# aynik/carta1

Measured on AMD Instinct MI355X. Metric: atrac1_stereo_frames_per_s_encode, higher is better.
Workload: dtype f32+f64

## Files before the change

carta1_amd/csrc/c1_api.hip:

```cpp
#include <algorithm>
#include <cmath>
#include <cstdarg>
#include <cstdio>
#include <cstdlib>
#include <cstring>
#include <limits>
#include <map>
#include <memory>
#include <atomic>
#include <mutex>
#include <string>
#include <thread>
#include <vector>

#include "c1_internal.h"
#include "c1_detect_bound.h"

#pragma clang fp contract(off)

namespace {

#include "c1_default_tables.inc"

thread_local std::string g_error;
// ... 66 lines not shown
  }
  for (int i = 0; i < 16; i++) { d->pre32_64[i][0] = (float)t.mdct_fwd64[2 * i]; d->pre32_64[i][1] = (float)t.mdct_fwd64[2 * i + 1]; }
  for (int i = 0; i < 64; i++) { d->pre32_256[i][0] = (float)t.mdct_fwd256[2 * i]; d->pre32_256[i][1] = (float)t.mdct_fwd256[2 * i + 1]; }
  for (int i = 0; i < 128; i++) { d->pre32_512[i][0] = (float)t.mdct_fwd512[2 * i]; d->pre32_512[i][1] = (float)t.mdct_fwd512[2 * i + 1]; }
  auto sigma2 = [&](const double *tab, int pairs, double want) {
    double mx = 0;
    for (int i = 0; i < pairs; i++) {
      const double m = tab[2 * i] * tab[2 * i] + tab[2 * i + 1] * tab[2 * i + 1];
      if (!(std::fabs(m - want) <= 1e-9 * want)) ok = false;
      mx = std::max(mx, m);
    }
    return mx;
  };
  const double s64 = sigma2(t.mdct_fwd64, 16, 0.5 / 64), s256 = sigma2(t.mdct_fwd256, 64, 0.5 / 256), s512 = sigma2(t.mdct_fwd512, 128, 1.0 / 512);
  const double (*tw)[2] = d->fft_tw;
  for (int h = 1; h <= 128; h <<= 1)
    for (int k = 0; k < h; k++) {
      const double ang = -M_PI * (double)k / (double)h;
      if (std::fabs(tw[h - 1 + k][0] - std::cos(ang)) > 1e-12 || std::fabs(tw[h - 1 + k][1] - std::sin(ang)) > 1e-12) ok = false;
    }
  for (int r = 0; r < 2; r++) {
    const int h = r == 0 ? 4 : 16;
    for (int k = 0; k < h; k++) {
      const double *a = tw[h - 1 + k], *b = tw[2 * h - 1 + k];
      float (*dst)[2] = r == 0 ? d->r4b[k] : d->r4c[k];
      dst[0][0] = (float)a[0]; dst[0][1] = (float)a[1];
      dst[1][0] = (float)b[0]; dst[1][1] = (float)b[1];
      dst[2][0] = (float)(a[0] * b[0] - a[1] * b[1]);
      dst[2][1] = (float)(a[0] * b[1] + a[1] * b[0]);
    }
  }
  for (int k = 0; k < 64; k++) { d->r2d[k][0] = (float)tw[63 + k][0]; d->r2d[k][1] = (float)tw[63 + k][1]; }
  for (int i = 0; i < 64 * 16; i++) d->norm32[i] = (float)d->norm[i];
  for (int i = 0; i < 16; i++) { d->inv32_64[i][0] = (float)t.mdct_inv64[2 * i]; d->inv32_64[i][1] = (float)t.mdct_inv64[2 * i + 1]; }
  for (int i = 0; i < 64; i++) { d->inv32_256[i][0] = (float)t.mdct_inv256[2 * i]; d->inv32_256[i][1] = (float)t.mdct_inv256[2 * i + 1]; }
  for (int i = 0; i < 128; i++) { d->inv32_512[i][0] = (float)t.mdct_inv512[2 * i]; d->inv32_512[i][1] = (float)t.mdct_inv512[2 * i + 1]; }
  for (int i = 0; i < 256; i++) { d->tw32[i][0] = (float)tw[i][0]; d->tw32[i][1] = (float)tw[i][1]; }
  const double u = std::ldexp(1.0, -24) * kSpecTheta;
  const double ka64 = kSpecKAPost + kSpecKARoundA + 2 * kSpecKARound4 + kSpecKAPre;
  const double ka128 = ka64 + kSpecKARound2;
  const double ka16 = kSpecKAPost + kSpecKARoundA + kSpecKARound4 + kSpecKAPre;
  for (int b = 0; b < 3; b++) {
    const double n = b == 2 ? 128 : 64, sg2 = b == 2 ? s512 : s256;
    d->spec_cz[b] = round_up_f32(u * (b == 2 ? ka128 : ka64) * std::sqrt(sg2 * n));
    const double gb = u * sg2 * std::sqrt(2 * n);
    if (b == 2) { d->spec_cw[b] = round_up_f32(gb * (5 * kSpecGH + kSpecGQ)); d->spec_cl[b] = 0.0f; }
    else { d->spec_cw[b] = round_up_f32(gb * kSpecGH * kSpecGQ); d->spec_cl[b] = round_up_f32(gb * (7 * kSpecGH + kSpecGQ)); }
    d->spec_cz_short[b] = round_up_f32(u * ka16 * std::sqrt(s64 * 16));
    const double gs = u * s64 * std::sqrt(2.0 * 16);
    if (b == 2) { d->spec_cw_short[b] = round_up_f32(gs * (5 * kSpecGH + kSpecGQ)); d->spec_cl_short[b] = 0.0f; }
    else { d->spec_cw_short[b] = round_up_f32(gs * kSpecGH * kSpecGQ); d->spec_cl_short[b] = round_up_f32(gs * (7 * kSpecGH + kSpecGQ)); }
  }
  d->spec_cz[3] = d->spec_cw[3] = d->spec_cl[3] = d->spec_cz_short[3] = d->spec_cw_short[3] = d->spec_cl_short[3] = 0.0f;
  d->spec_eabs = (float)std::ldexp(1.0, -70);
  for (int b = 0; b < 3; b++)
    d->det_ck[b] = round_up_f32(std::ldexp(1.0, -24) * C1_DET_THETA * (b == 2 ? C1_DET_K256 * 16.0 : C1_DET_K128 * std::sqrt(128.0)));
  d->det_ck[3] = 0.0f;
  d->det_eabs = round_up_f32(C1_DET_EABS);
  d->spec_ok = ok ? 1 : 0;
}

void build_device_tables(const c1_tables &t, C1DevTables *d) {
  memset(d, 0, sizeof *d);
  qmf_even_taps(d->tap_e);
  for (int j = 0; j < 24; j++) d->tap_o[j] = d->tap_e[23 - j];
  memcpy(d->window, t.window_short, sizeof d->window);
  memcpy(d->mdct_fwd64, t.mdct_fwd64, sizeof d->mdct_fwd64);
  memcpy(d->mdct_fwd256, t.mdct_fwd256, sizeof d->mdct_fwd256);
  memcpy(d->mdct_fwd512, t.mdct_fwd512, sizeof d->mdct_fwd512);
  memcpy(d->mdct_inv64, t.mdct_inv64, sizeof d->mdct_inv64);
  memcpy(d->mdct_inv256, t.mdct_inv256, sizeof d->mdct_inv256);
  memcpy(d->mdct_inv512, t.mdct_inv512, sizeof d->mdct_inv512);
  int stage = 0;
  for (int h = 1; h <= 128; h <<= 1, stage++) {
    const double wr = t.fft_w[stage][0], wi = t.fft_w[stage][1];
    double tr = 1.0, ti = 0.0;
    for (int k = 0; k < h; k++) {
      d->fft_tw[h - 1 + k][0] = tr;
      d->fft_tw[h - 1 + k][1] = ti;
      const double nr = tr * wr - ti * wi;
      ti = tr * wi + ti * wr;
      tr = nr;
    }
  }
  memcpy(d->scale_factors, t.scale_factors, sizeof d->scale_factors);
  for (int s = 0; s < 64; s++)
    for (int wl = 0; wl < 16; wl++) {
      const int bits = wl == 0 ? 0 : wl + 1;
      const int range = bits ? (1 << (bits - 1)) - 1 : 0;
      d->norm[s * 16 + wl] = (double)range / t.scale_factors[s];
    }
  d->log1p10 = t.log1p_10;
  auto floor_f32_bits = [](double x) -> uint32_t {
    float f = (float)x;
    if ((double)f > x) f = std::nextafterf(f, 0.0f);
    uint32_t u;
    memcpy(&u, &f, 4);
    return u;
  };
  d->sf_m1 = floor_f32_bits(C1D_SCALE_FACTORS[1]) & 0x7fffffu;
  d->sf_m2 = floor_f32_bits(C1D_SCALE_FACTORS[2]) & 0x7fffffu;
  d->sf_fast = 1;
  const uint32_t tm1 = floor_f32_bits(t.scale_factors[1]) & 0x7fffffu, tm2 = floor_f32_bits(t.scale_factors[2]) & 0x7fffffu;
  for (int i = 0; i < 64; i++) {
    const uint32_t u = floor_f32_bits(t.scale_factors[i]);
    const int e = (int)(u >> 23) - 127, want_e = i / 3 - 21;
    const uint32_t frac = u & 0x7fffffu, want = i % 3 == 0 ? 0u : (i % 3 == 1 ? tm1 : tm2);
    const bool exact_pow2 = i % 3 != 0 || (double)std::ldexp(1.0f, want_e) == t.scale_factors[i];
    if (e != want_e || frac != want || !exact_pow2) d->sf_fast = 0;
  }
  d->dq_fast = 1;
  d->dq_step = 1;
  for (int wl = 1; wl < 16 && d->dq_fast; wl++) {
    const int bits = wl + 1;
    const double range = (double)((1 << (bits - 1)) - 1), y = 1.0 / range;
    d->inv_range[wl] = y;
    for (int s = 1; s < 64 && d->dq_fast; s++) {
      const double sf = t.scale_factors[s];
      for (int q = -(1 << (bits - 1)); q < (1 << (bits - 1)); q++) {
        const double a = (double)q * sf;
        const double q0 = a * y, r = std::fma(-q0, range, a), fast = std::fma(r, y, q0), exact = a / range;
        if (!(fast == exact) || std::signbit(fast) != std::signbit(exact)) { d->dq_fast = 0; break; }
        const float f_exact = (float)exact, f_step = (float)((double)q * (sf * y));
        if (!(f_step == f_exact) || std::signbit(f_step) != std::signbit(f_exact)) d->dq_step = 0;
      }
    }
  }
  if (!d->dq_fast || getenv("C1_NO_DQ_STEP")) d->dq_step = 0;
  build_spec_tables(t, d);
}

int fill_call_fields(const c1_encode_options &o, C1DevEncOpts *d) {
  if (std::isnan(o.transient_threshold)) return fail(C1_ERR_ARG, "transient_threshold is NaN");
  d->threshold = o.transient_threshold;
  const bool detect = o.fixed_block_modes[0] < 0;
  for (int b = 0; b < 3; b++) {
    const int m = o.fixed_block_modes[b];
    if (detect) { d->modes[b] = -1; continue; }
    if (m < 0 || m > (b == 2 ? 3 : 2))
      return fail(C1_ERR_ARG, "fixed_block_modes[%d] = %d is outside 0..%d", b, m, b == 2 ? 3 : 2);
    d->modes[b] = m;
  }
  static const int no_tonal = getenv("C1_ALLOC_NO_TONAL") ? atoi(getenv("C1_ALLOC_NO_TONAL")) : 0;
  d->alloc_no_tonal = no_tonal;
  return C1_OK;
}

int build_table_fields(const c1_encode_options &o, C1DevEncOpts *d);

int build_encode_opts(const c1_encode_options &o, C1DevEncOpts *d) {
  struct Entry { double biased[64]; C1DevEncOpts table_part; };
  static std::mutex mu;
  static std::vector<Entry> cache;
  bool hit = false;
  {
    std::lock_guard<std::mutex> lock(mu);
    for (const Entry &e : cache)
      if (memcmp(e.biased, o.biased_scale_factors, sizeof e.biased) == 0) { *d = e.table_part; hit = true; break; }
  }
  if (!hit) {
    const int rc = build_table_fields(o, d);
    if (rc) return rc;
    std::lock_guard<std::mutex> lock(mu);
    if (cache.size() >= 8) cache.erase(cache.begin());
    Entry e;
    memcpy(e.biased, o.biased_scale_factors, sizeof e.biased);
    e.table_part = *d;
    cache.push_back(e);
  }
  return fill_call_fields(o, d);
}

int build_table_fields(const c1_encode_options &o, C1DevEncOpts *d) {
  memset(d, 0, sizeof *d);
  for (int i = 0; i < 64; i++) {
    if (!std::isfinite(o.biased_scale_factors[i]) || o.biased_scale_factors[i] < 0)
      return fail(C1_ERR_ARG, "biased_scale_factors[%d] is not a finite non-negative number", i);
    d->biased[i] = o.biased_scale_factors[i];
  }
  {
    const double l1 = std::log2(d->biased[1]), l63 = std::log2(d->biased[63]);
    const double slope = (l63 - l1) / 62.0;
    d->la_slope = (std::isfinite(slope) && std::isfinite(l1)) ? (float)slope : 0.0f;
    d->la_off = (std::isfinite(slope) && std::isfinite(l1)) ? (float)(l1 - slope) : 0.0f;
  }
  float pri[64 * 15];
  std::vector<float> uniq;
  for (int s = 1; s < 64; s++)
    for (int wl = 0; wl < 15; wl++) {
      const int b0 = wl == 0 ? 0 : wl + 1, b1 = wl + 2;
      const double ddf = wl == 0 ? 2.0 - std::ldexp(1.0, -b1) : std::ldexp(1.0, -b0) - std::ldexp(1.0, -b1);
      const double dbits = (double)(b1 - b0);
      pri[s * 15 + wl] = (float)(d->biased[s] * ddf / dbits);
      uniq.push_back(pri[s * 15 + wl]);
    }
  std::sort(uniq.begin(), uniq.end());
  uniq.erase(std::unique(uniq.begin(), uniq.end()), uniq.end());
  for (int s = 1; s < 64; s++)
    for (int wl = 0; wl < 15; wl++) {
      const auto it = std::lower_bound(uniq.begin(), uniq.end(), pri[s * 15 + wl]);
      d->rank[s * 16 + wl] = (uint16_t)(1 + (it - uniq.begin()));
    }
  d->rank_affine = 0;
  {
    std::vector<int> order;
    for (int s = 1; s < 64; s++)
      for (int wl = 0; wl < 15; wl++) order.push_back(s * 16 + wl);
    std::sort(order.begin(), order.end(), [&](int x, int y) { return d->rank[x] < d->rank[y]; });
    for (int A = 1; A <= 12 && !d->rank_affine; A++)
      for (int B = 1; B <= 36 && !d->rank_affine; B++)
        for (int C = -2 * B; C <= 2 * B && !d->rank_affine; C++) {
          auto key = [&](int idx) { const int s = idx >> 4, wl = idx & 15; return wl == 0 ? A * s + C : A * s - B * wl - B; };
          bool ok = true;
          int lo = key(order[0]), hi = lo;
          for (size_t i = 1; i < order.size() && ok; i++) {
            const int k0 = key(order[i - 1]), k1 = key(order[i]);
            const bool req = d->rank[order[i]] == d->rank[order[i - 1]];
            if (req ? (k1 != k0) : !(k1 > k0)) ok = false;
            lo = std::min(lo, k1); hi = std::max(hi, k1);
          }
          if (ok && hi - lo + 1 < 1023) {
            d->rank_affine = 1; d->rank_a = A; d->rank_b = B; d->rank_c = C; d->rank_off = 1 - lo;
          }
        }
  }
  if (d->rank_affine) {
    const int A = d->rank_a, B = d->rank_b, C = d->rank_c, off = d->rank_off;
    auto rk = [&](int s, int wl) { return wl == 0 ? A * s + C + off : A * s + off - B * (wl + 1); };
    auto entry = [&](int s, int wl) { return ((uint32_t)rk(s, wl) << 21) | ((uint32_t)s << 10) | ((uint32_t)wl << 6); };
    d->rank_step0 = (1u << 6) + ((uint32_t)(-2 * B - C) << 21);
    d->rank_step = (1u << 6) - ((uint32_t)B << 21);
    bool ok = true;
    for (int s = 1; s < 64 && ok; s++)
      for (int wl = 0; wl < 15 && ok; wl++) {
        if (rk(s, wl) < 1 || rk(s, wl) > 1022) ok = false;
        if (wl < 14 && entry(s, wl) + (wl == 0 ? d->rank_step0 : d->rank_step) != entry(s, wl + 1)) ok = false;
      }
    if (!ok) { d->rank_affine = 0; d->rank_step0 = d->rank_step = 0; }
  }
  {
    bool ok = true;
    for (int c = 0; c < 8; c++) {
      const double size = (double)kDistSizes[c];
      for (int s = 0; s < 64; s++) {
        const double bs = d->biased[s];
        const double zb = s != 0 ? (double)(float)(bs * 2.0 * size) : 0.0;
        const double cs = bs * size;
        d->dist[c][s][0] = zb;
        d->dist[c][s][1] = cs;
        if (s == 0) continue;
        if (!(zb >= (double)std::numeric_limits<float>::min())) ok = false;
        uint64_t u;
        memcpy(&u, &cs, sizeof u);
        for (int wl = 1; wl <= 15; wl++) {
          const int bits = wl + 1;
          const double want = bs * std::ldexp(1.0, -bits) * size;
          if ((int)((u >> 52) & 0x7ff) <= bits || (int)((u >> 52) & 0x7ff) == 0x7ff) { ok = false; continue; }
          const uint64_t v = u - ((uint64_t)bits << 52);
          if (memcmp(&v, &want, sizeof v) != 0) ok = false;
        }
      }
    }
    d->dist_tables = (ok && !getenv("C1_NO_DIST_TABLES")) ? 1 : 0;
  }
  return C1_OK;
}

constexpr int kTotals = 8;
constexpr int64_t kSpecMinUnits = 64;
constexpr int kListHead = 8;
constexpr int64_t kMaxModesBatchFrames = (int64_t)1 << 22;
constexpr int64_t kMaxChunkFrames = (int64_t)1 << 27;
constexpr bool kSignalStartsFused = false;

struct Timing {
  hipEvent_t start, stop;
  int kind;
};
enum { K_ANALYSIS = 0, K_ALLOCATE, K_PACK, K_DECODE, K_REDO, K_PACK_UNITS, K_DECODE_FIELDS, K_FROM_STATE, K_SIGNAL_STARTS, K_CHOOSE, K_MEASURE, K_METER, K_METER_PCM, K_KINDS };
const char *const kKindNames[K_KINDS] = {"analysis", "allocate", "pack", "decode", "redo", "pack_units", "decode_fields", "from_state", "signal_starts", "choose", "measure", "meter", "meter_pcm"};

}

struct c1_ctx {
  std::recursive_mutex mu;
  int device = 0;
  hipStream_t stream = nullptr;
  bool own_stream = false;
  C1DevTables *d_tables = nullptr;
  C1DevEncOpts *d_opts = nullptr;
  c1_encode_options last_opts;
  bool have_opts = false;
  int64_t ws_units = 0;
  float *d_coefs[2] = {nullptr, nullptr};
  uint8_t *d_side[2] = {nullptr, nullptr};
  uint8_t *d_alloc[2] = {nullptr, nullptr};
  uint8_t *d_cand[2] = {nullptr, nullptr};
  uint32_t *d_work[2] = {nullptr, nullptr};
  float *d_eps[2] = {nullptr, nullptr};
  uint32_t *d_redo[2] = {nullptr, nullptr};
  unsigned long long *d_spec_totals = nullptr;
  int spec_mode = 1;
  float spec_defer = 1.0f;
  bool decode_binary32 = false;
  int decode_model = C1_DECODE_EXACT;
  bool spec_tables_ok = false;
  int64_t det_units = 0;
  float *d_bands[2] = {nullptr, nullptr};
  double *d_feat[2] = {nullptr, nullptr};
  uint8_t *d_modes[2] = {nullptr, nullptr};
  uint32_t *d_lists[2] = {nullptr, nullptr};
  C1DevEncOpts *d_palette = nullptr;
  double *d_mask = nullptr, *h_mask = nullptr;
  hipEvent_t ev_mask = nullptr;
  double pal_tables[C1_MAX_BIAS_PALETTE][64];
  int pal_n = 0;
  uint32_t *d_pal_lists = nullptr;
  int64_t pal_entries = 0;
  uint8_t *d_trial = nullptr;
  int64_t trial_units = 0, trial_n = 0;
  float *d_bm_coefs = nullptr;
  uint8_t *d_bm_side = nullptr, *d_bm_cand_side = nullptr;
  int64_t bm_units = 0;
  bool overlap = false;
  hipStream_t s_tail = nullptr;
  hipEvent_t ev_main[2] = {nullptr, nullptr}, ev_tail[2] = {nullptr, nullptr};
  bool tail_used[2] = {false, false};
  bool tail_pending = false;
  int ws_next = 0;
  int64_t chunk_frames = 0;
  bool pipeline = true;
  int measured_wide = -1;
  bool signal_starts_fused = false;
  hipStream_t s_ana = nullptr, s_rest = nullptr;
  hipEvent_t ev_in = nullptr, ev_ana[2] = {nullptr, nullptr}, ev_free[2] = {nullptr, nullptr}, ev_end[2] = {nullptr, nullptr};
  int timing_depth = 0;
  bool profiling = false;
  std::vector<Timing> timings;
  std::vector<hipEvent_t> event_pool;
  double ms[K_KINDS] = {};
  int launches[K_KINDS] = {};
  void *d_io = nullptr;
  size_t d_io_bytes = 0;
  void *d_sig = nullptr;
  size_t d_sig_bytes = 0;
  uint32_t *h_rows = nullptr;
  size_t h_rows_bytes = 0;
  hipEvent_t ev_rows = nullptr;
  bool rows_pending = false;
  hipStream_t s_up = nullptr, s_down = nullptr;
  void *d_ring = nullptr;
  size_t d_ring_bytes = 0;
  hipEvent_t ev_up[2] = {nullptr, nullptr}, ev_run[2] = {nullptr, nullptr}, ev_down[2] = {nullptr, nullptr};
};

namespace {

#define CTX_GUARD(c)                                   \
  std::unique_lock<std::recursive_mutex> ctx_guard_;   \
  if (c) ctx_guard_ = std::unique_lock<std::recursive_mutex>((c)->mu)

int join_tail(c1_ctx *ctx) {
  if (!ctx->tail_pending) return C1_OK;
  for (int p = 0; p < 2; p++)
    if (ctx->tail_used[p]) HIP_TRY(hipStreamWaitEvent(ctx->stream, ctx->ev_tail[p], 0));
  ctx->tail_pending = false;
  return C1_OK;
}

int ctx_bind(c1_ctx *ctx, bool join = true) {
  if (!ctx) return fail(C1_ERR_ARG, "context is NULL");
  HIP_TRY(hipSetDevice(ctx->device));
  if (join) return join_tail(ctx);
  return C1_OK;
}

void free_workspace(c1_ctx *ctx) {
  for (int p = 0; p < 2; p++) {
    if (ctx->d_coefs[p]) (void)hipFree(ctx->d_coefs[p]);
    if (ctx->d_side[p]) (void)hipFree(ctx->d_side[p]);
    if (ctx->d_alloc[p]) (void)hipFree(ctx->d_alloc[p]);
    if (ctx->d_cand[p]) (void)hipFree(ctx->d_cand[p]);
    if (ctx->d_work[p]) (void)hipFree(ctx->d_work[p]);
    if (ctx->d_eps[p]) (void)hipFree(ctx->d_eps[p]);
    if (ctx->d_redo[p]) (void)hipFree(ctx->d_redo[p]);
    ctx->d_coefs[p] = nullptr; ctx->d_side[p] = nullptr; ctx->d_alloc[p] = nullptr; ctx->d_cand[p] = nullptr; ctx->d_work[p] = nullptr;
    ctx->d_eps[p] = nullptr; ctx->d_redo[p] = nullptr;
  }
  ctx->ws_units = 0;
  for (int p = 0; p < 2; p++) {
    if (ctx->d_bands[p]) (void)hipFree(ctx->d_bands[p]);
    if (ctx->d_feat[p]) (void)hipFree(ctx->d_feat[p]);
    if (ctx->d_modes[p]) (void)hipFree(ctx->d_modes[p]);
    if (ctx->d_lists[p]) (void)hipFree(ctx->d_lists[p]);
    ctx->d_bands[p] = nullptr; ctx->d_feat[p] = nullptr; ctx->d_modes[p] = nullptr; ctx->d_lists[p] = nullptr;
  }
  ctx->det_units = 0;
  if (ctx->d_pal_lists) (void)hipFree(ctx->d_pal_lists);
  ctx->d_pal_lists = nullptr;
  ctx->pal_entries = 0;
  if (ctx->d_trial) (void)hipFree(ctx->d_trial);
  ctx->d_trial = nullptr;
  ctx->trial_units = ctx->trial_n = 0;
  if (ctx->d_bm_coefs) (void)hipFree(ctx->d_bm_coefs);
  if (ctx->d_bm_side) (void)hipFree(ctx->d_bm_side);
  if (ctx->d_bm_cand_side) (void)hipFree(ctx->d_bm_cand_side);
  ctx->d_bm_coefs = nullptr; ctx->d_bm_side = nullptr; ctx->d_bm_cand_side = nullptr;
  ctx->bm_units = 0;
}

int ensure_detect_workspace(c1_ctx *ctx, int64_t units) {
  if (units <= ctx->det_units) return C1_OK;
  HIP_TRY(hipDeviceSynchronize());
  for (int p = 0; p < (ctx->pipeline ? 2 : 1); p++) {
    if (ctx->d_bands[p]) (void)hipFree(ctx->d_bands[p]);
    if (ctx->d_feat[p]) (void)hipFree(ctx->d_feat[p]);
    if (ctx->d_modes[p]) (void)hipFree(ctx->d_modes[p]);
    if (ctx->d_lists[p]) (void)hipFree(ctx->d_lists[p]);
    ctx->d_bands[p] = nullptr; ctx->d_feat[p] = nullptr; ctx->d_modes[p] = nullptr; ctx->d_lists[p] = nullptr;
    HIP_TRY(hipMalloc(&ctx->d_bands[p], (size_t)(units + C1_MAX_CHANNELS) * 512 * sizeof(float)));
    HIP_TRY(hipMalloc(&ctx->d_feat[p], (size_t)(units + C1_MAX_CHANNELS) * kFeatureWsDoubles * sizeof(double)));
    HIP_TRY(hipMalloc(&ctx->d_modes[p], (size_t)units));
    HIP_TRY(hipMalloc(&ctx->d_lists[p], ((size_t)units * 3 + 4) * sizeof(uint32_t)));
  }
  ctx->det_units = units;
  return C1_OK;
}

int ensure_workspace(c1_ctx *ctx, int64_t units) {
  if (units <= ctx->ws_units) return C1_OK;
  HIP_TRY(hipDeviceSynchronize());
  free_workspace(ctx);
  ctx->tail_used[0] = ctx->tail_used[1] = false;
  ctx->tail_pending = false;
  for (int p = 0; p < ((ctx->pipeline || ctx->overlap) ? 2 : 1); p++) {
    HIP_TRY(hipMalloc(&ctx->d_coefs[p], (size_t)units * 512 * sizeof(float)));
    HIP_TRY(hipMalloc(&ctx->d_side[p], (size_t)units * kSideBytes));
    HIP_TRY(hipMalloc(&ctx->d_alloc[p], (size_t)units * kAllocBytes));
    HIP_TRY(hipMalloc(&ctx->d_cand[p], (size_t)units * kCandidateBytes));
    HIP_TRY(hipMalloc(&ctx->d_work[p], ((size_t)units * 8 + 4) * sizeof(uint32_t)));
    HIP_TRY(hipMalloc(&ctx->d_eps[p], (size_t)units * kEpsFloats * sizeof(float)));
    HIP_TRY(hipMalloc(&ctx->d_redo[p], ((size_t)units * 4 + kListHead + 64) * sizeof(uint32_t)));
  }
  ctx->ws_units = units;
  return C1_OK;
}

constexpr size_t kWsBytesPerUnit = 512 * sizeof(float) + kSideBytes + kAllocBytes + kCandidateBytes + 8 * sizeof(uint32_t) + kEpsFloats * sizeof(float) + 4 * sizeof(uint32_t);
constexpr size_t kDetectWsBytesPerUnit = 512 * sizeof(float) + kFeatureWsDoubles * sizeof(double) + 1 + 3 * sizeof(uint32_t);
constexpr size_t kBestModesWsBytesPerUnit = 512 * sizeof(float) + 2 * kSideBytes;
int64_t chunk_for_call(c1_ctx *ctx, int64_t frames, int channels, bool detect, int trial_n = 0, bool best_modes = false) {
  const int64_t want = std::min(frames, ctx->chunk_frames);
  const bool trial_fits = trial_n == 0 || (want * channels <= ctx->trial_units && trial_n <= ctx->trial_n);
  if (want * channels <= ctx->ws_units && (!detect || want * channels <= ctx->det_units) && trial_fits &&
      (!best_modes || want * channels <= ctx->bm_units)) return want;
  size_t free_b = 0, total_b = 0;
  if (hipMemGetInfo(&free_b, &total_b) != hipSuccess) { (void)hipGetLastError(); return std::min<int64_t>(want, 1048576); }
  const size_t sets = (ctx->pipeline || ctx->overlap) ? 2 : 1, det_sets = ctx->pipeline ? 2 : 1;
  size_t avail = free_b + (size_t)ctx->ws_units * kWsBytesPerUnit * sets;
  size_t per_unit = kWsBytesPerUnit * sets;
  if (detect) { avail += (size_t)ctx->det_units * kDetectWsBytesPerUnit * det_sets; per_unit += kDetectWsBytesPerUnit * det_sets; }
  if (trial_n > 0) { avail += (size_t)ctx->trial_units * ctx->trial_n * kAllocBytes; per_unit += (size_t)trial_n * kAllocBytes; }
  if (best_modes) { avail += (size_t)ctx->bm_units * kBestModesWsBytesPerUnit; per_unit += kBestModesWsBytesPerUnit; }
  const int64_t fit = (int64_t)((double)avail * 0.9 / (double)per_unit) / channels;
  return std::max<int64_t>(16, std::min(want, fit));
}

void bind_lists(c1_ctx *ctx, int p, C1EncodeLaunch *L) {
  uint32_t *base = ctx->d_redo[p];
  const size_t u = (size_t)ctx->ws_units;
  L->redo_count = base;
  L->realloc_count = base + 1;
  L->reana_count = base + 2;
  L->redo_list = base + kListHead;
  L->realloc_list = base + kListHead + u;
  L->reana_list = base + kListHead + 2 * u;
}
void bind_defer(c1_ctx *ctx, int p, C1EncodeLaunch *L) {
  L->defer_list = ctx->d_redo[p] + kListHead + 3 * (size_t)ctx->ws_units;
}

int ensure_io(c1_ctx *ctx, size_t bytes) {
  if (bytes <= ctx->d_io_bytes) return C1_OK;
  if (ctx->d_io) hipFree(ctx->d_io);
  ctx->d_io = nullptr; ctx->d_io_bytes = 0;
  HIP_TRY(hipMalloc(&ctx->d_io, bytes));
  ctx->d_io_bytes = bytes;
  return C1_OK;
}

int upload_opts(c1_ctx *ctx, const c1_encode_options *opts) {
  if (!opts) return fail(C1_ERR_ARG, "options are NULL");
  if (ctx->have_opts && memcmp(&ctx->last_opts, opts, sizeof *opts) == 0) return C1_OK;
  C1DevEncOpts h;
  const int rc = build_encode_opts(*opts, &h);
  if (rc) return rc;
  int jr = join_tail(ctx);
  if (jr) return jr;
  HIP_TRY(hipStreamSynchronize(ctx->stream));
  HIP_TRY(hipMemcpy(ctx->d_opts, &h, sizeof h, hipMemcpyHostToDevice));
  ctx->last_opts = *opts;
  ctx->have_opts = true;
  return C1_OK;
}

struct PaletteCall {
  int n;
  const uint8_t *index;
};

int check_palette(const char *what, const c1_encode_options *palette, int n, bool call_fields) {
  if (n < 1 || n > C1_MAX_BIAS_PALETTE) return fail(C1_ERR_ARG, "%s: n_palette = %d is outside 1..%d", what, n, C1_MAX_BIAS_PALETTE);
  if (!palette) return fail(C1_ERR_ARG, "%s: palette is NULL", what);
  std::unique_ptr<C1DevEncOpts> d(new C1DevEncOpts);
  for (int k = 0; k < n; k++) {
    c1_encode_options o = palette[k];
    if (!call_fields) {
      o.transient_threshold = 1.0;
      o.fixed_block_modes[0] = o.fixed_block_modes[1] = o.fixed_block_modes[2] = -1;
    }
    const int rc = build_encode_opts(o, d.get());
    if (rc) { const std::string inner = g_error; return fail(rc, "%s: palette entry %d: %s", what, k, inner.c_str()); }
    if (call_fields && k > 0) {
      if (memcmp(&palette[k].transient_threshold, &palette[0].transient_threshold, sizeof(double)) != 0)
        return fail(C1_ERR_ARG, "%s: palette entry %d: transient_threshold differs from entry 0's, and no modes are given", what, k);
      if (memcmp(palette[k].fixed_block_modes, palette[0].fixed_block_modes, sizeof palette[0].fixed_block_modes) != 0)
        return fail(C1_ERR_ARG, "%s: palette entry %d: fixed_block_modes differ from entry 0's, and no modes are given", what, k);
    }
  }
  return C1_OK;
}

int check_measured_opts(const char *what, const c1_encode_options *opts, bool call_fields) {
  if (!opts) return fail(C1_ERR_ARG, "%s: options are NULL", what);
  std::unique_ptr<C1DevEncOpts> d(new C1DevEncOpts);
  c1_encode_options o = *opts;
  if (!call_fields) {
    o.transient_threshold = 1.0;
    o.fixed_block_modes[0] = o.fixed_block_modes[1] = o.fixed_block_modes[2] = -1;
  }
  const int rc = build_encode_opts(o, d.get());
  if (rc) { const std::string inner = g_error; return fail(rc, "%s: %s", what, inner.c_str()); }
  return C1_OK;
}

int upload_palette(c1_ctx *ctx, const char *what, const c1_encode_options *palette, int n) {
  bool same = ctx->d_palette && ctx->pal_n >= n;
  for (int k = 0; k < n && same; k++) same = memcmp(ctx->pal_tables[k], palette[k].biased_scale_factors, sizeof ctx->pal_tables[k]) == 0;
  if (same) return C1_OK;
  std::unique_ptr<C1DevEncOpts[]> h(new C1DevEncOpts[C1_MAX_BIAS_PALETTE]);
  for (int k = 0; k < n; k++) {
    c1_encode_options o = palette[k];
    o.transient_threshold = 1.0;
    o.fixed_block_modes[0] = o.fixed_block_modes[1] = o.fixed_block_modes[2] = -1;
    const int rc = build_encode_opts(o, &h[k]);
    if (rc) { const std::string inner = g_error; return fail(rc, "%s: palette entry %d: %s", what, k, inner.c_str()); }
  }
  int jr = join_tail(ctx);
  if (jr) return jr;
  HIP_TRY(hipStreamSynchronize(ctx->stream));
  if (!ctx->d_palette) HIP_TRY(hipMalloc(&ctx->d_palette, C1_MAX_BIAS_PALETTE * sizeof(C1DevEncOpts)));
  ctx->pal_n = 0;
  HIP_TRY(hipMemcpy(ctx->d_palette, h.get(), (size_t)n * sizeof(C1DevEncOpts), hipMemcpyHostToDevice));
  for (int k = 0; k < n; k++) memcpy(ctx->pal_tables[k], palette[k].biased_scale_factors, sizeof ctx->pal_tables[k]);
  ctx->pal_n = n;
  return C1_OK;
}

int ensure_palette_lists(c1_ctx *ctx, int64_t units, int n) {
  const int64_t entries = units * n;
  if (entries <= ctx->pal_entries) return C1_OK;
  HIP_TRY(hipDeviceSynchronize());
  if (ctx->d_pal_lists) (void)hipFree(ctx->d_pal_lists);
  ctx->d_pal_lists = nullptr; ctx->pal_entries = 0;
  HIP_TRY(hipMalloc(&ctx->d_pal_lists, ((size_t)entries + 8) * sizeof(uint32_t)));
  ctx->pal_entries = entries;
  return C1_OK;
}

int ensure_trial_allocs(c1_ctx *ctx, int64_t units, int n) {
  if (units <= ctx->trial_units && n <= ctx->trial_n) return C1_OK;
  HIP_TRY(hipDeviceSynchronize());
  if (ctx->d_trial) (void)hipFree(ctx->d_trial);
  ctx->d_trial = nullptr; ctx->trial_units = ctx->trial_n = 0;
  const int64_t u = std::max(units, ctx->trial_units), planes = std::max<int64_t>(n, ctx->trial_n);
  HIP_TRY(hipMalloc(&ctx->d_trial, (size_t)u * planes * kAllocBytes));
  ctx->trial_units = u; ctx->trial_n = planes;
  return C1_OK;
}

int ensure_best_modes_planes(c1_ctx *ctx, int64_t units) {
  if (units <= ctx->bm_units) return C1_OK;
  HIP_TRY(hipDeviceSynchronize());
  if (ctx->d_bm_coefs) (void)hipFree(ctx->d_bm_coefs);
  if (ctx->d_bm_side) (void)hipFree(ctx->d_bm_side);
  if (ctx->d_bm_cand_side) (void)hipFree(ctx->d_bm_cand_side);
  ctx->d_bm_coefs = nullptr; ctx->d_bm_side = nullptr; ctx->d_bm_cand_side = nullptr; ctx->bm_units = 0;
  HIP_TRY(hipMalloc(&ctx->d_bm_coefs, (size_t)units * 512 * sizeof(float)));
  HIP_TRY(hipMalloc(&ctx->d_bm_side, (size_t)units * kSideBytes));
  HIP_TRY(hipMalloc(&ctx->d_bm_cand_side, (size_t)units * kSideBytes));
  ctx->bm_units = units;
  return C1_OK;
}

struct BestModesCall {
  int n;
  const uint8_t *cand;
  uint8_t *choice, *modes_out;
  double *distortion, *energy;
  const int8_t *sf_offsets = nullptr;
  int n_offsets = 0;
  uint8_t *taken = nullptr;
  int8_t *shifts = nullptr;
};

struct BestBiasCall {
  int n;
  uint8_t *choice;
  double *distortion, *energy;
};

struct MeasuredCall {
  uint8_t *taken;
  double *distortion, *energy;
  const int8_t *sf_offsets = nullptr;
  int n_offsets = 0;
  int8_t *shifts = nullptr;
  const double *mask = nullptr;
  bool has_spread = false;
  double *weights = nullptr;
};

int check_index_bytes(const char *what, const uint8_t *index, int64_t frames, int channels, int n) {
  for (int64_t i = 0; i < frames * channels; i++) {
    if (index[i] < n) continue;
    if (channels == 2) return fail(C1_ERR_ARG, "%s: frame %lld, channel %d: bias index %d is not below n_palette = %d", what, (long long)(i / 2), (int)(i & 1), (int)index[i], n);
    return fail(C1_ERR_ARG, "%s: frame %lld: bias index %d is not below n_palette = %d", what, (long long)i, (int)index[i], n);
  }
  return C1_OK;
}

hipEvent_t take_event(c1_ctx *ctx) {
  if (!ctx->event_pool.empty()) {
    hipEvent_t e = ctx->event_pool.back();
    ctx->event_pool.pop_back();
    return e;
  }
  hipEvent_t e;
  hipEventCreateWithFlags(&e, hipEventDisableSystemFence);
  return e;
}
struct ScopedTiming {
  c1_ctx *ctx;
  Timing t;
  bool on;
  hipStream_t stream;
  ScopedTiming(c1_ctx *c, int kind, hipStream_t s = nullptr) : ctx(c), on(c->profiling), stream(s ? s : c->stream) {
    if (!on) return;
    t.kind = kind;
    t.start = take_event(ctx);
    t.stop = take_event(ctx);
    (void)hipEventRecord(t.start, stream);
  }
  ~ScopedTiming() {
    if (!on) return;
    (void)hipEventRecord(t.stop, stream);
    ctx->timings.push_back(t);
  }
};
void reset_timings(c1_ctx *ctx) {
  for (auto &t : ctx->timings) { ctx->event_pool.push_back(t.start); ctx->event_pool.push_back(t.stop); }
  ctx->timings.clear();
  for (int k = 0; k < K_KINDS; k++) { ctx->ms[k] = 0; ctx->launches[k] = 0; }
}
int collect_timings(c1_ctx *ctx) {
  if (ctx->timings.empty()) return C1_OK;
  int jr = join_tail(ctx);
  if (jr) return jr;
  HIP_TRY(hipStreamSynchronize(ctx->stream));
  for (auto &t : ctx->timings) {
    float ms = 0;
    HIP_TRY(hipEventElapsedTime(&ms, t.start, t.stop));
    ctx->ms[t.kind] += ms;
    ctx->launches[t.kind]++;
    ctx->event_pool.push_back(t.start);
    ctx->event_pool.push_back(t.stop);
  }
  ctx->timings.clear();
  return C1_OK;
}

void launch_measured(c1_ctx *ctx, const C1EncodeLaunch &L, bool all_long, const MeasuredCall *mc, int64_t at, hipStream_t stream) {
  ScopedTiming t(ctx, K_MEASURE, stream);
  uint8_t *taken = mc->taken ? mc->taken + at : nullptr;
  int8_t *shifts = mc->shifts ? mc->shifts + at * 52 : nullptr;
  double *distortion = mc->distortion ? mc->distortion + at * 2 : nullptr, *energy = mc->energy ? mc->energy + at : nullptr;
  double *weights = mc->weights ? mc->weights + at * 52 : nullptr;
  const bool finalize = L.units != nullptr;
  const int64_t units = L.frames * L.channels;
  const bool wide = ctx->measured_wide < 0 ? units <= kMeasuredWideUnits : ctx->measured_wide != 0;
  if (wide) {
    static const int8_t kNoOffset[1] = {0};
    c1k_launch_measured_wide(L, all_long, finalize, mc->sf_offsets ? mc->sf_offsets : kNoOffset, mc->sf_offsets ? mc->n_offsets : 1, mc->mask,
                             mc->has_spread, taken, mc->sf_offsets ? shifts : nullptr, distortion, energy, weights, stream);
  } else if (mc->mask) {
    c1k_launch_measured_masked(L, all_long, finalize, mc->sf_offsets, mc->n_offsets, mc->mask, mc->has_spread, taken, shifts, distortion,
                               energy, weights, stream);
  } else if (mc->sf_offsets) {
    c1k_launch_measured_sf(L, all_long, finalize, mc->sf_offsets, mc->n_offsets, taken, shifts, distortion, energy, stream);
  } else {
    c1k_launch_measured_alloc(L, all_long, finalize, taken, distortion, energy, stream);
  }
}

void launch_measured_modes(c1_ctx *ctx, const C1EncodeLaunch &L, const uint8_t *trial, int64_t trial_stride, const BestModesCall *bm,
                           int64_t at, hipStream_t stream) {
  ScopedTiming t(ctx, K_MEASURE, stream);
  const int64_t units = L.frames * L.channels;
  const bool wide = ctx->measured_wide < 0 ? units <= kMeasuredModesWideUnits : ctx->measured_wide != 0;
  (wide ? c1k_launch_measured_modes_wide : c1k_launch_measured_modes)(
      L, ctx->d_bm_coefs, ctx->d_bm_side, trial, trial_stride, bm->cand, bm->n, bm->sf_offsets, bm->n_offsets, L.units != nullptr,
      bm->choice ? bm->choice + at : nullptr, bm->modes_out ? bm->modes_out + at : nullptr, bm->taken ? bm->taken + at : nullptr,
      bm->shifts ? bm->shifts + at * 52 : nullptr, bm->distortion ? bm->distortion + at * bm->n * 2 : nullptr,
      bm->energy ? bm->energy + at * bm->n : nullptr, stream);
}

int check_channels(int channels) {
  if (channels != 1 && channels != 2) return fail(C1_ERR_ARG, "channels must be 1 or 2, got %d", channels);
  return C1_OK;
}

int check_mode_bytes(const char *what, const uint8_t *modes, int64_t frames, int channels) {
  static const char *const kField[3] = {"low", "mid", "high"};
  for (int64_t i = 0; i < frames * channels; i++) {
    const int b = modes[i];
    if ((b & ~0x3a) == 0 && ((b & 0x30) == 0 || (b & 0x30) == 0x30)) continue;
    char where[64];
    if (channels == 2) snprintf(where, sizeof where, "frame %lld, channel %d", (long long)(i / 2), (int)(i & 1));
    else snprintf(where, sizeof where, "frame %lld", (long long)i);
    for (int k = 0; k < 3; k++) {
      const int m = (b >> (2 * k)) & 3, other = k == 2 ? 3 : 2;
      if (m != 0 && m != other)
        return fail(C1_ERR_ARG, "%s: %s: %s field of mode byte 0x%02x is %d, not 0 or %d", what, where, kField[k], b, m, other);
    }
    return fail(C1_ERR_ARG, "%s: %s: bits 6-7 of mode byte 0x%02x are set", what, where, b);
  }
  return C1_OK;
}

int encode_device_impl(c1_ctx *ctx, const float *const *pcm, int channels, int64_t frames, int halo_frames,
                       const c1_encode_options *opts, uint8_t *units, float *bands, float *coefs_tap,
                       uint8_t *side_tap, uint8_t *alloc_tap, bool lazy = false, const uint8_t *given_modes = nullptr,
                       const PaletteCall *pal = nullptr, const BestBiasCall *best = nullptr, const BestModesCall *bm = nullptr,
                       const MeasuredCall *mc = nullptr) {
  CTX_GUARD(ctx);
  int rc = ctx_bind(ctx, false);
  if (rc) return rc;
  if ((rc = check_channels(channels))) return rc;
  if (frames < 0) return fail(C1_ERR_ARG, "frames must be >= 0");
  if (halo_frames < 0 || halo_frames > 2) return fail(C1_ERR_ARG, "halo_frames must be 0, 1 or 2");
  if (!pcm) return fail(C1_ERR_ARG, "pcm is NULL");
  for (int c = 0; c < channels; c++) {
    if (!pcm[c] && frames > 0) return fail(C1_ERR_ARG, "pcm[%d] is NULL", c);
    if ((uintptr_t)pcm[c] & 15) return fail(C1_ERR_ARG, "pcm[%d] must be 16-byte aligned on the device", c);
  }
  if ((rc = upload_opts(ctx, opts))) return rc;
  if (ctx->profiling && ctx->timing_depth == 0) reset_timings(ctx);
  if (frames == 0) return C1_OK;
  const bool detect = given_modes || bm || opts->fixed_block_modes[0] < 0;
  const bool taps = coefs_tap || side_tap || alloc_tap;
  const int64_t chunk = taps ? ctx->chunk_frames : chunk_for_call(ctx, frames, channels, detect, best ? best->n : (bm ? bm->n : 0), bm != nullptr);
  if ((rc = ensure_workspace(ctx, (taps ? frames : std::min(frames, chunk)) * channels))) return rc;
  if (detect && (rc = ensure_detect_workspace(ctx, (taps ? frames : std::min(frames, chunk)) * channels))) return rc;
  if (pal && (rc = ensure_palette_lists(ctx, std::min(frames, chunk) * channels, pal->n))) return rc;
  if (best && (rc = ensure_trial_allocs(ctx, std::min(frames, chunk) * channels, best->n))) return rc;
  if (bm && (rc = ensure_trial_allocs(ctx, std::min(frames, chunk) * channels, bm->n))) return rc;
  if (bm && (rc = ensure_best_modes_planes(ctx, std::min(frames, chunk) * channels))) return rc;
  bool bm_long = false, bm_short = false;
  for (int k = 0; bm && k < bm->n; k++) {
    if ((bm->cand[k] & 0x3f) != 0x3a) bm_long = true;
    if ((bm->cand[k] & 0x3f) != 0) bm_short = true;
  }
  if (taps && (!coefs_tap || !side_tap || !alloc_tap)) return fail(C1_ERR_ARG, "coefs, side and alloc taps must be given together");
  if (taps && frames > kMaxChunkFrames) return fail(C1_ERR_ARG, "stage taps are not chunked: at most %lld frames per call", (long long)kMaxChunkFrames);
  const bool all_long_modes = !detect && opts->fixed_block_modes[0] == 0 && opts->fixed_block_modes[1] == 0 &&
                              opts->fixed_block_modes[2] == 0 && !getenv("C1_NO_FAST_LONG");
  const bool all_short_modes = !detect && opts->fixed_block_modes[0] != 0 && opts->fixed_block_modes[1] != 0 &&
                               opts->fixed_block_modes[2] != 0;
  bool speculate = (all_long_modes || all_short_modes) && !taps && !pal && !best && !bm && !mc && units && ctx->spec_tables_ok && ctx->spec_mode != 0;
  bool quantize32 = !taps && units && ctx->spec_tables_ok && ctx->spec_mode != 0;
  static const bool det_spec_env_off = getenv("C1_DETECT_SPEC") && atoi(getenv("C1_DETECT_SPEC")) == 0;
  bool detect_spec = detect && !given_modes && !bm && !taps && ctx->spec_tables_ok && ctx->spec_mode != 0 && !det_spec_env_off;
  if (ctx->spec_mode == 1 && frames * channels < kSpecMinUnits) speculate = quantize32 = detect_spec = false;
  const bool overlap = speculate && ctx->overlap && ctx->s_tail != nullptr;
  if (!overlap && (rc = join_tail(ctx))) return rc;
  const bool piped = ctx->pipeline && !taps && frames > chunk && !speculate && !bm;
  hipStream_t sA = piped ? ctx->s_ana : ctx->stream, sB = piped ? ctx->s_rest : ctx->stream;
  if (piped) {
    HIP_TRY(hipEventRecord(ctx->ev_in, ctx->stream));
    HIP_TRY(hipStreamWaitEvent(sA, ctx->ev_in, 0));
    HIP_TRY(hipStreamWaitEvent(sB, ctx->ev_in, 0));
  }
  int64_t index = 0;
  for (int64_t f0 = 0, n = 0; f0 < frames; f0 += n, ++index) {
    n = taps ? frames : std::min(chunk, frames - f0);
    int p = piped ? (int)(index & 1) : 0;
    if (overlap) { p = ctx->ws_next; ctx->ws_next ^= 1; }
    C1EncodeLaunch L;
    memset(&L, 0, sizeof L);
    for (int c = 0; c < channels; c++) L.pcm[c] = pcm[c] + f0 * 512;
    L.channels = channels;
    L.frames = n;
    L.halo_frames = (int)std::min<int64_t>(2, f0 + halo_frames);
    L.tables = ctx->d_tables;
    L.opts = ctx->d_opts;
    L.coefs = taps ? coefs_tap : ctx->d_coefs[p];
    L.side = taps ? side_tap : ctx->d_side[p];
    L.alloc = taps ? alloc_tap : ctx->d_alloc[p];
    L.cand = ctx->d_cand[p];
    L.work_count = ctx->d_work[p];
    L.work_list = ctx->d_work[p] + 4;
    L.sel_list = ctx->d_work[p] + 4 + (size_t)ctx->ws_units * 7;
    L.bands = bands ? bands + f0 * channels * 512 : nullptr;
    L.units = units ? units + f0 * channels * C1_UNIT_BYTES : nullptr;
    const bool all_long = all_long_modes;
    if (piped && index >= 2) HIP_TRY(hipStreamWaitEvent(sA, ctx->ev_free[p], 0));
    if (speculate) {
      L.eps = ctx->d_eps[p];
      bind_lists(ctx, p, &L);
      if (ctx->spec_mode == 1) { bind_defer(ctx, p, &L); L.spec_defer = ctx->spec_defer; }
      if (c1k_pick_run(n, channels, 0) <= 64 && !getenv("C1_NO_SF_PREPASS"))
        L.open_masks = reinterpret_cast<unsigned long long *>((reinterpret_cast<uintptr_t>(ctx->d_redo[p] + kListHead + 3 * (size_t)ctx->ws_units + (size_t)ctx->ws_units / 4 + 4) + 7) & ~(uintptr_t)7);
      if (overlap && ctx->tail_used[p]) HIP_TRY(hipStreamWaitEvent(sA, ctx->ev_tail[p], 0));
      HIP_TRY(hipMemsetAsync(ctx->d_redo[p], 0, kListHead * sizeof(uint32_t), sA));
      {
        ScopedTiming t(ctx, K_ANALYSIS, sA);
        c1k_launch_analysis_spec(L, all_short_modes, sA);
        if (L.defer_list) {
          C1EncodeLaunch D = L;
          uint32_t *dense = ctx->d_redo[p] + kListHead + 2 * (size_t)ctx->ws_units;
          c1k_launch_defer_compact(L, dense, ctx->d_redo[p] + 3, sA);
          D.unit_list = dense;
          D.unit_count = ctx->d_redo[p] + 3;
          D.list_runs = 1;
          D.defer_list = nullptr;
          if (all_long_modes) c1k_launch_analysis_long(D, sA); else c1k_launch_analysis(D, false, sA);
        }
      }
      if (L.open_masks) {
        ScopedTiming t(ctx, K_REDO, sA);
        {
          C1EncodeLaunch X = L;
          uint32_t *open_list = ctx->d_redo[p] + kListHead + 2 * (size_t)ctx->ws_units;
          c1k_launch_open_compact(L, open_list, ctx->d_redo[p] + 5, sA);
          X.unit_list = open_list;
          X.unit_count = ctx->d_redo[p] + 5;
          X.list_runs = 0;
          X.list_zero_eps = 1;
          X.defer_list = nullptr;
          X.open_masks = nullptr;
          if (all_long_modes) c1k_launch_analysis_long(X, sA); else c1k_launch_analysis(X, false, sA);
        }
      }
      { ScopedTiming t(ctx, K_ALLOCATE, sA); c1k_launch_allocate(L, sA); }
      if (overlap && ctx->tail_used[p ^ 1]) HIP_TRY(hipStreamWaitEvent(sA, ctx->ev_tail[p ^ 1], 0));
      { ScopedTiming t(ctx, K_PACK, sA); c1k_launch_pack_spec(L, all_long_modes, sA); }
      hipStream_t sT = sA;
      if (overlap) {
        sT = ctx->s_tail;
        HIP_TRY(hipEventRecord(ctx->ev_main[p], sA));
        HIP_TRY(hipStreamWaitEvent(sT, ctx->ev_main[p], 0));
      }
      {
        ScopedTiming t(ctx, K_REDO, sT);
        hipStream_t sA = sT;
        C1EncodeLaunch R = L;
        R.defer_list = nullptr;
        R.unit_list = L.reana_list;
        R.unit_count = L.reana_count;
        if (all_long_modes) c1k_launch_analysis_long(R, sA); else c1k_launch_analysis(R, false, sA);
        if (!L.open_masks) {
          C1EncodeLaunch A = R;
          A.unit_list = L.realloc_list;
          A.unit_count = L.realloc_count;
          c1k_launch_allocate(A, sA);
        }
        R.unit_list = L.redo_list;
        R.unit_count = L.redo_count;
        c1k_launch_pack(R, all_long_modes, sA);
        c1k_launch_spec_totals(ctx->d_spec_totals, (uint64_t)(n * channels), ctx->d_redo[p], 0, sA);
      }
      if (overlap) {
        HIP_TRY(hipEventRecord(ctx->ev_tail[p], sT));
        ctx->tail_used[p] = true;
        ctx->tail_pending = true;
      }
      continue;
    }
    {
      ScopedTiming t(ctx, K_ANALYSIS, sA);
      if (all_long) c1k_launch_analysis_long(L, sA);
      else if (bm) {
        C1EncodeLaunch S2 = L;
        S2.coefs = ctx->d_bm_coefs;
        S2.side = ctx->d_bm_side;
        HIP_TRY(hipMemsetAsync(ctx->d_bm_cand_side, bm_long ? 0 : 0x3a, (size_t)n * channels, sA));
        c1k_launch_modes_front(L, ctx->d_bm_cand_side, ctx->d_bands[p], ctx->d_modes[p], ctx->d_lists[p], sA);
        c1k_launch_mdct_bands(bm_long ? L : S2, ctx->d_bands[p], ctx->d_modes[p], ctx->d_lists[p], sA);
        if (bm_long && bm_short) {
          c1k_launch_const_mode_lists(0x3a, n * channels, ctx->d_modes[p], ctx->d_lists[p], sA);
          c1k_launch_mdct_bands(S2, ctx->d_bands[p], ctx->d_modes[p], ctx->d_lists[p], sA);
        }
      } else if (given_modes) {
        c1k_launch_modes_front(L, given_modes + f0 * channels, ctx->d_bands[p], ctx->d_modes[p], ctx->d_lists[p], sA);
        c1k_launch_mdct_bands(L, ctx->d_bands[p], ctx->d_modes[p], ctx->d_lists[p], sA);
      } else if (detect) {
        c1k_launch_detect(L, ctx->d_bands[p], ctx->d_feat[p], ctx->d_modes[p], ctx->d_lists[p], detect_spec, nullptr, sA);
        if (detect_spec) c1k_launch_spec_totals(ctx->d_spec_totals, (uint64_t)(n * channels), ctx->d_lists[p] + 2, 2, sA);
        if (L.bands) HIP_TRY(hipMemcpyAsync(L.bands, ctx->d_bands[p] + (size_t)channels * 512, (size_t)n * channels * 512 * sizeof(float),
                                            hipMemcpyDeviceToDevice, sA));
      } else c1k_launch_analysis(L, false, sA);
    }
    if (piped) {
      HIP_TRY(hipEventRecord(ctx->ev_ana[p], sA));
      HIP_TRY(hipStreamWaitEvent(sB, ctx->ev_ana[p], 0));
    }
    if (bm) {
      const int64_t trial_stride = ctx->trial_units * kAllocBytes;
      for (int k = 0; k < bm->n; k++) {
        { ScopedTiming t(ctx, K_ANALYSIS, sB); c1k_launch_compose_side(L.side, ctx->d_bm_side, n * channels, bm->cand[k], ctx->d_bm_cand_side, sB); }
        ScopedTiming t(ctx, K_ALLOCATE, sB);
        C1EncodeLaunch A = L;
        A.side = ctx->d_bm_cand_side;
        A.alloc = ctx->d_trial + (size_t)k * trial_stride;
        c1k_launch_allocate(A, sB);
      }
      if (bm->sf_offsets) {
        launch_measured_modes(ctx, L, ctx->d_trial, trial_stride, bm, f0 * channels, sB);
      } else {
        ScopedTiming t(ctx, K_CHOOSE, sB);
        c1k_launch_choose_modes(L, ctx->d_bm_coefs, ctx->d_bm_side, ctx->d_trial, trial_stride, bm->cand, bm->n, L.units != nullptr,
                                bm->choice ? bm->choice + f0 * channels : nullptr, bm->modes_out ? bm->modes_out + f0 * channels : nullptr,
                                bm->distortion ? bm->distortion + f0 * channels * bm->n : nullptr,
                                bm->energy ? bm->energy + f0 * channels * bm->n : nullptr, sB);
      }
    } else if (best) {
      const int64_t trial_stride = ctx->trial_units * kAllocBytes;
      {
        ScopedTiming t(ctx, K_ALLOCATE, sB);
        for (int k = 0; k < best->n; k++) {
          C1EncodeLaunch A = L;
          A.opts = ctx->d_palette + k;
          A.alloc = ctx->d_trial + (size_t)k * trial_stride;
          c1k_launch_allocate(A, sB);
        }
      }
      ScopedTiming t(ctx, K_CHOOSE, sB);
      c1k_launch_choose_bias(L, ctx->d_trial, trial_stride, best->n, all_long, best->choice ? best->choice + f0 * channels : nullptr,
                             best->distortion ? best->distortion + f0 * channels * best->n : nullptr,
                             best->energy ? best->energy + f0 * channels : nullptr, sB);
    } else if (pal) {
      ScopedTiming t(ctx, K_ALLOCATE, sB);
      c1k_launch_allocate_palette(L, ctx->d_palette, pal->n, pal->index + f0 * channels, ctx->d_pal_lists, ctx->d_pal_lists + 8, n * channels, sB);
    } else { ScopedTiming t(ctx, K_ALLOCATE, sB); c1k_launch_allocate(L, sB); }
    if (mc) launch_measured(ctx, L, all_long, mc, f0 * channels, sB);
    if (L.units && quantize32) {
      ScopedTiming t(ctx, K_PACK, sB);
      L.eps = ctx->d_eps[p];
      bind_lists(ctx, p, &L);
      HIP_TRY(hipMemsetAsync(L.eps, 0, (size_t)n * channels * kEpsFloats * sizeof(float), sB));
      HIP_TRY(hipMemsetAsync(ctx->d_redo[p], 0, kListHead * sizeof(uint32_t), sB));
      c1k_launch_pack_spec(L, all_long, sB);
      C1EncodeLaunch R = L;
      R.unit_list = L.redo_list;
      R.unit_count = L.redo_count;
      c1k_launch_pack(R, all_long, sB);
      c1k_launch_spec_totals(ctx->d_spec_totals, (uint64_t)(n * channels), L.redo_count, 1, sB);
    } else if (L.units) { ScopedTiming t(ctx, K_PACK, sB); c1k_launch_pack(L, all_long, sB); }
    if (piped) HIP_TRY(hipEventRecord(ctx->ev_free[p], sB));
  }
  if (piped) {
    HIP_TRY(hipEventRecord(ctx->ev_end[0], sA));
    HIP_TRY(hipEventRecord(ctx->ev_end[1], sB));
    HIP_TRY(hipStreamWaitEvent(ctx->stream, ctx->ev_end[0], 0));
    HIP_TRY(hipStreamWaitEvent(ctx->stream, ctx->ev_end[1], 0));
  }
  if (overlap && !lazy && (rc = join_tail(ctx))) return rc;
  HIP_TRY(hipGetLastError());
  return C1_OK;
}

struct XsMatrix {
  uint32_t col[32];
  uint32_t apply(uint32_t s) const {
    uint32_t r = 0;
    for (int b = 0; b < 32; b++) if ((s >> b) & 1u) r ^= col[b];
    return r;
  }
};
uint32_t xs_step(uint32_t s) { s ^= s << 13; s ^= s >> 17; s ^= s << 5; return s; }
XsMatrix xs_power(uint64_t n) {
  XsMatrix result, base;
  for (int b = 0; b < 32; b++) { result.col[b] = 1u << b; base.col[b] = xs_step(1u << b); }
  while (n) {
    if (n & 1) { XsMatrix r; for (int b = 0; b < 32; b++) r.col[b] = base.apply(result.col[b]); result = r; }
    XsMatrix sq;
    for (int b = 0; b < 32; b++) sq.col[b] = base.apply(base.col[b]);
    base = sq;
    n >>= 1;
  }
  return result;
}

}

namespace {
struct DeviceScratch {
  std::vector<void *> ptrs;
  ~DeviceScratch() { for (void *p : ptrs) (void)hipFree(p); }
  template <class T> int alloc(T **out, size_t count) {
    void *p = nullptr;
    if (hipMalloc(&p, std::max<size_t>(count, 1) * sizeof(T)) != hipSuccess) return fail(C1_ERR_HIP, "device allocation of %zu bytes failed", count * sizeof(T));
    ptrs.push_back(p);
    *out = static_cast<T *>(p);
    return C1_OK;
  }
};
}

extern "C" {

int c1_abi_version(void) { return C1_ABI_VERSION; }
const char *c1_last_error(void) { return g_error.c_str(); }

int c1_device_count(int *count) {
  if (!count) return fail(C1_ERR_ARG, "count is NULL");
  int n = 0;
  const hipError_t e = hipGetDeviceCount(&n);
  if (e != hipSuccess) {
    *count = 0;
    return fail(C1_ERR_NO_DEVICE, "hipGetDeviceCount: %s", hipGetErrorString(e));
  }
  *count = n;
  return C1_OK;
}

int c1_get_default_tables(c1_tables *out) {
  if (!out) return fail(C1_ERR_ARG, "out is NULL");
  default_tables(out);
  return C1_OK;
}

int c1_set_tables(const c1_tables *tables) {
  std::lock_guard<std::mutex> lock(g_tables_mutex);
  if (!tables) { g_tables_custom = false; g_tables_gen++; return C1_OK; }
  const double *p = reinterpret_cast<const double *>(tables);
  for (size_t i = 0; i < sizeof(c1_tables) / sizeof(double); i++)
    if (!std::isfinite(p[i])) return fail(C1_ERR_ARG, "table entry %zu is not finite", i);
  g_tables = *tables;
  g_tables_custom = true;
  g_tables_gen++;
  return C1_OK;
}

int c1_table_fast_paths(int *scale_factor_bits, int *dequant_reciprocal) {
  c1_tables t;
  {
    std::lock_guard<std::mutex> lock(g_tables_mutex);
    if (g_tables_custom) t = g_tables; else default_tables(&t);
  }
  std::unique_ptr<C1DevTables> d(new C1DevTables);
  build_device_tables(t, d.get());
  if (scale_factor_bits) *scale_factor_bits = d->sf_fast;
  if (dequant_reciprocal) *dequant_reciprocal = d->dq_fast + d->dq_step;
  return C1_OK;
}

int c1_alloc_rank_form(const c1_encode_options *opts, int *affine, int *coef) {
  if (!opts) return fail(C1_ERR_ARG, "opts is NULL");
  std::unique_ptr<C1DevEncOpts> d(new C1DevEncOpts);
  const int rc = build_table_fields(*opts, d.get());
  if (rc) return rc;
  if (affine) *affine = d->rank_affine;
  if (coef) { coef[0] = d->rank_a; coef[1] = d->rank_b; coef[2] = d->rank_c; coef[3] = d->rank_off; }
  return C1_OK;
}

int c1_alloc_tables(const c1_encode_options *opts, int *affine, uint32_t *steps, uint16_t *rank, int *dist_ok, double *dist) {
  if (!opts) return fail(C1_ERR_ARG, "opts is NULL");
  std::unique_ptr<C1DevEncOpts> d(new C1DevEncOpts);
  const int rc = build_table_fields(*opts, d.get());
  if (rc) return rc;
  if (affine) *affine = d->rank_affine;
  if (steps) { steps[0] = d->rank_step0; steps[1] = d->rank_step; }
  if (rank) {
    for (int s = 0; s < 64; s++)
      for (int wl = 0; wl < 16; wl++)
        rank[s * 16 + wl] = !d->rank_affine ? d->rank[s * 16 + wl]
                            : (uint16_t)(wl == 0 ? d->rank_a * s + d->rank_c + d->rank_off : d->rank_a * s + d->rank_off - d->rank_b * (wl + 1));
  }
  if (dist_ok) *dist_ok = d->dist_tables;
  if (dist) memcpy(dist, d->dist, sizeof d->dist);
  return C1_OK;
}

int c1_default_encode_options(c1_encode_options *out) {
  if (!out) return fail(C1_ERR_ARG, "out is NULL");
  memset(out, 0, sizeof *out);
  c1_tables t;
  {
    std::lock_guard<std::mutex> lock(g_tables_mutex);
    if (g_tables_custom) t = g_tables; else default_tables(&t);
  }
  memcpy(out->biased_scale_factors, t.scale_factors, sizeof out->biased_scale_factors);
  out->transient_threshold = 1.0;
  out->fixed_block_modes[0] = out->fixed_block_modes[1] = out->fixed_block_modes[2] = -1;
  return C1_OK;
}

int c1_ctx_create(int device, void *hip_stream, c1_ctx **out) {
  if (!out) return fail(C1_ERR_ARG, "out is NULL");
  *out = nullptr;
  int n = 0;
  const hipError_t e = hipGetDeviceCount(&n);
  if (e != hipSuccess || n == 0)
    return fail(C1_ERR_NO_DEVICE, "no HIP device available (%s); this library has no CPU path",
                e != hipSuccess ? hipGetErrorString(e) : "device count is 0");
  if (device < 0 || device >= n) return fail(C1_ERR_ARG, "device %d out of range (0..%d)", device, n - 1);
  HIP_TRY(hipSetDevice(device));
  c1_ctx *ctx = new c1_ctx();
  ctx->device = device;
  if (hip_stream) ctx->stream = (hipStream_t)hip_stream;
  else {
    const hipError_t se = hipStreamCreateWithFlags(&ctx->stream, hipStreamNonBlocking);
    if (se != hipSuccess) { delete ctx; return fail(C1_ERR_HIP, "hipStreamCreate: %s", hipGetErrorString(se)); }
    ctx->own_stream = true;
  }
  c1_tables t;
  {
    std::lock_guard<std::mutex> lock(g_tables_mutex);
    if (g_tables_custom) t = g_tables; else default_tables(&t);
  }
  C1DevTables *h = new C1DevTables();
  build_device_tables(t, h);
  hipError_t me = hipMalloc(&ctx->d_tables, sizeof(C1DevTables));
  if (me == hipSuccess) me = hipMalloc(&ctx->d_opts, sizeof(C1DevEncOpts));
  if (me == hipSuccess) me = hipMemcpy(ctx->d_tables, h, sizeof *h, hipMemcpyHostToDevice);
  if (me == hipSuccess) me = hipMalloc(&ctx->d_spec_totals, kTotals * sizeof(unsigned long long));
  if (me == hipSuccess) me = hipMemset(ctx->d_spec_totals, 0, kTotals * sizeof(unsigned long long));
  ctx->spec_tables_ok = h->spec_ok != 0;
  {
    const char *sp = getenv("C1_SPEC");
    ctx->spec_mode = sp ? atoi(sp) : 1;
    if (ctx->spec_mode < 0 || ctx->spec_mode > 2) ctx->spec_mode = 1;
    const char *sd = getenv("C1_SPEC_DEFER");
    if (sd && atof(sd) > 0) ctx->spec_defer = (float)atof(sd);
  }
  delete h;
  if (me != hipSuccess) { c1_ctx_destroy(ctx); return fail(C1_ERR_HIP, "table upload: %s", hipGetErrorString(me)); }
  {
    hipError_t pe = hipStreamCreateWithFlags(&ctx->s_ana, hipStreamNonBlocking);
    if (pe == hipSuccess) pe = hipStreamCreateWithFlags(&ctx->s_rest, hipStreamNonBlocking);
    if (pe == hipSuccess) pe = hipEventCreateWithFlags(&ctx->ev_in, hipEventDisableTiming);
    for (int p = 0; p < 2 && pe == hipSuccess; p++) {
      pe = hipEventCreateWithFlags(&ctx->ev_ana[p], hipEventDisableTiming);
      if (pe == hipSuccess) pe = hipEventCreateWithFlags(&ctx->ev_free[p], hipEventDisableTiming);
      if (pe == hipSuccess) pe = hipEventCreateWithFlags(&ctx->ev_end[p], hipEventDisableTiming);
    }
    if (pe != hipSuccess) { c1_ctx_destroy(ctx); return fail(C1_ERR_HIP, "pipeline streams: %s", hipGetErrorString(pe)); }
    if (pe == hipSuccess) pe = hipStreamCreateWithFlags(&ctx->s_tail, hipStreamNonBlocking);
    for (int p = 0; p < 2 && pe == hipSuccess; p++) {
      pe = hipEventCreateWithFlags(&ctx->ev_main[p], hipEventDisableTiming);
      if (pe == hipSuccess) pe = hipEventCreateWithFlags(&ctx->ev_tail[p], hipEventDisableTiming);
    }
    if (pe != hipSuccess) { c1_ctx_destroy(ctx); return fail(C1_ERR_HIP, "tail stream: %s", hipGetErrorString(pe)); }
    const char *ov = getenv("C1_OVERLAP");
    ctx->overlap = ov ? atoi(ov) != 0 : false;
    const char *pl = getenv("C1_PIPELINE");
    ctx->pipeline = pl ? atoi(pl) != 0 : false;
  }
  const char *mw = getenv("C1_MEASURED_WIDE");
  ctx->measured_wide = mw ? (atoi(mw) != 0 ? 1 : 0) : -1;
  const char *ss = getenv("C1_SIGNAL_STARTS");
  ctx->signal_starts_fused = ss ? atoi(ss) != 0 : kSignalStartsFused;
  const char *env = getenv("C1_CHUNK_FRAMES");
  ctx->chunk_frames = env ? atoll(env) : (int64_t)1 << 24;
  if (ctx->chunk_frames < 16) ctx->chunk_frames = 16;
  if (ctx->chunk_frames > kMaxChunkFrames) ctx->chunk_frames = kMaxChunkFrames;
  *out = ctx;
  return C1_OK;
}

int c1_ctx_destroy(c1_ctx *ctx) {
  if (!ctx) return C1_OK;
  hipSetDevice(ctx->device);
  if (ctx->s_tail) hipStreamSynchronize(ctx->s_tail);
  if (ctx->stream) hipStreamSynchronize(ctx->stream);
  for (auto &t : ctx->timings) { hipEventDestroy(t.start); hipEventDestroy(t.stop); }
  for (auto e : ctx->event_pool) hipEventDestroy(e);
  if (ctx->d_tables) hipFree(ctx->d_tables);
  if (ctx->d_opts) hipFree(ctx->d_opts);
  if (ctx->d_palette) hipFree(ctx->d_palette);
  if (ctx->d_mask) hipFree(ctx->d_mask);
  if (ctx->h_mask) hipHostFree(ctx->h_mask);
  if (ctx->ev_mask) hipEventDestroy(ctx->ev_mask);
  if (ctx->d_spec_totals) hipFree(ctx->d_spec_totals);
  (void)hipDeviceSynchronize();
  free_workspace(ctx);
  if (ctx->s_tail) (void)hipStreamDestroy(ctx->s_tail);
  for (int p = 0; p < 2; p++) {
    if (ctx->ev_main[p]) (void)hipEventDestroy(ctx->ev_main[p]);
    if (ctx->ev_tail[p]) (void)hipEventDestroy(ctx->ev_tail[p]);
  }
  if (ctx->s_ana) (void)hipStreamDestroy(ctx->s_ana);
  if (ctx->s_rest) (void)hipStreamDestroy(ctx->s_rest);
  if (ctx->ev_in) (void)hipEventDestroy(ctx->ev_in);
  for (int p = 0; p < 2; p++) {
    if (ctx->ev_ana[p]) (void)hipEventDestroy(ctx->ev_ana[p]);
    if (ctx->ev_free[p]) (void)hipEventDestroy(ctx->ev_free[p]);
    if (ctx->ev_end[p]) (void)hipEventDestroy(ctx->ev_end[p]);
  }
  if (ctx->d_io) hipFree(ctx->d_io);
  if (ctx->d_sig) (void)hipFree(ctx->d_sig);
  if (ctx->h_rows) (void)hipHostFree(ctx->h_rows);
  if (ctx->ev_rows) (void)hipEventDestroy(ctx->ev_rows);
  if (ctx->d_ring) (void)hipFree(ctx->d_ring);
  if (ctx->s_up) (void)hipStreamDestroy(ctx->s_up);
  if (ctx->s_down) (void)hipStreamDestroy(ctx->s_down);
  for (int p = 0; p < 2; p++) {
    if (ctx->ev_up[p]) (void)hipEventDestroy(ctx->ev_up[p]);
    if (ctx->ev_run[p]) (void)hipEventDestroy(ctx->ev_run[p]);
    if (ctx->ev_down[p]) (void)hipEventDestroy(ctx->ev_down[p]);
  }
  if (ctx->own_stream && ctx->stream) hipStreamDestroy(ctx->stream);
  delete ctx;
  return C1_OK;
}

int c1_ctx_synchronize(c1_ctx *ctx) {
  CTX_GUARD(ctx);
  int rc = ctx_bind(ctx);
  if (rc) return rc;
  HIP_TRY(hipStreamSynchronize(ctx->stream));
  return C1_OK;
}

int c1_ctx_set_profiling(c1_ctx *ctx, int enabled) {
  if (!ctx) return fail(C1_ERR_ARG, "context is NULL");
  CTX_GUARD(ctx);
  ctx->profiling = enabled != 0;
  return C1_OK;
}

int c1_ctx_set_speculation(c1_ctx *ctx, int mode) {
  if (!ctx) return fail(C1_ERR_ARG, "context is NULL");
  if (mode < 0 || mode > 2) return fail(C1_ERR_ARG, "speculation mode must be 0, 1 or 2, got %d", mode);
  CTX_GUARD(ctx);
  ctx->spec_mode = mode;
  return C1_OK;
}

int c1_ctx_set_decode_model(c1_ctx *ctx, int model) {
  if (!ctx) return fail(C1_ERR_ARG, "context is NULL");
  if (model != C1_DECODE_EXACT && model != C1_DECODE_BINARY32_BULK && model != C1_DECODE_BINARY32)
    return fail(C1_ERR_ARG, "decode model must be 0, 1 or 2, got %d", model);
  CTX_GUARD(ctx);
  ctx->decode_model = model;
  ctx->decode_binary32 = model != C1_DECODE_EXACT;
  return C1_OK;
}

int c1_ctx_get_decode_model(c1_ctx *ctx, int *model) {
  if (!ctx) return fail(C1_ERR_ARG, "context is NULL");
  if (!model) return fail(C1_ERR_ARG, "model is NULL");
  CTX_GUARD(ctx);
  *model = ctx->decode_model;
  return C1_OK;
}

int c1_ctx_set_decode_precision(c1_ctx *ctx, int binary32) {
  return c1_ctx_set_decode_model(ctx, binary32 ? C1_DECODE_BINARY32_BULK : C1_DECODE_EXACT);
}

int c1_ctx_speculation_stats(c1_ctx *ctx, uint64_t *units, uint64_t *redone, int reset) {
  CTX_GUARD(ctx);
  int rc = ctx_bind(ctx);
  if (rc) return rc;
  unsigned long long tot[2] = {0, 0};
  HIP_TRY(hipMemcpyAsync(tot, ctx->d_spec_totals, sizeof tot, hipMemcpyDeviceToHost, ctx->stream));
  HIP_TRY(hipStreamSynchronize(ctx->stream));
  if (units) *units = tot[0];
  if (redone) *redone = tot[1];
  if (reset) {
    HIP_TRY(hipMemsetAsync(ctx->d_spec_totals, 0, kTotals * sizeof(unsigned long long), ctx->stream));
    HIP_TRY(hipStreamSynchronize(ctx->stream));
  }
  return C1_OK;
}

int c1_ctx_speculation_deferred(c1_ctx *ctx, uint64_t *units) {
  CTX_GUARD(ctx);
  int rc = ctx_bind(ctx);
  if (rc) return rc;
  unsigned long long tot[kTotals];
  HIP_TRY(hipMemcpyAsync(tot, ctx->d_spec_totals, sizeof tot, hipMemcpyDeviceToHost, ctx->stream));
  HIP_TRY(hipStreamSynchronize(ctx->stream));
  if (units) *units = tot[6];
  return C1_OK;
}

int c1_ctx_quantization_stats(c1_ctx *ctx, uint64_t *units, uint64_t *repacked) {
  CTX_GUARD(ctx);
  int rc = ctx_bind(ctx);
  if (rc) return rc;
  unsigned long long tot[4] = {0, 0, 0, 0};
  HIP_TRY(hipMemcpyAsync(tot, ctx->d_spec_totals, sizeof tot, hipMemcpyDeviceToHost, ctx->stream));
  HIP_TRY(hipStreamSynchronize(ctx->stream));
  if (units) *units = tot[2];
  if (repacked) *repacked = tot[3];
  return C1_OK;
}

int c1_ctx_detection_stats(c1_ctx *ctx, uint64_t *units, uint64_t *rechecked) {
  CTX_GUARD(ctx);
  int rc = ctx_bind(ctx);
  if (rc) return rc;
  unsigned long long tot[6] = {0, 0, 0, 0, 0, 0};
  HIP_TRY(hipMemcpyAsync(tot, ctx->d_spec_totals, sizeof tot, hipMemcpyDeviceToHost, ctx->stream));
  HIP_TRY(hipStreamSynchronize(ctx->stream));
  if (units) *units = tot[4];
  if (rechecked) *rechecked = tot[5];
  return C1_OK;
}

int c1_ctx_kernel_ms(c1_ctx *ctx, const char *name, double *ms, int *launches) {
  CTX_GUARD(ctx);
  int rc = ctx_bind(ctx);
  if (rc) return rc;
  if (!name || !ms) return fail(C1_ERR_ARG, "name or ms is NULL");
  if ((rc = collect_timings(ctx))) return rc;
  double total = 0;
  int count = 0;
  for (int k = 0; k < K_KINDS; k++) {
    if (!strcmp(name, kKindNames[k])) {
      *ms = ctx->ms[k];
      if (launches) *launches = ctx->launches[k];
      return C1_OK;
    }
    total += ctx->ms[k];
    count += ctx->launches[k];
  }
  if (!strcmp(name, "total")) {
    *ms = total;
    if (launches) *launches = count;
    return C1_OK;
  }
  return fail(C1_ERR_ARG, "unknown kernel name '%s'", name);
}

int c1_encode_device(c1_ctx *ctx, const float *const *pcm, int channels, int64_t frames, int halo_frames,
                     const c1_encode_options *opts, uint8_t *units) {
  if (!units && frames > 0) return fail(C1_ERR_ARG, "units is NULL");
  return encode_device_impl(ctx, pcm, channels, frames, halo_frames, opts, units, nullptr, nullptr, nullptr, nullptr, ctx && ctx->own_stream);
}
static int encode_device_joined(c1_ctx *ctx, const float *const *pcm, int channels, int64_t frames, int halo_frames,
                                const c1_encode_options *opts, uint8_t *units) {
  if (!units && frames > 0) return fail(C1_ERR_ARG, "units is NULL");
  return encode_device_impl(ctx, pcm, channels, frames, halo_frames, opts, units, nullptr, nullptr, nullptr, nullptr, false);
}

int c1_encode_modes_device(c1_ctx *ctx, const float *const *pcm, int channels, int64_t frames, int halo_frames,
                           const c1_encode_options *opts, const uint8_t *modes, uint8_t *units) {
  if (frames > 0 && (!modes || !units)) return fail(C1_ERR_ARG, "modes or units is NULL");
  if (frames > kMaxChunkFrames) return fail(C1_ERR_ARG, "at most %lld frames per call", (long long)kMaxChunkFrames);
  return encode_device_impl(ctx, pcm, channels, frames, halo_frames, opts, units, nullptr, nullptr, nullptr, nullptr, false, frames > 0 ? modes : nullptr);
}

int c1_encode_stages_device(c1_ctx *ctx, const float *const *pcm, int channels, int64_t frames, int halo_frames,
                            const c1_encode_options *opts, float *bands, float *coefs, uint8_t *side,
                            uint8_t *alloc) {
  return encode_device_impl(ctx, pcm, channels, frames, halo_frames, opts, nullptr, bands, coefs, side, alloc);
}

int c1_detect_stages_device(c1_ctx *ctx, const float *const *pcm, int channels, int64_t frames, int halo_frames,
                            const c1_encode_options *opts, float *mags, uint8_t *modes) {
  CTX_GUARD(ctx);
  int rc = ctx_bind(ctx);
  if (rc) return rc;
  if ((rc = check_channels(channels))) return rc;
  if (frames < 0 || halo_frames < 0 || halo_frames > 2) return fail(C1_ERR_ARG, "bad frames / halo_frames");
  if (!pcm || !opts) return fail(C1_ERR_ARG, "NULL argument");
  if (opts->fixed_block_modes[0] >= 0) return fail(C1_ERR_ARG, "the detector taps need transient detection (fixed_block_modes -1)");
  if (frames > kMaxChunkFrames) return fail(C1_ERR_ARG, "stage taps are not chunked: at most %lld frames per call", (long long)kMaxChunkFrames);
  for (int c = 0; c < channels; c++)
    if (!pcm[c] || ((uintptr_t)pcm[c] & 15)) return fail(C1_ERR_ARG, "pcm[%d] must be a 16-byte aligned device pointer", c);
  if ((rc = upload_opts(ctx, opts))) return rc;
  if (frames == 0) return C1_OK;
  const int64_t units = frames * channels;
  if ((rc = ensure_workspace(ctx, units))) return rc;
  if ((rc = ensure_detect_workspace(ctx, units))) return rc;
  C1EncodeLaunch L;
  memset(&L, 0, sizeof L);
  for (int c = 0; c < channels; c++) L.pcm[c] = pcm[c];
  L.channels = channels; L.frames = frames; L.halo_frames = halo_frames;
  L.tables = ctx->d_tables; L.opts = ctx->d_opts;
  L.coefs = ctx->d_coefs[0]; L.side = ctx->d_side[0]; L.alloc = ctx->d_alloc[0]; L.cand = ctx->d_cand[0];
  L.work_count = ctx->d_work[0]; L.work_list = ctx->d_work[0] + 4; L.sel_list = ctx->d_work[0] + 4 + (size_t)ctx->ws_units * 7;
  L.mags = mags;
  c1k_launch_detect(L, ctx->d_bands[0], ctx->d_feat[0], ctx->d_modes[0], ctx->d_lists[0], false, nullptr, ctx->stream);
  if (modes) HIP_TRY(hipMemcpyAsync(modes, ctx->d_modes[0], (size_t)units, hipMemcpyDeviceToDevice, ctx->stream));
  HIP_TRY(hipGetLastError());
  return C1_OK;
}

int c1_detect_scores_device(c1_ctx *ctx, const float *const *pcm, int channels, int64_t frames, int halo_frames,
                            const c1_encode_options *opts, int speculative, double *scores, uint8_t *modes, uint32_t *open_units) {
  CTX_GUARD(ctx);
  int rc = ctx_bind(ctx);
  if (rc) return rc;
  if ((rc = check_channels(channels))) return rc;
  if (frames < 0 || halo_frames < 0 || halo_frames > 2) return fail(C1_ERR_ARG, "bad frames / halo_frames");
  if (!pcm || !opts) return fail(C1_ERR_ARG, "NULL argument");
  if (opts->fixed_block_modes[0] >= 0) return fail(C1_ERR_ARG, "the detector taps need transient detection (fixed_block_modes -1)");
  if (frames > kMaxChunkFrames) return fail(C1_ERR_ARG, "stage taps are not chunked: at most %lld frames per call", (long long)kMaxChunkFrames);
  if (speculative && !ctx->spec_tables_ok) return fail(C1_ERR_ARG, "the installed tables do not admit the speculative paths");
  for (int c = 0; c < channels; c++)
    if (!pcm[c] || ((uintptr_t)pcm[c] & 15)) return fail(C1_ERR_ARG, "pcm[%d] must be a 16-byte aligned device pointer", c);
  if ((rc = upload_opts(ctx, opts))) return rc;
  if (frames == 0) return C1_OK;
  const int64_t units = frames * channels;
  if ((rc = ensure_detect_workspace(ctx, units))) return rc;
  C1EncodeLaunch L;
  memset(&L, 0, sizeof L);
  for (int c = 0; c < channels; c++) L.pcm[c] = pcm[c];
  L.channels = channels; L.frames = frames; L.halo_frames = halo_frames;
  L.tables = ctx->d_tables; L.opts = ctx->d_opts;
  c1k_launch_detect(L, ctx->d_bands[0], ctx->d_feat[0], ctx->d_modes[0], ctx->d_lists[0], speculative != 0, scores, ctx->stream);
  if (modes) HIP_TRY(hipMemcpyAsync(modes, ctx->d_modes[0], (size_t)units, hipMemcpyDeviceToDevice, ctx->stream));
  if (open_units) HIP_TRY(hipMemcpyAsync(open_units, ctx->d_lists[0] + 2, sizeof(uint32_t), hipMemcpyDeviceToDevice, ctx->stream));
  HIP_TRY(hipGetLastError());
  return C1_OK;
}

int c1_detect_spec_mags_device(c1_ctx *ctx, const float *const *pcm, int channels, int64_t frames, int halo_frames,
                               float *mags, float *bounds) {
  CTX_GUARD(ctx);
  int rc = ctx_bind(ctx);
  if (rc) return rc;
  if ((rc = check_channels(channels))) return rc;
  if (frames < 0 || halo_frames < 0 || halo_frames > 2) return fail(C1_ERR_ARG, "bad frames / halo_frames");
  if (!pcm || !mags || !bounds) return fail(C1_ERR_ARG, "NULL argument");
  if (frames > kMaxChunkFrames) return fail(C1_ERR_ARG, "stage taps are not chunked: at most %lld frames per call", (long long)kMaxChunkFrames);
  if (!ctx->spec_tables_ok) return fail(C1_ERR_ARG, "the installed tables do not admit the speculative paths");
  for (int c = 0; c < channels; c++)
    if (!pcm[c] || ((uintptr_t)pcm[c] & 15)) return fail(C1_ERR_ARG, "pcm[%d] must be a 16-byte aligned device pointer", c);
  if (frames == 0) return C1_OK;
  if ((rc = ensure_detect_workspace(ctx, frames * channels))) return rc;
  C1EncodeLaunch L;
  memset(&L, 0, sizeof L);
  for (int c = 0; c < channels; c++) L.pcm[c] = pcm[c];
  L.channels = channels; L.frames = frames; L.halo_frames = halo_frames;
  L.tables = ctx->d_tables; L.opts = ctx->d_opts;
  L.mags = mags; L.mag_bounds = bounds;
  c1k_launch_detect_spec_tap(L, ctx->d_bands[0], ctx->d_feat[0], ctx->stream);
  HIP_TRY(hipGetLastError());
  return C1_OK;
}

int c1_log2f_error_device(c1_ctx *ctx, uint32_t first_bits, uint64_t count, double *out_host) {
  CTX_GUARD(ctx);
  int rc = ctx_bind(ctx);
  if (rc) return rc;
  if (!out_host) return fail(C1_ERR_ARG, "out is NULL");
  if (first_bits < 0x00800000u || (uint64_t)first_bits + count > 0x7f800000ull) return fail(C1_ERR_ARG, "range must stay within the normal positive binary32 numbers");
  if ((rc = ensure_io(ctx, 16))) return rc;
  c1k_launch_log2f_error(first_bits, count, reinterpret_cast<unsigned long long *>(ctx->d_io), ctx->stream);
  HIP_TRY(hipGetLastError());
  HIP_TRY(hipMemcpyAsync(out_host, ctx->d_io, 16, hipMemcpyDeviceToHost, ctx->stream));
  HIP_TRY(hipStreamSynchronize(ctx->stream));
  return C1_OK;
}

int c1_alloc_bounds_device(c1_ctx *ctx, const uint8_t *side, int64_t units, const c1_encode_options *opts, double *out) {
  CTX_GUARD(ctx);
  int rc = ctx_bind(ctx);
  if (rc) return rc;
  if (units < 0 || units > ((int64_t)1 << 24) || (units > 0 && (!side || !out))) return fail(C1_ERR_ARG, "bad units / NULL argument");
  if ((rc = upload_opts(ctx, opts))) return rc;
  if (units == 0) return C1_OK;
  if ((rc = ensure_workspace(ctx, units * 2))) return rc;
  C1EncodeLaunch L;
  memset(&L, 0, sizeof L);
  L.channels = 1;
  L.frames = units;
  L.tables = ctx->d_tables;
  L.opts = ctx->d_opts;
  L.side = const_cast<uint8_t *>(side);
  L.alloc = ctx->d_alloc[0];
  L.cand = ctx->d_cand[0];
  L.work_count = ctx->d_work[0];
  L.work_list = ctx->d_work[0] + 4;
  L.sel_list = ctx->d_work[0] + 4 + (size_t)ctx->ws_units * 7;
  c1k_launch_alloc_tap(L, out, ctx->stream);
  HIP_TRY(hipGetLastError());
  return C1_OK;
}

int c1_libm_device(c1_ctx *ctx, int fn, const double *in, double *out, int64_t n) {
  CTX_GUARD(ctx);
  int rc = ctx_bind(ctx);
  if (rc) return rc;
  if (fn < 0 || fn > 4 || n < 0 || (n > 0 && (!in || !out))) return fail(C1_ERR_ARG, "bad fn / n / NULL argument");
  if (fn == 4) c1k_launch_js_log2(in, out, n, ctx->stream);
  else c1k_launch_libm(fn, in, out, n, ctx->stream);
  HIP_TRY(hipGetLastError());
  return C1_OK;
}

int c1_spec_stages_device(c1_ctx *ctx, const float *const *pcm, int channels, int64_t frames, int halo_frames,
                          const c1_encode_options *opts, float *coefs, float *eps, uint8_t *side) {
  CTX_GUARD(ctx);
  int rc = ctx_bind(ctx);
  if (rc) return rc;
  if ((rc = check_channels(channels))) return rc;
  if (frames < 0 || halo_frames < 0 || halo_frames > 2) return fail(C1_ERR_ARG, "bad frames / halo_frames");
  if (!pcm || !opts || !coefs || !eps || !side) return fail(C1_ERR_ARG, "NULL argument");
  const bool sp_long = opts->fixed_block_modes[0] == 0 && opts->fixed_block_modes[1] == 0 && opts->fixed_block_modes[2] == 0;
  const bool sp_short = opts->fixed_block_modes[0] > 0 && opts->fixed_block_modes[1] > 0 && opts->fixed_block_modes[2] > 0;
  if (!sp_long && !sp_short)
    return fail(C1_ERR_ARG, "the speculative analysis covers fixed block modes with all bands long or all bands short");
  if (!ctx->spec_tables_ok) return fail(C1_ERR_STATE, "the installed tables fail the checks the error bound relies on");
  for (int c = 0; c < channels; c++)
    if (!pcm[c] || ((uintptr_t)pcm[c] & 15)) return fail(C1_ERR_ARG, "pcm[%d] must be a 16-byte aligned device pointer", c);
  if ((rc = upload_opts(ctx, opts))) return rc;
  if (frames == 0) return C1_OK;
  C1EncodeLaunch L;
  memset(&L, 0, sizeof L);
  for (int c = 0; c < channels; c++) L.pcm[c] = pcm[c];
  L.channels = channels; L.frames = frames; L.halo_frames = halo_frames;
  L.tables = ctx->d_tables; L.opts = ctx->d_opts;
  L.coefs = coefs; L.eps = eps; L.side = side;
  c1k_launch_analysis_spec(L, sp_short, ctx->stream);
  HIP_TRY(hipGetLastError());
  return C1_OK;
}


int c1_quantize(c1_ctx *ctx, const float *coefficients, int n, int scale_factor_index, int bits_per_sample, int32_t *out) {
  CTX_GUARD(ctx);
  int rc = ctx_bind(ctx);
  if (rc) return rc;
  if (n < 0 || (n > 0 && (!coefficients || !out))) return fail(C1_ERR_ARG, "quantize: bad arguments");
  if (scale_factor_index < 0 || scale_factor_index > 63) return fail(C1_ERR_ARG, "quantize: scaleFactorIndex %d outside SCALE_FACTORS", scale_factor_index);
  if (n == 0) return C1_OK;
  DeviceScratch ds;
  float *dx; int32_t *dq;
  if ((rc = ds.alloc(&dx, (size_t)n)) || (rc = ds.alloc(&dq, (size_t)n))) return rc;
  HIP_TRY(hipMemcpyAsync(dx, coefficients, (size_t)n * sizeof(float), hipMemcpyHostToDevice, ctx->stream));
  c1k_launch_quantize_one(ctx->d_tables, dx, n, scale_factor_index, bits_per_sample, dq, ctx->stream);
  HIP_TRY(hipMemcpyAsync(out, dq, (size_t)n * sizeof(int32_t), hipMemcpyDeviceToHost, ctx->stream));
  HIP_TRY(hipStreamSynchronize(ctx->stream));
  return C1_OK;
}

int c1_dequantize(c1_ctx *ctx, const int32_t *quantized, int n, int scale_factor_index, int bits_per_sample, float *out) {
  CTX_GUARD(ctx);
  int rc = ctx_bind(ctx);
  if (rc) return rc;
  if (n < 0 || (n > 0 && (!quantized || !out))) return fail(C1_ERR_ARG, "dequantize: bad arguments");
  if (scale_factor_index < 0 || scale_factor_index > 63) return fail(C1_ERR_ARG, "dequantize: scaleFactorIndex %d outside SCALE_FACTORS", scale_factor_index);
  if (n == 0) return C1_OK;
  DeviceScratch ds;
  int32_t *dq; float *dx;
  if ((rc = ds.alloc(&dq, (size_t)n)) || (rc = ds.alloc(&dx, (size_t)n))) return rc;
  HIP_TRY(hipMemcpyAsync(dq, quantized, (size_t)n * sizeof(int32_t), hipMemcpyHostToDevice, ctx->stream));
  c1k_launch_dequantize_one(ctx->d_tables, dq, n, scale_factor_index, bits_per_sample, dx, ctx->stream);
  HIP_TRY(hipMemcpyAsync(out, dx, (size_t)n * sizeof(float), hipMemcpyDeviceToHost, ctx->stream));
  HIP_TRY(hipStreamSynchronize(ctx->stream));
  return C1_OK;
}

int c1_fft(c1_ctx *ctx, float *real, float *imag, int n, const double *w) {
  CTX_GUARD(ctx);
  int rc = ctx_bind(ctx);
  if (rc) return rc;
  if (n < 1 || (n & (n - 1)) || n > (1 << 22)) return fail(C1_ERR_ARG, "fft: size must be a power of two <= 2^22, got %d", n);
  if (!real || !imag || (n > 1 && !w)) return fail(C1_ERR_ARG, "fft: NULL argument");
  if (n == 1) return C1_OK;
  int stages = 0;
  while ((1 << stages) < n) stages++;
  DeviceScratch ds;
  float *dr, *di; double *dw, *dtw;
  if ((rc = ds.alloc(&dr, (size_t)n)) || (rc = ds.alloc(&di, (size_t)n)) || (rc = ds.alloc(&dw, (size_t)2 * stages)) || (rc = ds.alloc(&dtw, (size_t)n))) return rc;
  HIP_TRY(hipMemcpyAsync(dr, real, (size_t)n * sizeof(float), hipMemcpyHostToDevice, ctx->stream));
  HIP_TRY(hipMemcpyAsync(di, imag, (size_t)n * sizeof(float), hipMemcpyHostToDevice, ctx->stream));
  HIP_TRY(hipMemcpyAsync(dw, w, (size_t)2 * stages * sizeof(double), hipMemcpyHostToDevice, ctx->stream));
  c1k_launch_fft_reference(dr, di, n, dw, dtw, ctx->stream);
  HIP_TRY(hipMemcpyAsync(real, dr, (size_t)n * sizeof(float), hipMemcpyDeviceToHost, ctx->stream));
  HIP_TRY(hipMemcpyAsync(imag, di, (size_t)n * sizeof(float), hipMemcpyDeviceToHost, ctx->stream));
  HIP_TRY(hipStreamSynchronize(ctx->stream));
  return C1_OK;
}

int c1_qmf_analysis_batch(c1_ctx *ctx, const float *pcm, int64_t frames, int halo_frames, float *bands) {
  CTX_GUARD(ctx);
  int rc = ctx_bind(ctx);
  if (rc) return rc;
  if (frames < 0 || halo_frames < 0 || halo_frames > 2) return fail(C1_ERR_ARG, "qmf analysis: bad frames / halo_frames");
  if (frames == 0) return C1_OK;
  if (!pcm || !bands) return fail(C1_ERR_ARG, "qmf analysis: NULL argument");
  if (frames > (1 << 20)) return fail(C1_ERR_ARG, "qmf analysis: at most 2^20 frames per call");
  DeviceScratch ds;
  float *dp, *db, *dc; uint8_t *dside, *dalloc;
  const size_t total = (size_t)(frames + halo_frames) * 512;
  if ((rc = ds.alloc(&dp, total)) || (rc = ds.alloc(&db, (size_t)frames * 512)) || (rc = ds.alloc(&dc, (size_t)frames * 512)) ||
      (rc = ds.alloc(&dside, (size_t)frames * kSideBytes)) || (rc = ds.alloc(&dalloc, (size_t)frames * kAllocBytes))) return rc;
  HIP_TRY(hipMemcpyAsync(dp, pcm, total * sizeof(float), hipMemcpyHostToDevice, ctx->stream));
  c1_encode_options o;
  c1_default_encode_options(&o);
  o.fixed_block_modes[0] = o.fixed_block_modes[1] = o.fixed_block_modes[2] = 0;
  const float *chan[1] = {dp + (size_t)halo_frames * 512};
  if ((rc = encode_device_impl(ctx, chan, 1, frames, halo_frames, &o, nullptr, db, dc, dside, dalloc))) return rc;
  HIP_TRY(hipMemcpyAsync(bands, db, (size_t)frames * 512 * sizeof(float), hipMemcpyDeviceToHost, ctx->stream));
  HIP_TRY(hipStreamSynchronize(ctx->stream));
  return C1_OK;
}

int c1_mdct_batch(c1_ctx *ctx, const float *bands, int64_t frames, int halo_frames, const int32_t *block_modes, float *coefs,
                  float *bands_windowed) {
  CTX_GUARD(ctx);
  int rc = ctx_bind(ctx);
  if (rc) return rc;
  if (frames < 0 || halo_frames < 0 || halo_frames > 1) return fail(C1_ERR_ARG, "mdct: halo_frames must be 0 or 1");
  if (frames == 0) return C1_OK;
  if (!bands || !block_modes || !coefs) return fail(C1_ERR_ARG, "mdct: NULL argument");
  if (frames > (1 << 20)) return fail(C1_ERR_ARG, "mdct: at most 2^20 frames per call");
  std::vector<uint8_t> modes((size_t)frames);
  std::vector<uint32_t> lists(4 + 2 * (size_t)frames, 0u);
  for (int64_t f = 0; f < frames; f++) {
    const int m0 = block_modes[3 * f] ? 2 : 0, m1 = block_modes[3 * f + 1] ? 2 : 0, m2 = block_modes[3 * f + 2] ? 3 : 0;
    modes[(size_t)f] = (uint8_t)(m0 | (m1 << 2) | (m2 << 4));
    if (modes[(size_t)f] == 0) lists[4 + lists[0]++] = (uint32_t)f;
    else lists[4 + (size_t)frames + lists[1]++] = (uint32_t)f;
  }
  DeviceScratch ds;
  float *db, *dc, *dw = nullptr; uint8_t *dm, *dside; uint32_t *dl;
  if ((rc = ds.alloc(&db, (size_t)(frames + 1) * 512)) || (rc = ds.alloc(&dc, (size_t)frames * 512)) || (rc = ds.alloc(&dm, (size_t)frames)) ||
      (rc = ds.alloc(&dside, (size_t)frames * kSideBytes)) || (rc = ds.alloc(&dl, lists.size()))) return rc;
  if (bands_windowed && (rc = ds.alloc(&dw, (size_t)frames * 512))) return rc;
  if (!halo_frames) HIP_TRY(hipMemsetAsync(db, 0, 512 * sizeof(float), ctx->stream));
  HIP_TRY(hipMemcpyAsync(db + (halo_frames ? 0 : 512), bands, (size_t)(frames + halo_frames) * 512 * sizeof(float), hipMemcpyHostToDevice, ctx->stream));
  HIP_TRY(hipMemcpyAsync(dm, modes.data(), modes.size(), hipMemcpyHostToDevice, ctx->stream));
  HIP_TRY(hipMemcpyAsync(dl, lists.data(), lists.size() * sizeof(uint32_t), hipMemcpyHostToDevice, ctx->stream));
  C1EncodeLaunch L;
  memset(&L, 0, sizeof L);
  L.channels = 1; L.frames = frames; L.halo_frames = halo_frames;
  L.tables = ctx->d_tables; L.opts = ctx->d_opts;
  L.coefs = dc; L.side = dside;
  c1k_launch_mdct_bands(L, db, dm, dl, ctx->stream);
  if (dw) c1k_launch_window_bands(db + 512, dm, frames, ctx->d_tables, dw, ctx->stream);
  HIP_TRY(hipMemcpyAsync(coefs, dc, (size_t)frames * 512 * sizeof(float), hipMemcpyDeviceToHost, ctx->stream));
  if (dw) HIP_TRY(hipMemcpyAsync(bands_windowed, dw, (size_t)frames * 512 * sizeof(float), hipMemcpyDeviceToHost, ctx->stream));
  HIP_TRY(hipStreamSynchronize(ctx->stream));
  HIP_TRY(hipGetLastError());
  return C1_OK;
}


namespace {
constexpr int64_t kMaxStageFrames = (int64_t)1 << 20;

int check_field_domain(const char *what, int64_t units, int channels, int64_t first_frame, const int32_t *nbfu, const int32_t *sfi,
                       const int32_t *wl) {
  auto where = [&](int64_t u) {
    char at[64];
    if (channels == 1) snprintf(at, sizeof at, "frame %lld", (long long)(first_frame + u));
    else snprintf(at, sizeof at, "frame %lld channel %d", (long long)(first_frame + u / channels), (int)(u % channels));
    return std::string(at);
  };
  for (int64_t u = 0; u < units; u++) {
    const int32_t n = nbfu[u];
    if (n < 0 || n > 52) return fail(C1_ERR_ARG, "%s: %s: nBfu %d outside 0..52", what, where(u).c_str(), n);
    for (int b = 0; b < n; b++) {
      const int32_t w = wl[52 * u + b], s = sfi[52 * u + b];
      if (w < 0 || w > 15) return fail(C1_ERR_ARG, "%s: %s BFU %d: word length index %d outside 0..15", what, where(u).c_str(), b, w);
      if (s < 0 || s > 63) return fail(C1_ERR_ARG, "%s: %s BFU %d: scale factor index %d outside 0..63", what, where(u).c_str(), b, s);
    }
  }
  return C1_OK;
}

constexpr int64_t kFieldInts = 1 + 3 + 52 + 52 + 512;
C1FieldPtrs field_layout(const int32_t *base, int64_t units) {
  return C1FieldPtrs{base, base + units, base + 4 * units, base + 56 * units, base + 108 * units};
}
C1FieldPtrs field_unit(const C1FieldPtrs &p, int64_t u) {
  return C1FieldPtrs{p.nbfu + u, p.modes + 3 * u, p.sfi + 52 * u, p.wl + 52 * u, p.q + 512 * u};
}
}

int c1_unpack_units(c1_ctx *ctx, const uint8_t *units, int64_t frames, int32_t *nbfu, int32_t *block_modes, int32_t *sfi,
                    int32_t *wl, int32_t *quantized) {
  CTX_GUARD(ctx);
  int rc = ctx_bind(ctx);
  if (rc) return rc;
  if (frames < 0 || frames > kMaxStageFrames) return fail(C1_ERR_ARG, "unpack: frames must be 0 .. 2^20, got %lld", (long long)frames);
  if (frames == 0) return C1_OK;
  if (!units || !nbfu || !block_modes || !sfi || !wl || !quantized) return fail(C1_ERR_ARG, "unpack: NULL argument");
  DeviceScratch ds;
  uint8_t *du; int32_t *dn, *dm, *ds_, *dw, *dq;
  const size_t n = (size_t)frames;
  if ((rc = ds.alloc(&du, n * C1_UNIT_BYTES)) || (rc = ds.alloc(&dn, n)) || (rc = ds.alloc(&dm, 3 * n)) || (rc = ds.alloc(&ds_, 52 * n)) ||
      (rc = ds.alloc(&dw, 52 * n)) || (rc = ds.alloc(&dq, 512 * n))) return rc;
  HIP_TRY(hipMemcpyAsync(du, units, n * C1_UNIT_BYTES, hipMemcpyHostToDevice, ctx->stream));
  c1k_launch_unpack_units(du, frames, dn, dm, ds_, dw, dq, ctx->stream);
  HIP_TRY(hipGetLastError());
  HIP_TRY(hipMemcpyAsync(nbfu, dn, n * sizeof(int32_t), hipMemcpyDeviceToHost, ctx->stream));
  HIP_TRY(hipMemcpyAsync(block_modes, dm, 3 * n * sizeof(int32_t), hipMemcpyDeviceToHost, ctx->stream));
  HIP_TRY(hipMemcpyAsync(sfi, ds_, 52 * n * sizeof(int32_t), hipMemcpyDeviceToHost, ctx->stream));
  HIP_TRY(hipMemcpyAsync(wl, dw, 52 * n * sizeof(int32_t), hipMemcpyDeviceToHost, ctx->stream));
  HIP_TRY(hipMemcpyAsync(quantized, dq, 512 * n * sizeof(int32_t), hipMemcpyDeviceToHost, ctx->stream));
  HIP_TRY(hipStreamSynchronize(ctx->stream));
  return C1_OK;
}

int c1_dequantize_frames(c1_ctx *ctx, int64_t frames, const int32_t *nbfu, const int32_t *block_modes, const int32_t *sfi,
                         const int32_t *wl, const int32_t *quantized, float *coefs) {
  CTX_GUARD(ctx);
  int rc = ctx_bind(ctx);
  if (rc) return rc;
  if (frames < 0 || frames > kMaxStageFrames) return fail(C1_ERR_ARG, "dequantize frames: frames must be 0 .. 2^20, got %lld", (long long)frames);
  if (frames == 0) return C1_OK;
  if (!nbfu || !block_modes || !sfi || !wl || !quantized || !coefs) return fail(C1_ERR_ARG, "dequantize frames: NULL argument");
  if ((rc = check_field_domain("dequantize frames", frames, 1, 0, nbfu, sfi, wl))) return rc;
  DeviceScratch ds;
  int32_t *dn, *dm, *ds_, *dw, *dq; float *dc;
  const size_t n = (size_t)frames;
  if ((rc = ds.alloc(&dn, n)) || (rc = ds.alloc(&dm, 3 * n)) || (rc = ds.alloc(&ds_, 52 * n)) || (rc = ds.alloc(&dw, 52 * n)) ||
      (rc = ds.alloc(&dq, 512 * n)) || (rc = ds.alloc(&dc, 512 * n))) return rc;
  HIP_TRY(hipMemcpyAsync(dn, nbfu, n * sizeof(int32_t), hipMemcpyHostToDevice, ctx->stream));
  HIP_TRY(hipMemcpyAsync(dm, block_modes, 3 * n * sizeof(int32_t), hipMemcpyHostToDevice, ctx->stream));
  HIP_TRY(hipMemcpyAsync(ds_, sfi, 52 * n * sizeof(int32_t), hipMemcpyHostToDevice, ctx->stream));
  HIP_TRY(hipMemcpyAsync(dw, wl, 52 * n * sizeof(int32_t), hipMemcpyHostToDevice, ctx->stream));
  HIP_TRY(hipMemcpyAsync(dq, quantized, 512 * n * sizeof(int32_t), hipMemcpyHostToDevice, ctx->stream));
  c1k_launch_dequantize_frames(ctx->d_tables, dn, dm, ds_, dw, dq, frames, dc, ctx->stream);
  HIP_TRY(hipGetLastError());
  HIP_TRY(hipMemcpyAsync(coefs, dc, 512 * n * sizeof(float), hipMemcpyDeviceToHost, ctx->stream));
  HIP_TRY(hipStreamSynchronize(ctx->stream));
  return C1_OK;
}

int c1_imdct_batch(c1_ctx *ctx, const float *coefs, int64_t frames, int halo_frames, const int32_t *block_modes, float *bands) {
  CTX_GUARD(ctx);
  int rc = ctx_bind(ctx);
  if (rc) return rc;
  if (halo_frames < 0 || halo_frames > 1) return fail(C1_ERR_ARG, "imdct: halo_frames must be 0 or 1, got %d", halo_frames);
  if (frames < 0 || frames > kMaxStageFrames) return fail(C1_ERR_ARG, "imdct: frames must be 0 .. 2^20, got %lld", (long long)frames);
  if (frames == 0) return C1_OK;
  if (!coefs || !block_modes || !bands) return fail(C1_ERR_ARG, "imdct: NULL argument");
  DeviceScratch ds;
  float *dc, *db; int32_t *dm;
  const size_t n = (size_t)frames, all = (size_t)(frames + halo_frames);
  if ((rc = ds.alloc(&dc, 512 * all)) || (rc = ds.alloc(&dm, 3 * all)) || (rc = ds.alloc(&db, 512 * n))) return rc;
  HIP_TRY(hipMemcpyAsync(dc, coefs, 512 * all * sizeof(float), hipMemcpyHostToDevice, ctx->stream));
  HIP_TRY(hipMemcpyAsync(dm, block_modes, 3 * all * sizeof(int32_t), hipMemcpyHostToDevice, ctx->stream));
  c1k_launch_imdct_frames(ctx->d_tables, dc, dm, frames, halo_frames, db, ctx->stream);
  HIP_TRY(hipGetLastError());
  HIP_TRY(hipMemcpyAsync(bands, db, 512 * n * sizeof(float), hipMemcpyDeviceToHost, ctx->stream));
  HIP_TRY(hipStreamSynchronize(ctx->stream));
  return C1_OK;
}

int c1_qmf_synthesis_batch(c1_ctx *ctx, const float *bands, int64_t frames, int halo_frames, float *pcm) {
  CTX_GUARD(ctx);
  int rc = ctx_bind(ctx);
  if (rc) return rc;
  if (halo_frames < 0 || halo_frames > 1) return fail(C1_ERR_ARG, "qmf synthesis: halo_frames must be 0 or 1, got %d", halo_frames);
  if (frames < 0 || frames > kMaxStageFrames) return fail(C1_ERR_ARG, "qmf synthesis: frames must be 0 .. 2^20, got %lld", (long long)frames);
  if (frames == 0) return C1_OK;
  if (!bands || !pcm) return fail(C1_ERR_ARG, "qmf synthesis: NULL argument");
  DeviceScratch ds;
  float *db, *dp;
  const size_t n = (size_t)frames, all = (size_t)(frames + halo_frames);
  if ((rc = ds.alloc(&db, 512 * all)) || (rc = ds.alloc(&dp, 512 * n))) return rc;
  HIP_TRY(hipMemcpyAsync(db, bands, 512 * all * sizeof(float), hipMemcpyHostToDevice, ctx->stream));
  c1k_launch_qmf_synthesis_frames(ctx->d_tables, db, frames, halo_frames, dp, ctx->stream);
  HIP_TRY(hipGetLastError());
  HIP_TRY(hipMemcpyAsync(pcm, dp, 512 * n * sizeof(float), hipMemcpyDeviceToHost, ctx->stream));
  HIP_TRY(hipStreamSynchronize(ctx->stream));
  return C1_OK;
}


int c1_select_block_modes(c1_ctx *ctx, const float *bands, int64_t frames, int halo_frames, double threshold, int32_t *block_modes) {
  CTX_GUARD(ctx);
  int rc = ctx_bind(ctx);
  if (rc) return rc;
  if (halo_frames < 0 || halo_frames > 1) return fail(C1_ERR_ARG, "select block modes: halo_frames must be 0 or 1, got %d", halo_frames);
  if (frames < 0 || frames > kMaxStageFrames) return fail(C1_ERR_ARG, "select block modes: frames must be 0 .. 2^20, got %lld", (long long)frames);
  if (frames == 0) return C1_OK;
  if (!bands || !block_modes) return fail(C1_ERR_ARG, "select block modes: NULL argument");
  DeviceScratch ds;
  float *db, *dm; int32_t *dmodes;
  const size_t n = (size_t)frames, all = (size_t)(frames + halo_frames);
  if ((rc = ds.alloc(&db, 512 * all)) || (rc = ds.alloc(&dm, 256 * all)) || (rc = ds.alloc(&dmodes, 3 * n))) return rc;
  HIP_TRY(hipMemcpyAsync(db, bands, 512 * all * sizeof(float), hipMemcpyHostToDevice, ctx->stream));
  c1k_launch_block_modes_from_bands(ctx->d_tables, db, frames, halo_frames, threshold, dm, dmodes, ctx->stream);
  HIP_TRY(hipGetLastError());
  HIP_TRY(hipMemcpyAsync(block_modes, dmodes, 3 * n * sizeof(int32_t), hipMemcpyDeviceToHost, ctx->stream));
  HIP_TRY(hipStreamSynchronize(ctx->stream));
  return C1_OK;
}

int c1_quantize_frames(c1_ctx *ctx, const float *coefs, int64_t frames, const int32_t *block_modes, const c1_encode_options *opts,
                       int32_t *nbfu, int32_t *sfi, int32_t *wl, int32_t *quantized) {
  CTX_GUARD(ctx);
  int rc = ctx_bind(ctx);
  if (rc) return rc;
  if (!opts) return fail(C1_ERR_ARG, "quantize frames: options are NULL");
  if (frames < 0 || frames > kMaxStageFrames) return fail(C1_ERR_ARG, "quantize frames: frames must be 0 .. 2^20, got %lld", (long long)frames);
  if (frames == 0) return C1_OK;
  if (!coefs || !block_modes || !nbfu || !sfi || !wl || !quantized) return fail(C1_ERR_ARG, "quantize frames: NULL argument");
  c1_encode_options o = *opts;
  o.transient_threshold = 1.0;
  o.fixed_block_modes[0] = o.fixed_block_modes[1] = o.fixed_block_modes[2] = -1;
  if ((rc = upload_opts(ctx, &o))) return rc;
  DeviceScratch ds;
  float *dc; int32_t *dmodes, *dn, *ds_, *dw, *dq; uint8_t *dside, *dalloc, *dcand; uint32_t *dwork;
  const size_t n = (size_t)frames;
  if ((rc = ds.alloc(&dc, 512 * n)) || (rc = ds.alloc(&dmodes, 3 * n)) || (rc = ds.alloc(&dside, kSideBytes * n)) ||
      (rc = ds.alloc(&dalloc, kAllocBytes * n)) || (rc = ds.alloc(&dcand, (size_t)kCandidateBytes * n)) ||
      (rc = ds.alloc(&dwork, 4 + 8 * n)) || (rc = ds.alloc(&dn, n)) || (rc = ds.alloc(&ds_, 52 * n)) || (rc = ds.alloc(&dw, 52 * n)) ||
      (rc = ds.alloc(&dq, 512 * n))) return rc;
  HIP_TRY(hipMemcpyAsync(dc, coefs, 512 * n * sizeof(float), hipMemcpyHostToDevice, ctx->stream));
  HIP_TRY(hipMemcpyAsync(dmodes, block_modes, 3 * n * sizeof(int32_t), hipMemcpyHostToDevice, ctx->stream));
  c1k_launch_stage_scale_factors(ctx->d_tables, dc, dmodes, frames, dside, ctx->stream);
  C1EncodeLaunch L;
  memset(&L, 0, sizeof L);
  L.channels = 1;
  L.frames = frames;
  L.tables = ctx->d_tables;
  L.opts = ctx->d_opts;
  L.side = dside;
  L.alloc = dalloc;
  L.cand = dcand;
// ... 3456 lines not shown
```

carta1_amd/csrc/c1_internal.h:

```cpp
#pragma once

#include <hip/hip_runtime.h>
#include <stdint.h>
#include <stdlib.h>

#include "../../include/carta1_hip.h"

struct C1DevTables {
  double tap_e[24];
  double tap_o[24];
  double window[32];
  double mdct_fwd64[32];
  double mdct_fwd256[128];
  double mdct_fwd512[256];
  double mdct_inv64[32];
  double mdct_inv256[128];
  double mdct_inv512[256];
  double fft_tw[256][2];
  double scale_factors[64];
  double norm[64 * 16];
  double log1p10;
  uint32_t sf_m1, sf_m2;
  int32_t sf_fast;
  int32_t dq_fast;
  int32_t dq_step;
  double inv_range[16];
  float tap32[24];
  float tap_pair[26][2];
  float win32[32];
  float pre32_64[16][2];
  float pre32_256[64][2];
  float pre32_512[128][2];
  float r4b[4][3][2];
  float r4c[16][3][2];
  float r2d[64][2];
  float norm32[64 * 16];
  float inv32_64[16][2], inv32_256[64][2], inv32_512[128][2];
  float tw32[256][2];
  float spec_cz[4], spec_cw[4], spec_cl[4];
  float spec_cz_short[4], spec_cw_short[4], spec_cl_short[4];
  float spec_eabs;
  float det_ck[4];
  float det_eabs;
  int32_t spec_ok;
};

struct C1DevEncOpts {
  double biased[64];
  double threshold;
  int32_t modes[3];
  int32_t pad_;
  uint16_t rank[64 * 16];
  int32_t rank_affine, rank_a, rank_b, rank_c, rank_off;
  float la_slope, la_off;
  int32_t alloc_no_tonal;
  uint32_t rank_step0, rank_step;
  int32_t dist_tables;
  alignas(16) double dist[8][64][2];
};
constexpr int kDistSizes[8] = {4, 6, 7, 8, 9, 10, 12, 20};

constexpr int kRunFrames = 16;
constexpr int kRunFramesDecode = 64;
constexpr int kRunFramesLong = 64;
constexpr int kSideBytes = 64;
constexpr int kAllocBytes = 32;
constexpr int kCandidateBytes = 8 * 8 + 8 * 32 + 8 * 8;
constexpr int kCandLbOffset = 8 * 8 + 8 * 32;
constexpr int kEpsFloats = 4;
constexpr uint32_t kEpsFlagSfOpen = 1u;
constexpr uint32_t kEpsFlagExact = 2u;
constexpr int kSpecCheckFrames = 16;

struct C1EncodeLaunch {
  const float *pcm[C1_MAX_CHANNELS];
  int channels;
  int64_t frames;
  int halo_frames;
  const C1DevTables *tables;
  const C1DevEncOpts *opts;
  float *coefs;
  uint8_t *side;
  uint8_t *alloc;
  uint8_t *cand;
  uint32_t *work_list;
  uint32_t *work_count;
  uint32_t *sel_list;
  float *bands;
  float *mags;
  float *mag_bounds;
  uint8_t *units;
  float *eps;
  uint32_t *redo_list;
  uint32_t *redo_count;
  uint32_t *realloc_list;
  uint32_t *realloc_count;
  uint32_t *reana_list;
  uint32_t *reana_count;
  uint32_t *defer_list;
  unsigned long long *open_masks;
  int list_zero_eps;
  float spec_defer;
  const uint32_t *unit_list;
  const uint32_t *unit_count;
  int list_runs;
  int run_frames;
  int spread_bits;
};

struct C1DecodeLaunch {
  const uint8_t *units;
  int channels;
  int64_t frames;
  int halo_units;
  const C1DevTables *tables;
  float *pcm[C1_MAX_CHANNELS];
  int run_frames;
};

struct C1MeasurePcmLaunch {
  const uint8_t *units;
  int channels;
  int64_t frames;
  int halo_units;
  int halo_frames;
  const C1DevTables *tables;
  const float *pcm[C1_MAX_CHANNELS];
  double *noise, *signal, *totals;
  int run_frames;
};

struct C1FieldPtrs {
  const int32_t *nbfu, *modes, *sfi, *wl, *q;
};
struct C1DecodeFieldsLaunch {
  C1FieldPtrs cur;
  C1FieldPtrs prev;
  int channels;
  int64_t frames;
  int halo_frames;
  const C1DevTables *tables;
  float *pcm[C1_MAX_CHANNELS];
  int run_frames;
  int binary32;
};

struct C1EncStateLaunch {
  const float *pcm;
  int64_t pcm_stride;
  const float *in;
  float *out;
  int64_t n;
  const C1DevTables *tables;
  const C1DevEncOpts *opts;
  float *coefs;
  uint8_t *side;
  int detect;
  int state_only;
  const uint32_t *src_rows, *in_rows, *out_rows;
  int in_broadcast, keep_mags;
};
struct C1DecStateLaunch {
  C1FieldPtrs fields;
  const float *in;
  float *out;
  float *pcm;
  int64_t pcm_stride;
  int64_t n;
  const C1DevTables *tables;
  const uint32_t *dst_rows, *in_rows, *out_rows;
  int in_broadcast;
  int binary32;
};

struct C1SignalStartsLaunch {
  const float *pcm;
  const float *in;
  float *out;
  int64_t n;
  const C1DevTables *tables;
  const C1DevEncOpts *opts;
  float *coefs;
  uint8_t *side;
  int detect, state_only;
  const uint32_t *src_rows, *in_rows, *out_rows, *counts, *first_rows;
  int64_t row_base;
  int in_broadcast, keep_mags, count_all;
  const uint8_t *modes;
};
struct C1ScatterRowsLaunch {
  const uint32_t *dst_rows;
  int64_t n;
  const uint32_t *units_src; uint32_t *units_dst;
  const uint8_t *taken_src; uint8_t *taken_dst;
  const uint32_t *shifts_src; uint32_t *shifts_dst;
  const uint32_t *distortion_src; uint32_t *distortion_dst;
  const uint32_t *energy_src; uint32_t *energy_dst;
  const uint32_t *weights_src; uint32_t *weights_dst;
};

constexpr int kRunDefault = 64;
inline int c1k_pick_run(int64_t frames, int channels, int slots) {
  static const int forced = getenv("C1_RUN_FRAMES") ? atoi(getenv("C1_RUN_FRAMES")) : 0;
  (void)slots;
  if (forced > 0) return forced < 4 ? 4 : forced;
  const int64_t units = frames * channels;
  if (units >= (int64_t)kRunDefault * 2048) return kRunDefault;
  const int run = (int)((units + 2047) / 2048);
  return run < 4 ? 4 : run;
}
template <class Kernel>
inline int c1k_wave_slots(Kernel kernel) {
  int per_cu = 0, cus = 0, dev = 0;
  if (hipOccupancyMaxActiveBlocksPerMultiprocessor(&per_cu, kernel, 64, 0) != hipSuccess || per_cu <= 0) per_cu = 8;
  if (hipGetDevice(&dev) != hipSuccess || hipDeviceGetAttribute(&cus, hipDeviceAttributeMultiprocessorCount, dev) != hipSuccess || cus <= 0) cus = 256;
  return per_cu * cus;
}

void c1k_launch_analysis(const C1EncodeLaunch &L, bool detect, hipStream_t stream);
void c1k_launch_analysis_long(const C1EncodeLaunch &L, hipStream_t stream);
void c1k_launch_analysis_spec(const C1EncodeLaunch &L, bool all_short, hipStream_t stream);
constexpr int kFeatureWsDoubles = 20;
void c1k_launch_detect(const C1EncodeLaunch &L, float *bands_ws, double *feat_ws, uint8_t *modes_ws, uint32_t *lists_ws,
                       bool speculative, double *score_tap, hipStream_t stream);
void c1k_launch_modes_front(const C1EncodeLaunch &L, const uint8_t *given_modes, float *bands_ws, uint8_t *modes_ws, uint32_t *lists_ws,
                            hipStream_t stream);
void c1k_launch_mdct_bands(const C1EncodeLaunch &L, const float *bands_ws, const uint8_t *modes_ws, const uint32_t *lists_ws, hipStream_t stream);
void c1k_launch_unpack_units(const uint8_t *units, int64_t frames, int32_t *nbfu, int32_t *modes, int32_t *sfi, int32_t *wl,
                             int32_t *q, hipStream_t stream);
void c1k_launch_dequantize_frames(const C1DevTables *tables, const int32_t *nbfu, const int32_t *modes, const int32_t *sfi,
                                  const int32_t *wl, const int32_t *q, int64_t frames, float *coefs, hipStream_t stream);
void c1k_launch_imdct_frames(const C1DevTables *tables, const float *coefs, const int32_t *modes, int64_t frames, int halo,
                             float *bands, hipStream_t stream);
void c1k_launch_qmf_synthesis_frames(const C1DevTables *tables, const float *bands, int64_t frames, int halo, float *pcm,
                                     hipStream_t stream);
void c1k_launch_block_modes_from_bands(const C1DevTables *tables, const float *bands, int64_t frames, int halo, double threshold,
                                       float *mags, int32_t *modes, hipStream_t stream);
void c1k_launch_stage_mode_lists(const int32_t *modes, int64_t frames, uint8_t *mode_bytes, uint32_t *lists, hipStream_t stream);
void c1k_launch_stage_scale_factors(const C1DevTables *tables, const float *coefs, const int32_t *modes, int64_t frames, uint8_t *side,
                                    hipStream_t stream);
void c1k_launch_stage_fields(const C1DevTables *tables, const float *coefs, const int32_t *modes, const uint8_t *side,
                             const uint8_t *alloc, int64_t frames, int32_t *nbfu, int32_t *sfi, int32_t *wl, int32_t *q,
                             hipStream_t stream);
void c1k_launch_pack_units(const int32_t *nbfu, const int32_t *modes, const int32_t *sfi, const int32_t *wl, const int32_t *q,
                           int64_t frames, uint8_t *units, hipStream_t stream);
void c1k_launch_quantize_one(const C1DevTables *tables, const float *x, int n, int sfi, int bits, int32_t *out, hipStream_t stream);
void c1k_launch_dequantize_one(const C1DevTables *tables, const int32_t *q, int n, int sfi, int bits, float *out, hipStream_t stream);
void c1k_launch_fft_reference(float *real, float *imag, int n, const double *w, double *twiddle_scratch , hipStream_t stream);
void c1k_launch_window_bands(const float *bands, const uint8_t *modes, int64_t units, const C1DevTables *tables, float *out, hipStream_t stream);
void c1k_launch_js_log2(const double *in, double *out, int64_t n, hipStream_t stream);
void c1k_launch_find_scale_factors(const double *values, const int64_t *offsets, const int64_t *counts, int64_t problems, int32_t *out,
                                   hipStream_t stream);
void c1k_launch_perform_fft(const double *samples, const int64_t *offsets, int64_t problems, int n, const double *w, double *tw,
                            float *re, float *im, float *mag, hipStream_t stream);
void c1k_launch_detect_transients(const double *cur, const int64_t *cur_off, const double *prev, const int64_t *prev_off,
                                  const uint8_t *has_prev, const double *thresholds, int64_t problems, const C1DevTables *tables,
                                  uint8_t *transient, double *scores, hipStream_t stream);
void c1k_launch_allocate_bits(const double *data, const int64_t *bfu_off, const int32_t *bfu_len, const int32_t *bfu_sizes,
                              const int32_t *max_bfus, int64_t problems, const double *bsf, int32_t *count, int32_t *wl, int32_t *sfi,
                              uint8_t *fallback, hipStream_t stream);
void c1k_launch_detect_spec_tap(const C1EncodeLaunch &L, float *bands_ws, double *feat_ws, hipStream_t stream);
void c1k_launch_libm(int fn, const double *in, double *out, int64_t n, hipStream_t stream);
void c1k_launch_log2f_error(uint32_t first, uint64_t count, unsigned long long *out, hipStream_t stream);
void c1k_launch_allocate(const C1EncodeLaunch &L, hipStream_t stream);
void c1k_launch_alloc_tap(const C1EncodeLaunch &L, double *out, hipStream_t stream);
void c1k_launch_allocate_palette(const C1EncodeLaunch &L, const C1DevEncOpts *palette, int n, const uint8_t *index, uint32_t *counts,
                                 uint32_t *lists, int64_t stride, hipStream_t stream);
void c1k_launch_choose_bias(const C1EncodeLaunch &L, const uint8_t *trial, int64_t trial_stride, int n_palette, bool all_long,
                            uint8_t *choice, double *distortion, double *energy, hipStream_t stream);
void c1k_launch_const_mode_lists(int byte, int64_t units, uint8_t *modes_ws, uint32_t *lists_ws, hipStream_t stream);
void c1k_launch_compose_side(const uint8_t *side_long, const uint8_t *side_short, int64_t units, int byte, uint8_t *out, hipStream_t stream);
void c1k_launch_choose_modes(const C1EncodeLaunch &L, const float *coefs_short, const uint8_t *side_short, const uint8_t *trial,
                             int64_t trial_stride, const uint8_t *cand, int n_cand, bool finalize, uint8_t *choice, uint8_t *modes_out,
                             double *distortion, double *energy, hipStream_t stream);
void c1k_launch_measured_modes(const C1EncodeLaunch &L, const float *coefs_short, const uint8_t *side_short, const uint8_t *trial,
                               int64_t trial_stride, const uint8_t *cand, int n_cand, const int8_t *sf_offsets, int n_offsets, bool finalize,
                               uint8_t *choice, uint8_t *modes_out, uint8_t *taken, int8_t *shifts, double *distortion, double *energy,
                               hipStream_t stream);
void c1k_launch_measured_modes_wide(const C1EncodeLaunch &L, const float *coefs_short, const uint8_t *side_short, const uint8_t *trial,
                                    int64_t trial_stride, const uint8_t *cand, int n_cand, const int8_t *sf_offsets, int n_offsets,
                                    bool finalize, uint8_t *choice, uint8_t *modes_out, uint8_t *taken, int8_t *shifts, double *distortion,
                                    double *energy, hipStream_t stream);
constexpr int64_t kMeasuredModesWideUnits = 8192;
void c1k_launch_measured_alloc(const C1EncodeLaunch &L, bool all_long, bool finalize, uint8_t *taken, double *distortion, double *energy,
                               hipStream_t stream);
void c1k_launch_measured_sf(const C1EncodeLaunch &L, bool all_long, bool finalize, const int8_t *sf_offsets, int n_offsets, uint8_t *taken,
                            int8_t *shifts, double *distortion, double *energy, hipStream_t stream);
void c1k_launch_measured_masked(const C1EncodeLaunch &L, bool all_long, bool finalize, const int8_t *sf_offsets, int n_offsets,
                                const double *mask, bool has_spread, uint8_t *taken, int8_t *shifts, double *distortion, double *energy,
                                double *weights, hipStream_t stream);
void c1k_launch_measured_wide(const C1EncodeLaunch &L, bool all_long, bool finalize, const int8_t *sf_offsets, int n_offsets,
                              const double *mask, bool has_spread, uint8_t *taken, int8_t *shifts, double *distortion, double *energy,
                              double *weights, hipStream_t stream);
constexpr int64_t kMeasuredWideUnits = 8192;
void c1k_launch_unit_mode_bytes(const uint8_t *units, int64_t n, uint8_t *modes, hipStream_t stream);
void c1k_launch_measure_units(const C1DevTables *tables, const float *coefs, const uint8_t *units, int64_t n, const double *mask,
                              bool has_spread, double *noise, double *signal, double *totals, double *weights, hipStream_t stream);
void c1k_launch_measure_pcm(const C1MeasurePcmLaunch &L, hipStream_t stream);
void c1k_launch_pack(const C1EncodeLaunch &L, bool all_long, hipStream_t stream);
void c1k_launch_pack_spec(const C1EncodeLaunch &L, bool all_long, hipStream_t stream);
void c1k_launch_spec_totals(unsigned long long *totals, uint64_t units, const uint32_t *counts, int kind, hipStream_t stream);
void c1k_launch_defer_compact(const C1EncodeLaunch &L, uint32_t *list, uint32_t *counts, hipStream_t stream);
void c1k_launch_open_compact(const C1EncodeLaunch &L, uint32_t *list, uint32_t *count, hipStream_t stream);
void c1k_launch_decode(const C1DecodeLaunch &L, bool binary32, hipStream_t stream);
void c1k_launch_decode_fields(const C1DecodeFieldsLaunch &L, hipStream_t stream);
void c1k_launch_encode_from_states(const C1EncStateLaunch &L, hipStream_t stream);
void c1k_launch_decode_from_states(const C1DecStateLaunch &L, hipStream_t stream);
void c1k_launch_encode_rows(const C1EncStateLaunch &L, hipStream_t stream);
void c1k_launch_decode_rows(const C1DecStateLaunch &L, hipStream_t stream);
void c1k_launch_copy_rows(uint32_t *dst, const uint32_t *dst_rows, const uint32_t *src, const uint32_t *src_rows, int src_broadcast,
                          int64_t n, int dwords, hipStream_t stream);
void c1k_launch_signal_starts(const C1SignalStartsLaunch &L, hipStream_t stream);
void c1k_launch_scatter_signal_rows(const C1ScatterRowsLaunch &L, hipStream_t stream);
void c1k_launch_state_mags(const C1DevTables *tables, const float *bands, int64_t rows, float *states, hipStream_t stream);
void c1k_launch_generate_white(const uint32_t *frame_states, int64_t frames, float *pcm, int kind_mask, double amp, hipStream_t stream);
void c1k_launch_generate_pink(const uint32_t *segment_states, int64_t frames, float *pcm, int kind_mask, hipStream_t stream);
void c1k_launch_generate_sines(int64_t frames, float *pcm, int kind_mask, uint32_t seed, hipStream_t stream);
void c1k_launch_pcm_from_int(const void *src, int bits, int channels, int64_t n, float *const *pcm, hipStream_t stream);
void c1k_launch_pcm_to_int16(const float *const *pcm, int channels, int64_t n, int16_t *dst, hipStream_t stream);
```

carta1_amd/csrc/c1_k_spec.hip:

```cpp
#include "c1_device.h"

namespace {

constexpr int kR2 = 840;
constexpr int kW2 = kR2 + 320;
constexpr int kMemFloats = kW2 + 304;
constexpr int kW1Tail = 768;
constexpr int kIn2 = 1;
struct alignas(16) SpecLds {
  alignas(16) float mem[kMemFloats];
  alignas(16) float pre2[76];
  alignas(4) uint8_t sfi[64];
};
typedef uint4 SpecGeo;
static_assert(sizeof(SpecLds) % 16 == 0 && (kW2 + 48) % 4 == 0, "16-byte groups of every wave's buffers stay aligned");
__host__ __device__ constexpr int in01(int b, int i) { return kR2 + 64 * (i >> 5) + 32 * b + ((i & 31) ^ b); }

constexpr int kSpecWaves = 4;
constexpr int kSpecTabBase = (int)offsetof(C1DevTables, win32);
constexpr int kSpecTabFloats = ((int)offsetof(C1DevTables, r2d) + (int)sizeof(((C1DevTables *)nullptr)->r2d) - kSpecTabBase) / 4;
static_assert(offsetof(C1DevTables, pre32_64) > offsetof(C1DevTables, win32) && offsetof(C1DevTables, r2d) > offsetof(C1DevTables, r4c) &&
              offsetof(C1DevTables, norm32) == offsetof(C1DevTables, r2d) + sizeof(((C1DevTables *)nullptr)->r2d), "win32 .. r2d are one contiguous block");
constexpr int kSpecLdsBytes = kSpecWaves * (int)sizeof(SpecLds) + 64 * (int)sizeof(SpecGeo) + kSpecTabFloats * 4 + 28 * 16 + 64 * 8;
static_assert((kSpecLdsBytes + 1279) / 1280 <= 25, "speculative analysis: 5 workgroups of 4 waves per CU = at most 25 LDS blocks of 1 280 bytes each");
constexpr int kE2 = 0, kH2 = 288, kE0 = kR2, kH0 = kR2 + 160, kE1 = kR2 + 288, kH1 = kR2 + 448;

__device__ __forceinline__ int w1_phys(int v) { return __mul24(12, v >> 3) + (v & 7); }

template <int D, int NP, int OFF>
__device__ __forceinline__ void qmf_core_f32(const v2f (&Wr)[NP], TablesPtr T, float (&lo)[D], float (&hi)[D]) {
  static_assert(OFF + D - 1 + 23 < NP, "the window registers cover every tap");
  v2f tp[26];
#pragma unroll
  for (int j = 0; j < 26; j++) tp[j] = *reinterpret_cast<const __attribute__((address_space(4))) v2f *>(T->tap_pair[j]);
  const float e12 = T->tap32[12];
#pragma unroll
  for (int d = 0; d < D; d++) {
    v2f p1 = Wr[OFF + d + 23] * tp[0];
#pragma unroll
    for (int j = 1; j <= 10; j++) p1 = pk_fma(Wr[OFF + d + 23 - j], tp[j], p1);
    v2f p2 = Wr[OFF + d] * tp[23];
#pragma unroll
    for (int j = 22; j >= 13; j--) p2 = pk_fma(Wr[OFF + d + 23 - j], tp[j], p2);
    p1 = pk_fma(Wr[OFF + d + 12], tp[24], p1);
    p2 = pk_fma(Wr[OFF + d + 11], tp[25], p2);
    const v2f sum = p1 + p2;
    const float ev = __builtin_fmaf(e12, Wr[OFF + d + 11].y, sum.y);
    const float od = __builtin_fmaf(e12, Wr[OFF + d + 12].x, sum.x);
    lo[d] = ev + od;
    hi[d] = ev - od;
  }
}

struct SpecBase {
  int ia3, ic0;
  int q2;
  int ib, id;
  int pt0;
  int za, zb, zc, zd;
  int g;
  int e0, e1;
  int po0;
  int d1;
  bool band0, band2, use_lo, use_hi;
};
__device__ __forceinline__ SpecBase spec_base(int lane) {
  SpecBase B;
  const int band = lane < 16 ? 0 : (lane < 32 ? 1 : 2);
  const int g = lane - (band == 0 ? 0 : (band == 1 ? 16 : 32));
  const int n4 = band == 2 ? 128 : 64, q = n4 / 4;
  const int r = bitrev(g, band == 2 ? 5 : 4);
  auto in = [band](int i) { return band == 2 ? kIn2 + i : in01(band, i); };
  const int tab_base = band == 2 ? (int)offsetof(C1DevTables, pre32_512) : (int)offsetof(C1DevTables, pre32_256);
  B.ia3 = in(3 * n4 - 1 - 2 * r) - 192;
  B.ic0 = in(n4 + 2 * r);
  B.q2 = 2 * q;
  B.use_lo = r < 8;
  B.use_hi = r >= q - 8;
  B.ib = B.use_lo ? in(3 * n4 + 2 * r) : in(2 * r + 2 * q);
  B.id = B.use_lo ? in(n4 - 1 - 2 * r) : in(14 * q - 1 - 2 * r);
  B.pt0 = tab_base + 8 * r;
  const int pbase = band == 0 ? 0 : (band == 1 ? 64 : 128);
  B.za = zslot(pbase + 4 * g);
  B.zb = zslot(pbase + 16 * (g >> 2) + (g & 3));
  B.zc = zslot(pbase + 64 * (g >> 4) + (g & 15));
  B.zd = zslot(128 + (g & 31));
  B.g = g;
  const int cbase = band == 0 ? 0 : (band == 1 ? 128 : 256), n2 = 2 * n4;
  B.e0 = cbase + 2 * g;
  B.e1 = cbase + n2 - 1 - 2 * g;
  B.po0 = tab_base + 8 * g;
  B.d1 = band == 2 ? 64 : 16;
  B.band0 = band == 0;
  B.band2 = band == 2;
  return B;
}

__device__ __forceinline__ v2f pk_mul_yy_nyx(v2f x, v2f w) {
  v2f r;
  asm("v_pk_mul_f32 %0, %1, %2 op_sel:[1,1] op_sel_hi:[1,0] neg_lo:[0,1]" : "=v"(r) : "v"(x), "v"(w));
  return r;
}
__device__ __forceinline__ v2f pk_mul_yx_yny(v2f x, v2f t) {
  v2f r;
  asm("v_pk_mul_f32 %0, %1, %2 op_sel:[1,1] op_sel_hi:[0,1] neg_hi:[0,1]" : "=v"(r) : "v"(x), "v"(t));
  return r;
}
__device__ __forceinline__ v2f cmul32n(v2f x, v2f w) {
  const v2f t = pk_mul_yy_nyx(x, w);
  return pk_fma(x.xx, w, t);
}
__device__ __forceinline__ v2f lds_f2(const v2f *p) { return *(const volatile __attribute__((address_space(3))) v2f *)p; }
__device__ __forceinline__ void radix4_round(v2f (&x)[4], v2f wa, v2f wb, v2f wab) {
  const v2f y1 = cmul32n(x[1], wa), y2 = cmul32n(x[2], wb), y3 = cmul32n(x[3], wab);
  const v2f t0 = x[0] + y1, t1 = x[0] - y1, t2 = y2 + y3, t3 = y2 - y3;
  x[0] = t0 + t2;
  x[2] = t0 - t2;
  x[1] = pk_fma(t3.yx, PMN, t1);
  x[3] = pk_fma(t3.yx, PNM, t1);
}

__device__ __attribute__((noinline)) bool spec_should_defer(const uint8_t *sfi, int lane, float e0, float e1, float e2,
                                                  const C1DevEncOpts *O, float threshold) {
  const int s = lane < 52 ? (int)sfi[lane] : 0;
  const float size = (float)(lane < 4 ? 8 : lane < 8 ? 4 : lane < 12 ? 8 : lane < 24 ? 6 : lane < 28 ? 7 : lane < 32 ? 9 : lane < 36 ? 10 : lane < 44 ? 12 : 20);
  const bool act = s > 0;
  const float sf = (float)s;
  const float l = __builtin_fmaf(sf, 0.33333334f, -21.0f);
  const float lb = __builtin_fmaf(O->la_slope, sf, O->la_off);
  const float eb = lane >= 36 ? e2 : (lane >= 20 ? e1 : e0);
  const float sz = act ? size : 0.0f;
  constexpr float kBudget = 1136.0f;
  const float n_all = wave_sum(sz);
  if (!(n_all > 0.0f)) return false;
  float Lw = (wave_sum(sz * lb) - kBudget) * __builtin_amdgcn_rcpf(n_all);
  {
    const float d = lb - Lw;
    const float bits = fminf(fmaxf(d, 0.0f), 16.0f);
    const float spend = wave_sum(sz * bits);
    const float n = wave_sum((d > 0.0f && d < 16.0f) ? sz : 0.0f);
    if (n > 0.0f) Lw += (spend - kBudget) * __builtin_amdgcn_rcpf(n);
  }
  const float bits = fminf(fmaxf(lb - Lw, 0.0f), 16.0f);
  const float inv_sf = __builtin_amdgcn_exp2f(-l);
  const float pm = (act && bits >= 1.0f) ? size * eb * inv_sf * __builtin_amdgcn_exp2f(bits) : 0.0f;
  const float ps = act ? fminf(1.0f, 9.7f * eb * inv_sf) : 0.0f;
  const float P = wave_sum(pm + ps);
  return !(P <= threshold);
}

__device__ __forceinline__ uint32_t spread_block(uint32_t b, uint32_t n, int bits) {
  if (bits < 4) return b;
  const uint32_t mask = (1u << bits) - 1u;
  const int sh = (bits >> 1) + 1;
  uint32_t x = b;
  do {
    x = (x * 0x9E3779B1u) & mask;
    x ^= x >> sh;
    x = (x * 0x85EBCA6Bu) & mask;
    x ^= x >> sh;
  } while (x >= n);
  return x;
}

template <bool SHORT>
__global__ __launch_bounds__(C1_WAVE * kSpecWaves, 5) void k_analysis_spec(C1EncodeLaunch L) {
  __shared__ SpecLds Sw[kSpecWaves];
  __shared__ alignas(16) float tab[kSpecTabFloats];
  __shared__ alignas(16) float tail_w[28][4];
  __shared__ alignas(8) float out_w[64][2];
  __shared__ alignas(16) SpecGeo geo[64];
  const int wave = __builtin_amdgcn_readfirstlane((int)(threadIdx.x >> 6));
  SpecLds &S = Sw[wave];
  const int lane0 = threadIdx.x & 63;
  int lane = lane0;
  {
    const float *src = reinterpret_cast<const float *>(reinterpret_cast<const char *>(L.tables) + kSpecTabBase);
    for (int i = threadIdx.x; i < kSpecTabFloats; i += C1_WAVE * kSpecWaves) tab[i] = src[i];
    if (threadIdx.x < 28 * 4) {
      const int idx = threadIdx.x >> 2, j = threadIdx.x & 3;
      const bool input = idx < 10;
      const int k = 4 * (input ? idx - 1 : idx - 10) - 1 + j;
      tail_w[idx][j] = (k >= 0 && k < 32) ? src[input ? 31 - k : k] : 1.0f;
    }
    if (threadIdx.x >= 128 && threadIdx.x < 128 + 64) {
      const int l = threadIdx.x - 128, k = 2 * (l - 48);
      out_w[l][0] = l >= 48 ? src[31 - k] : 1.0f;
      out_w[l][1] = l >= 48 ? src[30 - k] : 1.0f;
    }
    if (!SHORT && threadIdx.x >= 192) {
      const int l = threadIdx.x - 192;
      const SpecBase G = spec_base(l);
      const SfLong F = sf_long_geometry(l);
      const int po = G.po0 - kSpecTabBase, u = G.band0 ? 8 * G.d1 : -8 * G.d1, t = G.band0 ? 256 : -256;
      geo[l] = make_uint4((uint32_t)(4 * (G.band0 ? G.e0 : G.e1)) | ((uint32_t)(4 * (G.band0 ? G.e1 : G.e0)) << 16),
                          (uint32_t)po | ((uint32_t)(po + 8 * G.d1) << 16), ((uint32_t)u & 0xffffu) | ((uint32_t)t << 16),
                          (uint32_t)(F.src & ~3) | ((uint32_t)F.b << 9) | (F.wide ? 1u << 15 : 0u) | (F.store ? 1u << 16 : 0u));
    }
  }
  __syncthreads();
  const float *win = tab;
  auto table_f2 = [&](int , int byte_offset) -> v2f {
    return lds_f2(reinterpret_cast<const v2f *>(reinterpret_cast<const char *>(tab) + (byte_offset - kSpecTabBase)));
  };
  const uint32_t n_slots = (uint32_t)((L.frames + L.run_frames - 1) / L.run_frames) * (uint32_t)L.channels;
  const uint32_t group = L.spread_bits > 0 ? spread_block(blockIdx.x, gridDim.x, L.spread_bits) : blockIdx.x;
  const uint32_t slot = group * kSpecWaves + (uint32_t)wave;
  if (slot >= n_slots) return;
  const int ch = (int)(slot % (uint32_t)L.channels);
  const int64_t f0 = (int64_t)(slot / (uint32_t)L.channels) * L.run_frames;
  const float *__restrict__ pcm = L.pcm[ch];
  float *mem = S.mem;

  for (int i = lane; i < 72; i += 64) mem[kW1Tail + i] = 0.0f;
  if (lane < 48) mem[kW2 + 256 + lane] = 0.0f;
  float ov0a = 0.0f, ov0b = 0.0f, ov1a = 0.0f, ov1b = 0.0f;
  for (int i = lane; i < 76; i += 64) S.pre2[i] = 0.0f;
  if (lane < 16) reinterpret_cast<uint32_t *>(S.sfi)[lane] = 0u;
  SpecBase B0 = spec_base(lane0);
  const SfLong SFL0 = SHORT ? sf_geometry(lane0, 2, 2, 3) : sf_long_geometry(lane0);
  if (SHORT && lane == 0) S.sfi[52] = (uint8_t)((L.opts->modes[0] & 3) | ((L.opts->modes[1] & 3) << 2) | ((L.opts->modes[2] & 3) << 4));
  const int s_band = lane0 < 16 ? 0 : (lane0 < 32 ? 1 : 2);
  const int s_g = lane0 - (s_band == 0 ? 0 : (s_band == 1 ? 16 : 32));
  const int s_blk = s_g >> 2, s_r2 = 2 * bitrev(s_g & 3, 2);
  const int s_eb0 = (s_band == 0 ? kE0 : (s_band == 1 ? kE1 : kE2)) + 32 * s_blk;
  const int s_hb0 = (s_band == 0 ? kH0 : (s_band == 1 ? kH1 : kH2)) + 32 * s_blk;
  const int s_c0 = (s_band == 0 ? 0 : (s_band == 1 ? 128 : 256)) + 32 * s_blk + 2 * (s_g & 3);
  constexpr int RT = 0;
  float p_prev = 0.0f, q_prev = 0.0f;
  wave_fence();

  const int64_t f_end = (f0 + L.run_frames < L.frames) ? f0 + L.run_frames : L.frames;
  int64_t f_first = f0 - 1;
  if (f_first < -(int64_t)L.halo_frames) f_first = -(int64_t)L.halo_frames;
  if (f_first > f0) f_first = f0;
  typedef float v4f __attribute__((ext_vector_type(4)));
  v4f pre_a, pre_b;
  {
    const v4f *p4 = reinterpret_cast<const v4f *>(pcm + f_first * 512);
    pre_a = p4[lane0]; pre_b = p4[64 + lane0];
    asm volatile("" : "+v"(pre_a), "+v"(pre_b));
  }
  uint32_t deferred_from = 0xffffffffu;
  unsigned long long open_bits = 0ull;
  for (int64_t f = f_first; f < f_end; ++f) {
    const bool emit = (f >= f0);
    TablesPtr T = tables_for_this_frame(L.tables);
    lane = lane_for_this_frame(lane0);
    if constexpr (!SHORT) {
      asm volatile("" : "+v"(B0.ia3), "+v"(B0.ic0), "+v"(B0.q2), "+v"(B0.ib), "+v"(B0.id), "+v"(B0.pt0));
      asm volatile("" : "+v"(B0.za), "+v"(B0.zb), "+v"(B0.zc), "+v"(B0.zd), "+v"(B0.g));
    }

    float P;
    {
      const v4f a = pre_a, b = pre_b;
      {
        const int p = w1_phys(lane);
        float dl = 0.0f;
        if (lane < 48) dl = mem[kW1Tail + p];
        const int s = __mul24(6, lane) - 2 * (lane & 1);
        *reinterpret_cast<v4f *>(&mem[72 + s]) = a;
        *reinterpret_cast<v4f *>(&mem[72 + 384 + s]) = b;
        if (lane < 48) mem[p] = dl;
      }
      v2f p2 = V2(a.x, a.y) * V2(a.x, a.y);
      p2 = pk_fma(V2(a.z, a.w), V2(a.z, a.w), p2);
      p2 = pk_fma(V2(b.x, b.y), V2(b.x, b.y), p2);
      p2 = pk_fma(V2(b.z, b.w), V2(b.z, b.w), p2);
      const float p = p2.x + p2.y;
      P = wave_sum(p);
    }
    wave_fence();
    float Q;
    {
      float lo[4], hi[4];
      if (own_block()) {
        v2f W[28];
        const float4 *src = reinterpret_cast<const float4 *>(mem + __mul24(12, lane));
#pragma unroll
        for (int k = 0; k < 14; k++) {
          v4f t = *reinterpret_cast<const v4f *>(&src[3 * (k >> 1) + (k & 1)]);
          if (k == 0) asm volatile("" : "+v"(t));
          W[2 * k] = V2(t.x, t.y); W[2 * k + 1] = V2(t.z, t.w);
        }
        qmf_core_f32<4, 28, 1>(W, T, lo, hi);
      } else { for (int d = 0; d < 4; d++) { lo[d] = mem[lane + d]; hi[d] = 1.0f; } }
      {
        const v4f *p4 = reinterpret_cast<const v4f *>(pcm + ((f + 1 < f_end) ? f + 1 : f) * 512);
        pre_a = p4[lane]; pre_b = p4[64 + lane];
      }
      if (lane < 48) mem[kW2 + lane] = mem[kW2 + 256 + lane];
      *reinterpret_cast<float4 *>(&mem[kW2 + 48 + 4 * lane]) = make_float4(lo[0], lo[1], lo[2], lo[3]);
      v2f q2 = V2(lo[0], lo[1]) * V2(lo[0], lo[1]);
      q2 = pk_fma(V2(lo[2], lo[3]), V2(lo[2], lo[3]), q2);
      const float q = q2.x + q2.y;
      Q = wave_sum(q);
      if constexpr (!SHORT) {
      if (emit && lane < 36) *reinterpret_cast<float2 *>(&mem[kIn2 + 111 + 2 * lane]) = *reinterpret_cast<const float2 *>(&S.pre2[2 * lane]);
      {
        const int wi = min(max(lane - 45, 0), 10);
        const float4 wh = *reinterpret_cast<const float4 *>(tail_w[wi]);
        const v2f h01 = V2(hi[0], hi[1]) * V2(wh.x, wh.y), h23 = V2(hi[2], hi[3]) * V2(wh.z, wh.w);
        if (emit && lane <= 54) *reinterpret_cast<float4 *>(&mem[kIn2 + 183 + 4 * lane]) = make_float4(h01.x, h01.y, h23.x, h23.y);
      }
      if (lane >= 46) {
        const float4 wl = *reinterpret_cast<const float4 *>(tail_w[10 + lane - 46]);
        const v2f l01 = V2(hi[0], hi[1]) * V2(wl.x, wl.y), l23 = V2(hi[2], hi[3]) * V2(wl.z, wl.w);
        *reinterpret_cast<float4 *>(&S.pre2[4 * (lane - 46)]) = make_float4(l01.x, l01.y, l23.x, l23.y);
      }
      } else {
        if (emit) {
          if (lane < 32) mem[kE2 + lane] = S.pre2[1 + lane];
          if (lane < 39) {
            const float x = S.pre2[33 + lane];
            mem[kE2 + 32 + lane] = win[lane & 31] * x;
            mem[kH2 + lane] = x * win[31 - (lane & 31)];
          }
        }
#pragma unroll
        for (int d = 0; d < 4; d++) {
          const int pos = 39 + 4 * lane + d;
          const float x = hi[d];
          if (pos < 256) {
            const float e = win[pos & 31] * x;
            if (emit) { mem[kE2 + 32 + pos] = e; mem[kH2 + pos] = x * win[31 - (pos & 31)]; }
            if (pos >= 224) S.pre2[1 + pos - 224] = e;
          } else S.pre2[33 + pos - 256] = x;
        }
      }
    }
    wave_fence();
    {
      float lo[2], hi[2];
      if (own_block()) {
        v2f W[26];
        const float4 *src = reinterpret_cast<const float4 *>(mem + kW2 + 4 * lane);
#pragma unroll
        for (int k = 0; k < 13; k++) {
          v4f t = *reinterpret_cast<const v4f *>(&src[k]);
          if (k == 0) asm volatile("" : "+v"(t));
          W[2 * k] = V2(t.x, t.y); W[2 * k + 1] = V2(t.z, t.w);
        }
        qmf_core_f32<2, 26, 1>(W, T, lo, hi);
      } else { for (int d = 0; d < 2; d++) { lo[d] = mem[lane + d]; hi[d] = 1.0f; } }
      if constexpr (!SHORT) {
      const int u = lane + 40, at = kR2 + 2 * (u + (u & ~15));
      {
        const v2f wh = *reinterpret_cast<const v2f *>(out_w[lane]);
        const v2f o0 = V2(lo[0], lo[1]) * wh, o1 = V2(hi[1], hi[0]) * wh.yx;
        if (emit) {
          *reinterpret_cast<v2f *>(&mem[at]) = o0;
          *reinterpret_cast<v2f *>(&mem[at + 32]) = o1;
        }
      }
      if (lane >= 48) {
        const int k = 2 * (lane - 48);
        const float wl0 = win[k], wl1 = win[k + 1];
        if (emit) {
          const int uo = lane - 24, ato = kR2 + 2 * (uo + (uo & ~15));
          *reinterpret_cast<float2 *>(&mem[ato]) = make_float2(ov0a, ov0b);
          *reinterpret_cast<float2 *>(&mem[ato + 32]) = make_float2(ov1b, ov1a);
        }
        ov0a = wl0 * lo[0]; ov0b = wl1 * lo[1];
        ov1a = wl0 * hi[0]; ov1b = wl1 * hi[1];
      }
      } else {
        const int k = (2 * lane) & 31;
        const float wl0 = win[k], wl1 = win[k + 1], wh0 = win[31 - k], wh1 = win[30 - k];
        const float e00 = wl0 * lo[0], e01 = wl1 * lo[1], e10 = wl0 * hi[0], e11 = wl1 * hi[1];
        if (emit) {
          if (lane >= 48) {
            *reinterpret_cast<float2 *>(&mem[kE0 + 2 * (lane - 48)]) = make_float2(ov0a, ov0b);
            *reinterpret_cast<float2 *>(&mem[kE1 + 2 * (lane - 48)]) = make_float2(ov1a, ov1b);
          }
          *reinterpret_cast<float2 *>(&mem[kE0 + 32 + 2 * lane]) = make_float2(e00, e01);
          *reinterpret_cast<float2 *>(&mem[kE1 + 32 + 2 * lane]) = make_float2(e10, e11);
          *reinterpret_cast<float2 *>(&mem[kH0 + 2 * lane]) = make_float2(lo[0] * wh0, lo[1] * wh1);
          *reinterpret_cast<float2 *>(&mem[kH1 + 2 * lane]) = make_float2(hi[0] * wh0, hi[1] * wh1);
        }
        if (lane >= 48) { ov0a = e00; ov0b = e01; ov1a = e10; ov1b = e11; }
      }
    }
    const float W = __builtin_amdgcn_sqrtf(P + p_prev), Lw = __builtin_amdgcn_sqrtf(Q + q_prev);
    p_prev = P; q_prev = Q;
    wave_fence();
    if (!emit) {
      asm volatile("" : "+v"(pre_a), "+v"(pre_b));
      continue;
    }

    v2f x[4];
    float zrow;
    uint32_t gw_sf = 0;
    if constexpr (!SHORT) {
    const SpecBase &B = B0;
    {
      const int qb = 4 * B.q2;
      const v2f t0 = table_f2(RT, B.pt0), t1 = table_f2(RT, B.pt0 + 2 * qb);
      const v2f t2 = table_f2(RT, B.pt0 + qb), t3 = table_f2(RT, B.pt0 + __mul24(3, qb));
      const float a0 = mem[B.ia3 + 192], c0 = mem[B.ic0];
      const float a1 = mem[B.ia3 + 64], c1 = mem[B.ic0 + 128];
      const float a2 = mem[B.ia3 + 128], c2 = mem[B.ic0 + 64];
      const float a3 = mem[B.ia3], c3 = mem[B.ic0 + 192];
      const float bb = mem[B.ib], dd = mem[B.id];
      const float b0 = B.use_lo ? bb : 0.0f, d0 = B.use_lo ? dd : 0.0f;
      const float b3 = B.use_hi ? bb : 0.0f, d3 = B.use_hi ? dd : 0.0f;
      const v2f rm0 = pk_fma(V2(b0, d0), PMN, V2(a0, c0)), rm3 = pk_fma(V2(b3, d3), PNM, V2(a3, c3));
      const v2f rm1 = V2(a1, c1), rm2 = V2(a2, c2);
      auto twiddle = [](v2f rm, v2f t) { const v2f u = pk_mul_yx_yny(rm, t); return pk_fma(rm, t.xx, u); };
      x[0] = twiddle(rm0, t0); x[1] = twiddle(rm1, t1); x[2] = twiddle(rm2, t2); x[3] = twiddle(rm3, t3);
      v2f en2 = x[0] * x[0];
#pragma unroll
      for (int j = 1; j < 4; j++) en2 = pk_fma(x[j], x[j], en2);
      zrow = row_allreduce(en2.x + en2.y);
      const v2f u0 = x[0] + x[1], u1 = x[0] - x[1], u2 = x[2] + x[3], u3 = x[2] - x[3];
      x[0] = u0 + u2;
      x[2] = u0 - u2;
      x[1] = pk_fma(u3.yx, PMN, u1);
      x[3] = pk_fma(u3.yx, PNM, u1);
    }
    v2f *z = reinterpret_cast<v2f *>(mem);
    {
      float4 *dst = reinterpret_cast<float4 *>(z + B.za);
      dst[0] = make_float4(x[0].x, x[0].y, x[1].x, x[1].y);
      dst[1] = make_float4(x[2].x, x[2].y, x[3].x, x[3].y);
    }
    const int twb = (int)offsetof(C1DevTables, r4b) + 24 * (B.g & 3);
    const v2f wBa = table_f2(RT, twb), wBb = table_f2(RT, twb + 8), wBc = table_f2(RT, twb + 16);
    wave_fence();
    {
      v2f *p = z + B.zb;
      x[0] = lds_f2(p); x[1] = lds_f2(p + 4); x[2] = lds_f2(p + 8); x[3] = lds_f2(p + 12);
      radix4_round(x, wBa, wBb, wBc);
      p[0] = x[0]; p[4] = x[1]; p[8] = x[2]; p[12] = x[3];
    }
    const int twc = (int)offsetof(C1DevTables, r4c) + 24 * (B.g & 15), twd = (int)offsetof(C1DevTables, r2d) + 8 * (B.g & 31);
    const v2f wCa = table_f2(RT, twc), wCb = table_f2(RT, twc + 8), wCc = table_f2(RT, twc + 16);
    const v2f wDa = table_f2(RT, twd), wDb = table_f2(RT, twd + 256);
    wave_fence();
    {
      v2f *p = z + B.zc;
      x[0] = lds_f2(p); x[1] = lds_f2(p + 20); x[2] = lds_f2(p + 40); x[3] = lds_f2(p + 60);
      radix4_round(x, wCa, wCb, wCc);
      if (B.band2) { p[0] = x[0]; p[20] = x[1]; p[40] = x[2]; p[60] = x[3]; }
    }
    const SpecGeo gw = geo[lane];
    const int po0 = kSpecTabBase + (int)(gw.y & 0xffffu), po1 = kSpecTabBase + (int)(gw.y >> 16);
    const v2f p0 = table_f2(RT, po0), p1 = table_f2(RT, po1);
    const v2f p2 = table_f2(RT, po0 + 256), p3 = table_f2(RT, po1 + 256);
    wave_fence();
    if (B.band2) {
      const v2f *p = z + B.zd;
      x[0] = lds_f2(p); x[1] = lds_f2(p + 80); x[2] = lds_f2(p + 40); x[3] = lds_f2(p + 120);
      const v2f y1 = cmul32n(x[1], wDa), y3 = cmul32n(x[3], wDb);
      const v2f e0 = x[0], e2 = x[2];
      x[0] = e0 + y1; x[1] = e0 - y1; x[2] = e2 + y3; x[3] = e2 - y3;
    }
    char *coefw = reinterpret_cast<char *>(mem + kR2);
    const int cf = (int)(gw.x & 0xffffu), cs = (int)(gw.x >> 16);
    const int su = (int)(gw.z << 16) >> 16, st = (int)gw.z >> 16, sut = su + st;
#pragma unroll
    for (int j = 0; j < 4; j++) {
      const v2f t = j == 0 ? p0 : (j == 1 ? p1 : (j == 2 ? p2 : p3));
      const int step = j == 0 ? 0 : (j == 1 ? su : (j == 2 ? st : sut));
      const v2f u = pk_mul_yx_yny(x[j], t);
      const v2f o = pk_fma(x[j], t.xx, u);
      *reinterpret_cast<float *>(coefw + (cf + step)) = -o.x;
      *reinterpret_cast<float *>(coefw + (cs - step)) = o.y;
    }
    gw_sf = gw.w;
    wave_fence();

    }
    float *coef = mem + kR2;
    if constexpr (SHORT) {
    int eb = s_eb0, hb = s_hb0, r2 = s_r2;
    asm volatile("" : "+v"(eb), "+v"(hb), "+v"(r2));
    {
      const int pt = (int)offsetof(C1DevTables, pre32_64) + 4 * r2;
      const v2f t0 = table_f2(RT, pt), t1 = table_f2(RT, pt + 64), t2 = table_f2(RT, pt + 32), t3 = table_f2(RT, pt + 96);
      const float a0 = mem[hb + 15 - r2], b0 = mem[hb + 16 + r2], c0 = mem[eb + 16 + r2], d0 = mem[eb + 15 - r2];
      const float a2 = mem[hb + 7 - r2], b2 = mem[hb + 24 + r2], c2 = mem[eb + 24 + r2], d2 = mem[eb + 7 - r2];
      const float a1 = mem[eb + 31 - r2], b1 = mem[eb + r2], c1 = mem[hb + r2], d1 = mem[hb + 31 - r2];
      const float a3 = mem[eb + 23 - r2], b3 = mem[eb + 8 + r2], c3 = mem[hb + 8 + r2], d3 = mem[hb + 23 - r2];
      const v2f rm0 = pk_fma(V2(b0, d0), PMN, V2(a0, c0)), rm2 = pk_fma(V2(b2, d2), PMN, V2(a2, c2));
      const v2f rm1 = pk_fma(V2(b1, d1), PNM, V2(a1, c1)), rm3 = pk_fma(V2(b3, d3), PNM, V2(a3, c3));
      auto twiddle = [](v2f rm, v2f t) { const v2f u = rm.yx * (t.yy * PMN); return pk_fma(rm, t.xx, u); };
      x[0] = twiddle(rm0, t0); x[1] = twiddle(rm1, t1); x[2] = twiddle(rm2, t2); x[3] = twiddle(rm3, t3);
      v2f en2 = x[0] * x[0];
#pragma unroll
      for (int j = 1; j < 4; j++) en2 = pk_fma(x[j], x[j], en2);
      float en = en2.x + en2.y;
      en += dpp_read<0xB1>(en);
      en += dpp_read<0x4E>(en);
      en = fmaxf(en, dpp_read<0x141>(en));
      zrow = fmaxf(en, dpp_read<0x140>(en));
      const v2f u0 = x[0] + x[1], u1 = x[0] - x[1], u2 = x[2] + x[3], u3 = x[2] - x[3];
      x[0] = u0 + u2;
      x[2] = u0 - u2;
      x[1] = pk_fma(u3.yx, PMN, u1);
      x[3] = pk_fma(u3.yx, PNM, u1);
    }
    {
      v2f *z = reinterpret_cast<v2f *>(mem);
      int za = B0.za, zb = B0.zb, g3 = s_g & 3;
      asm volatile("" : "+v"(za), "+v"(zb), "+v"(g3));
      const int twb = (int)offsetof(C1DevTables, r4b) + 24 * g3;
      const v2f wBa = table_f2(RT, twb), wBb = table_f2(RT, twb + 8), wBc = table_f2(RT, twb + 16);
      const int po = (int)offsetof(C1DevTables, pre32_64) + 8 * g3;
      const v2f p0 = table_f2(RT, po), p1 = table_f2(RT, po + 32), p2 = table_f2(RT, po + 64), p3 = table_f2(RT, po + 96);
      wave_fence();
      float4 *dst = reinterpret_cast<float4 *>(z + za);
      dst[0] = make_float4(x[0].x, x[0].y, x[1].x, x[1].y);
      dst[1] = make_float4(x[2].x, x[2].y, x[3].x, x[3].y);
      wave_fence();
      const v2f *p = z + zb;
      x[0] = p[0]; x[1] = p[4]; x[2] = p[8]; x[3] = p[12];
      radix4_round(x, wBa, wBb, wBc);
      wave_fence();
      float *coefw = mem + kR2;
      int c0i = s_c0;
      asm volatile("" : "+v"(c0i));
      const bool band0 = B0.band0;
#pragma unroll
      for (int j = 0; j < 4; j++) {
        const v2f t = j == 0 ? p0 : (j == 1 ? p1 : (j == 2 ? p2 : p3));
        const int e0 = c0i + 8 * j, e1 = (c0i | 31) - ((c0i & 31) + 8 * j);
        const v2f u = x[j].yx * (t.yy * PMN);
        const v2f o = pk_fma(x[j], t.xx, u);
        coefw[band0 ? e0 : e1] = -o.x;
        coefw[band0 ? e1 : e0] = o.y;
      }
    }
    wave_fence();

    }
    const int64_t unit = f * L.channels + ch;
    asm volatile("" : "+v"(pre_a), "+v"(pre_b));
    {
      v4f *dst = reinterpret_cast<v4f *>(L.coefs + (unit << 9));
      const v4f *src = reinterpret_cast<const v4f *>(coef);
      const int lq = lane_for_this_frame(lane0);
      __builtin_nontemporal_store(src[lq], &dst[lq]);
      __builtin_nontemporal_store(src[64 + lq], &dst[64 + lq]);
    }
    const float Z0 = __builtin_amdgcn_sqrtf(lane_value(zrow, 0)), Z1 = __builtin_amdgcn_sqrtf(lane_value(zrow, 16));
    const float Z2 = __builtin_amdgcn_sqrtf(SHORT ? fmaxf(lane_value(zrow, 32), lane_value(zrow, 48)) : lane_value(zrow, 32) + lane_value(zrow, 48));
    const float eabs = T->spec_eabs;
    const float cz0 = SHORT ? T->spec_cz_short[0] : T->spec_cz[0], cz1 = SHORT ? T->spec_cz_short[1] : T->spec_cz[1], cz2 = SHORT ? T->spec_cz_short[2] : T->spec_cz[2];
    const float cw0 = SHORT ? T->spec_cw_short[0] : T->spec_cw[0], cw1 = SHORT ? T->spec_cw_short[1] : T->spec_cw[1], cw2 = SHORT ? T->spec_cw_short[2] : T->spec_cw[2];
    const float cl0 = SHORT ? T->spec_cl_short[0] : T->spec_cl[0], cl1 = SHORT ? T->spec_cl_short[1] : T->spec_cl[1], cl2 = SHORT ? T->spec_cl_short[2] : T->spec_cl[2];
    const float e0 = __builtin_fmaf(cz0, Z0, __builtin_fmaf(cw0, W, __builtin_fmaf(cl0, Lw, eabs)));
    const float e1 = __builtin_fmaf(cz1, Z1, __builtin_fmaf(cw1, W, __builtin_fmaf(cl1, Lw, eabs)));
    const float e2 = __builtin_fmaf(cz2, Z2, __builtin_fmaf(cw2, W, __builtin_fmaf(cl2, Lw, eabs)));
    bool unstable;
    {
      SfLong SFL = SFL0;
      float mx = 0.0f;
      if constexpr (SHORT) {
        asm volatile("" : "+v"(SFL.src), "+v"(SFL.cnt));
        const float *src = coef + SFL.src;
#pragma unroll
        for (int j = 0; j < 12; j++) mx = fmaxf(mx, fabsf(src[j < SFL.cnt ? j : SFL.cnt - 1]));
      } else {
        const uint32_t sw = gw_sf;
        SFL.b = (int)((sw >> 9) & 63u);
        SFL.wide = ((sw >> 15) & 1u) != 0u;
        SFL.store = ((sw >> 16) & 1u) != 0u;
        const float4 *grp = reinterpret_cast<const float4 *>(coef + (sw & 0x1ffu));
        mx = sf_scan_long_groups(grp[0], grp[1], grp[2]);
      }
      const float other = __int_as_float(__builtin_amdgcn_update_dpp(0, __float_as_int(mx), 0xB1, 0xf, 0xf, false));
      mx = fmaxf(mx, SFL.wide ? other : 0.0f);
      const float e = SFL.b >= 36 ? e2 : (SFL.b >= 20 ? e1 : e0);
      const float lo = fmaxf((mx - e) * 0.99999976f, 0.0f), hi = (mx + e) * 1.00000024f;
      const int s_lo = scale_factor_index_fast(lo, T->sf_m1, T->sf_m2), s_hi = scale_factor_index_fast(hi, T->sf_m1, T->sf_m2);
      if (SFL.store) S.sfi[SFL.b] = (uint8_t)s_lo;
      unstable = lane < 60 && !(s_lo == s_hi && e < __builtin_huge_valf());
    }
    const bool any_unstable = __builtin_amdgcn_ballot_w64(unstable) != 0;
    wave_fence();
    if (L.defer_list != nullptr && (((int)(f - f0)) & (kSpecCheckFrames - 1)) == 0) {
      if (spec_should_defer(S.sfi, lane, e0, e1, e2, L.opts, L.spec_defer)) { deferred_from = (uint32_t)unit; break; }
    }
    if (any_unstable) open_bits |= 1ull << (int)((f - f0) & 63);
    if (lane < 16) reinterpret_cast<uint32_t *>(L.side + unit * kSideBytes)[lane] = reinterpret_cast<const uint32_t *>(S.sfi)[lane];
    if (lane == 0) *reinterpret_cast<float4 *>(L.eps + unit * kEpsFloats) = make_float4(e0, e1, e2, __int_as_float(any_unstable ? 1 : 0));
    wave_fence();
  }
  if (L.defer_list != nullptr && lane0 == 0) L.defer_list[slot] = deferred_from;
  if (L.open_masks != nullptr && lane0 == 0) L.open_masks[slot] = open_bits;
}

__global__ __launch_bounds__(256) void k_defer_compact(const uint32_t *__restrict__ slots, uint32_t n_slots, uint32_t *__restrict__ list, uint32_t *__restrict__ counts,
                                                        int channels, int run_frames, uint32_t frames) {
  const uint32_t i = blockIdx.x * 256u + threadIdx.x;
  const uint32_t u = i < n_slots ? slots[i] : 0xffffffffu;
  const bool on = u != 0xffffffffu;
  uint32_t covered = 0;
  if (on) {
    const uint32_t f = u / (uint32_t)channels;
    uint32_t end = (f / (uint32_t)run_frames + 1u) * (uint32_t)run_frames;
    if (end > frames) end = frames;
    covered = end - f;
  }
  const uint64_t mask = __builtin_amdgcn_ballot_w64(on);
  if (mask == 0) return;
  int cov = (int)covered;
  cov = wave_inclusive_scan(cov);
  const int lane = threadIdx.x & 63;
  uint32_t at = 0;
  if (lane == 63) {
    at = atomicAdd(counts, (uint32_t)__popcll(mask));
    atomicAdd(counts + 1, (uint32_t)cov);
  }
  at = (uint32_t)__builtin_amdgcn_readlane((int)at, 63);
  if (on) list[at + __popcll(mask & ((1ull << lane) - 1ull))] = u;
}

__global__ __launch_bounds__(256) void k_open_compact(const unsigned long long *__restrict__ masks, uint32_t n_slots, uint32_t *__restrict__ list,
                                                       uint32_t *__restrict__ count, int channels, int run_frames) {
  const uint32_t i = blockIdx.x * 256u + threadIdx.x;
  unsigned long long m = i < n_slots ? masks[i] : 0ull;
  const int mine = __popcll(m);
  if (__builtin_amdgcn_ballot_w64(mine != 0) == 0) return;
  const int scan = wave_inclusive_scan(mine);
  const int lane = threadIdx.x & 63;
  uint32_t at = 0;
  if (lane == 63) at = atomicAdd(count, (uint32_t)scan);
  at = (uint32_t)__builtin_amdgcn_readlane((int)at, 63) + (uint32_t)(scan - mine);
  const uint32_t run = i / (uint32_t)channels, ch = i % (uint32_t)channels;
  while (m != 0ull) {
    const int k = __ffsll((long long)m) - 1;
    m &= m - 1ull;
    list[at++] = (run * (uint32_t)run_frames + (uint32_t)k) * (uint32_t)channels + ch;
  }
}

__global__ void k_spec_totals(unsigned long long *totals, unsigned long long units, const uint32_t *counts, int kind) {
  if (kind == 0) {
    const unsigned long long deferred = counts[4];
    totals[0] += units - deferred;
    totals[1] += counts[2] + counts[5];
    totals[2] += deferred;
    totals[3] += counts[0] - counts[2];
    totals[6] += deferred;
  } else if (kind == 1) {
    totals[2] += units;
    totals[3] += counts[0];
  } else {
    totals[4] += units;
    totals[5] += counts[0];
  }
}

}

void c1k_launch_spec_totals(unsigned long long *totals, uint64_t units, const uint32_t *counts, int kind, hipStream_t stream) {
  hipLaunchKernelGGL(k_spec_totals, dim3(1), dim3(1), 0, stream, totals, (unsigned long long)units, counts, kind);
}
void c1k_launch_open_compact(const C1EncodeLaunch &L, uint32_t *list, uint32_t *count, hipStream_t stream) {
  const int run = c1k_pick_run(L.frames, L.channels, 0);
  const int64_t slots = (L.frames + run - 1) / run * L.channels;
  hipLaunchKernelGGL(k_open_compact, dim3((unsigned)((slots + 255) / 256)), dim3(256), 0, stream, (const unsigned long long *)L.open_masks, (uint32_t)slots, list, count,
                     L.channels, run);
}
void c1k_launch_defer_compact(const C1EncodeLaunch &L, uint32_t *list, uint32_t *counts, hipStream_t stream) {
  const int run = c1k_pick_run(L.frames, L.channels, 0);
  const int64_t slots = (L.frames + run - 1) / run * L.channels;
  hipLaunchKernelGGL(k_defer_compact, dim3((unsigned)((slots + 255) / 256)), dim3(256), 0, stream, (const uint32_t *)L.defer_list, (uint32_t)slots, list, counts,
                     L.channels, run, (uint32_t)L.frames);
}

void c1k_launch_analysis_spec(const C1EncodeLaunch &L0, bool all_short, hipStream_t stream) {
  static const int slots = c1k_wave_slots(k_analysis_spec<false>);
  C1EncodeLaunch L = L0;
  L.run_frames = c1k_pick_run(L.frames, L.channels, slots);
  const int64_t runs = (L.frames + L.run_frames - 1) / L.run_frames, n_slots = runs * L.channels;
  const dim3 grid((unsigned)((n_slots + kSpecWaves - 1) / kSpecWaves)), block(C1_WAVE * kSpecWaves);
  static const bool no_spread = getenv("C1_NO_SPREAD") != nullptr;
  L.spread_bits = 0;
  if (!no_spread) while ((1ll << L.spread_bits) < (int64_t)grid.x) L.spread_bits++;
  if (all_short) hipLaunchKernelGGL((k_analysis_spec<true>), grid, block, 0, stream, L);
  else hipLaunchKernelGGL((k_analysis_spec<false>), grid, block, 0, stream, L);
}
```

Baseline: 198.0 million.

## Interleave two analysis streams per wave in speculative long-block kernel

Restructures the speculative analysis kernel so each wavefront processes two independent slots (channel/run streams) interleaved frame by frame, halving threads per block while keeping the same number of slots per block. The goal is to expose instruction-level parallelism and hide the latency of wave reductions, LDS round trips and PCM loads by overlapping two independent dependency chains. Window weights are hoisted out of the per-stream loop. The cost is roughly doubled register and LDS pressure per wave (launch bounds drop to 3 waves per SIMD), plus extra bookkeeping for streams of different lengths. Short-block mode keeps a single stream, and an environment variable can select the old path.

```diff
diff --git a/carta1_amd/csrc/c1_api.hip b/carta1_amd/csrc/c1_api.hip
--- a/carta1_amd/csrc/c1_api.hip
+++ b/carta1_amd/csrc/c1_api.hip
@@ -392,6 +392,7 @@
   unsigned long long *d_spec_totals = nullptr;
   int spec_mode = 1;
   float spec_defer = 1.0f;
+  int spec_streams = kSpecStreams;
   bool decode_binary32 = false;
   int decode_model = C1_DECODE_EXACT;
   bool spec_tables_ok = false;
@@ -925,7 +926,7 @@
       HIP_TRY(hipMemsetAsync(ctx->d_redo[p], 0, kListHead * sizeof(uint32_t), sA));
       {
         ScopedTiming t(ctx, K_ANALYSIS, sA);
-        c1k_launch_analysis_spec(L, all_short_modes, sA);
+        c1k_launch_analysis_spec(L, all_short_modes, ctx->spec_streams, sA);
         if (L.defer_list) {
           C1EncodeLaunch D = L;
           uint32_t *dense = ctx->d_redo[p] + kListHead + 2 * (size_t)ctx->ws_units;
@@ -1245,6 +1246,8 @@
     if (ctx->spec_mode < 0 || ctx->spec_mode > 2) ctx->spec_mode = 1;
     const char *sd = getenv("C1_SPEC_DEFER");
     if (sd && atof(sd) > 0) ctx->spec_defer = (float)atof(sd);
+    const char *ss = getenv("C1_SPEC_STREAMS");
+    if (ss && (atoi(ss) == 1 || atoi(ss) == 2)) ctx->spec_streams = atoi(ss);
   }
   delete h;
   if (me != hipSuccess) { c1_ctx_destroy(ctx); return fail(C1_ERR_HIP, "table upload: %s", hipGetErrorString(me)); }
@@ -1630,7 +1633,7 @@
   L.channels = channels; L.frames = frames; L.halo_frames = halo_frames;
   L.tables = ctx->d_tables; L.opts = ctx->d_opts;
   L.coefs = coefs; L.eps = eps; L.side = side;
-  c1k_launch_analysis_spec(L, sp_short, ctx->stream);
+  c1k_launch_analysis_spec(L, sp_short, ctx->spec_streams, ctx->stream);
   HIP_TRY(hipGetLastError());
   return C1_OK;
 }
diff --git a/carta1_amd/csrc/c1_internal.h b/carta1_amd/csrc/c1_internal.h
--- a/carta1_amd/csrc/c1_internal.h
+++ b/carta1_amd/csrc/c1_internal.h
@@ -219,7 +219,8 @@
 
 void c1k_launch_analysis(const C1EncodeLaunch &L, bool detect, hipStream_t stream);
 void c1k_launch_analysis_long(const C1EncodeLaunch &L, hipStream_t stream);
-void c1k_launch_analysis_spec(const C1EncodeLaunch &L, bool all_short, hipStream_t stream);
+constexpr int kSpecStreams = 2;
+void c1k_launch_analysis_spec(const C1EncodeLaunch &L, bool all_short, int streams, hipStream_t stream);
 constexpr int kFeatureWsDoubles = 20;
 void c1k_launch_detect(const C1EncodeLaunch &L, float *bands_ws, double *feat_ws, uint8_t *modes_ws, uint32_t *lists_ws,
                        bool speculative, double *score_tap, hipStream_t stream);
diff --git a/carta1_amd/csrc/c1_k_spec.hip b/carta1_amd/csrc/c1_k_spec.hip
--- a/carta1_amd/csrc/c1_k_spec.hip
+++ b/carta1_amd/csrc/c1_k_spec.hip
@@ -163,39 +163,44 @@
   return x;
 }
 
-template <bool SHORT>
-__global__ __launch_bounds__(C1_WAVE * kSpecWaves, 5) void k_analysis_spec(C1EncodeLaunch L) {
+template <bool SHORT, int NS>
+__global__ __launch_bounds__(C1_WAVE * kSpecWaves / NS, NS == 1 ? 5 : 3) void k_analysis_spec(C1EncodeLaunch L) {
+  static_assert(NS == 1 || NS == 2, "one or two streams per wave");
+  static_assert(!SHORT || NS == 1, "short blocks: one stream per wave (two were not measured)");
+  constexpr int kThreads = C1_WAVE * kSpecWaves / NS;
   __shared__ SpecLds Sw[kSpecWaves];
   __shared__ alignas(16) float tab[kSpecTabFloats];
   __shared__ alignas(16) float tail_w[28][4];
   __shared__ alignas(8) float out_w[64][2];
   __shared__ alignas(16) SpecGeo geo[64];
   const int wave = __builtin_amdgcn_readfirstlane((int)(threadIdx.x >> 6));
-  SpecLds &S = Sw[wave];
+  SpecLds *const S = &Sw[wave * NS];
   const int lane0 = threadIdx.x & 63;
   int lane = lane0;
   {
     const float *src = reinterpret_cast<const float *>(reinterpret_cast<const char *>(L.tables) + kSpecTabBase);
-    for (int i = threadIdx.x; i < kSpecTabFloats; i += C1_WAVE * kSpecWaves) tab[i] = src[i];
-    if (threadIdx.x < 28 * 4) {
-      const int idx = threadIdx.x >> 2, j = threadIdx.x & 3;
+    for (int i = threadIdx.x; i < kSpecTabFloats; i += kThreads) tab[i] = src[i];
+    for (int v = threadIdx.x; v < C1_WAVE * kSpecWaves; v += kThreads) {
+    if (v < 28 * 4) {
+      const int idx = v >> 2, j = v & 3;
       const bool input = idx < 10;
       const int k = 4 * (input ? idx - 1 : idx - 10) - 1 + j;
       tail_w[idx][j] = (k >= 0 && k < 32) ? src[input ? 31 - k : k] : 1.0f;
     }
-    if (threadIdx.x >= 128 && threadIdx.x < 128 + 64) {
-      const int l = threadIdx.x - 128, k = 2 * (l - 48);
+    if (v >= 128 && v < 128 + 64) {
+      const int l = v - 128, k = 2 * (l - 48);
       out_w[l][0] = l >= 48 ? src[31 - k] : 1.0f;
       out_w[l][1] = l >= 48 ? src[30 - k] : 1.0f;
     }
-    if (!SHORT && threadIdx.x >= 192) {
-      const int l = threadIdx.x - 192;
+    if (!SHORT && v >= 192) {
+      const int l = v - 192;
       const SpecBase G = spec_base(l);
       const SfLong F = sf_long_geometry(l);
       const int po = G.po0 - kSpecTabBase, u = G.band0 ? 8 * G.d1 : -8 * G.d1, t = G.band0 ? 256 : -256;
       geo[l] = make_uint4((uint32_t)(4 * (G.band0 ? G.e0 : G.e1)) | ((uint32_t)(4 * (G.band0 ? G.e1 : G.e0)) << 16),
                           (uint32_t)po | ((uint32_t)(po + 8 * G.d1) << 16), ((uint32_t)u & 0xffffu) | ((uint32_t)t << 16),
                           (uint32_t)(F.src & ~3) | ((uint32_t)F.b << 9) | (F.wide ? 1u << 15 : 0u) | (F.store ? 1u << 16 : 0u));
+    }
     }
   }
   __syncthreads();
@@ -205,21 +210,46 @@
   };
   const uint32_t n_slots = (uint32_t)((L.frames + L.run_frames - 1) / L.run_frames) * (uint32_t)L.channels;
   const uint32_t group = L.spread_bits > 0 ? spread_block(blockIdx.x, gridDim.x, L.spread_bits) : blockIdx.x;
-  const uint32_t slot = group * kSpecWaves + (uint32_t)wave;
-  if (slot >= n_slots) return;
-  const int ch = (int)(slot % (uint32_t)L.channels);
-  const int64_t f0 = (int64_t)(slot / (uint32_t)L.channels) * L.run_frames;
-  const float *__restrict__ pcm = L.pcm[ch];
-  float *mem = S.mem;
-
-  for (int i = lane; i < 72; i += 64) mem[kW1Tail + i] = 0.0f;
-  if (lane < 48) mem[kW2 + 256 + lane] = 0.0f;
-  float ov0a = 0.0f, ov0b = 0.0f, ov1a = 0.0f, ov1b = 0.0f;
-  for (int i = lane; i < 76; i += 64) S.pre2[i] = 0.0f;
-  if (lane < 16) reinterpret_cast<uint32_t *>(S.sfi)[lane] = 0u;
+  const uint32_t slot0 = group * kSpecWaves + (uint32_t)(wave * NS);
+  if (slot0 >= n_slots) return;
+  const float *__restrict__ pcmf[NS];
+  int64_t unit0[NS];
+  int stop[NS], last[NS], kmin[NS];
+#pragma unroll
+  for (int s = 0; s < NS; s++) {
+    const bool have = s == 0 || slot0 + (uint32_t)s < n_slots;
+    const uint32_t slot = have ? slot0 + (uint32_t)s : slot0;
+    const int ch = (int)(slot % (uint32_t)L.channels);
+    const int64_t f0 = (int64_t)(slot / (uint32_t)L.channels) * L.run_frames;
+    const int64_t f_end = (f0 + L.run_frames < L.frames) ? f0 + L.run_frames : L.frames;
+    int64_t f_first = f0 - 1;
+    if (f_first < -(int64_t)L.halo_frames) f_first = -(int64_t)L.halo_frames;
+    if (f_first > f0) f_first = f0;
+    pcmf[s] = L.pcm[ch] + f0 * 512;
+    unit0[s] = f0 * L.channels + ch;
+    last[s] = (int)(f_end - f0) - 1;
+    stop[s] = have ? last[s] + 1 : 0;
+    kmin[s] = (int)(f_first - f0);
+  }
+
+  float ov0a[NS], ov0b[NS], ov1a[NS], ov1b[NS];
+  float p_prev[NS], q_prev[NS];
+  auto reset_state = [&](int s) {
+    float *mem = S[s].mem;
+    for (int i = lane; i < 72; i += 64) mem[kW1Tail + i] = 0.0f;
+    if (lane < 48) mem[kW2 + 256 + lane] = 0.0f;
+    ov0a[s] = 0.0f; ov0b[s] = 0.0f; ov1a[s] = 0.0f; ov1b[s] = 0.0f;
+    for (int i = lane; i < 76; i += 64) S[s].pre2[i] = 0.0f;
+    p_prev[s] = 0.0f; q_prev[s] = 0.0f;
+  };
+#pragma unroll
+  for (int s = 0; s < NS; s++) {
+    reset_state(s);
+    if (lane < 16) reinterpret_cast<uint32_t *>(S[s].sfi)[lane] = 0u;
+    if (SHORT && lane == 0) S[s].sfi[52] = (uint8_t)((L.opts->modes[0] & 3) | ((L.opts->modes[1] & 3) << 2) | ((L.opts->modes[2] & 3) << 4));
+  }
   SpecBase B0 = spec_base(lane0);
   const SfLong SFL0 = SHORT ? sf_geometry(lane0, 2, 2, 3) : sf_long_geometry(lane0);
-  if (SHORT && lane == 0) S.sfi[52] = (uint8_t)((L.opts->modes[0] & 3) | ((L.opts->modes[1] & 3) << 2) | ((L.opts->modes[2] & 3) << 4));
   const int s_band = lane0 < 16 ? 0 : (lane0 < 32 ? 1 : 2);
   const int s_g = lane0 - (s_band == 0 ? 0 : (s_band == 1 ? 16 : 32));
   const int s_blk = s_g >> 2, s_r2 = 2 * bitrev(s_g & 3, 2);
@@ -227,24 +257,28 @@
   const int s_hb0 = (s_band == 0 ? kH0 : (s_band == 1 ? kH1 : kH2)) + 32 * s_blk;
   const int s_c0 = (s_band == 0 ? 0 : (s_band == 1 ? 128 : 256)) + 32 * s_blk + 2 * (s_g & 3);
   constexpr int RT = 0;
-  float p_prev = 0.0f, q_prev = 0.0f;
   wave_fence();
 
-  const int64_t f_end = (f0 + L.run_frames < L.frames) ? f0 + L.run_frames : L.frames;
-  int64_t f_first = f0 - 1;
-  if (f_first < -(int64_t)L.halo_frames) f_first = -(int64_t)L.halo_frames;
-  if (f_first > f0) f_first = f0;
+  int k_first = kmin[0];
+  if (NS > 1 && kmin[NS - 1] < k_first) k_first = kmin[NS - 1];
   typedef float v4f __attribute__((ext_vector_type(4)));
-  v4f pre_a, pre_b;
-  {
-    const v4f *p4 = reinterpret_cast<const v4f *>(pcm + f_first * 512);
-    pre_a = p4[lane0]; pre_b = p4[64 + lane0];
-    asm volatile("" : "+v"(pre_a), "+v"(pre_b));
-  }
-  uint32_t deferred_from = 0xffffffffu;
-  unsigned long long open_bits = 0ull;
-  for (int64_t f = f_first; f < f_end; ++f) {
-    const bool emit = (f >= f0);
+  v4f pre_a[NS], pre_b[NS];
+  auto deliver_pcm = [&]() {
+    if constexpr (NS == 1) asm volatile("" : "+v"(pre_a[0]), "+v"(pre_b[0]));
+    else asm volatile("" : "+v"(pre_a[0]), "+v"(pre_b[0]), "+v"(pre_a[NS - 1]), "+v"(pre_b[NS - 1]));
+  };
+#pragma unroll
+  for (int s = 0; s < NS; s++) {
+    const v4f *p4 = reinterpret_cast<const v4f *>(pcmf[s] + (int64_t)(k_first > kmin[s] ? k_first : kmin[s]) * 512);
+    pre_a[s] = p4[lane0]; pre_b[s] = p4[64 + lane0];
+  }
+  deliver_pcm();
+  uint32_t deferred_from[NS];
+  unsigned long long open_bits[NS];
+#pragma unroll
+  for (int s = 0; s < NS; s++) { deferred_from[s] = 0xffffffffu; open_bits[s] = 0ull; }
+  for (int k = k_first; k < (NS > 1 && stop[NS - 1] > stop[0] ? stop[NS - 1] : stop[0]); ++k) {
+    const bool emit = (k >= 0);
     TablesPtr T = tables_for_this_frame(L.tables);
     lane = lane_for_this_frame(lane0);
     if constexpr (!SHORT) {
@@ -252,28 +286,41 @@
       asm volatile("" : "+v"(B0.za), "+v"(B0.zb), "+v"(B0.zc), "+v"(B0.zd), "+v"(B0.g));
     }
 
-    float P;
+    float P[NS];
     {
-      const v4f a = pre_a, b = pre_b;
-      {
-        const int p = w1_phys(lane);
-        float dl = 0.0f;
-        if (lane < 48) dl = mem[kW1Tail + p];
-        const int s = __mul24(6, lane) - 2 * (lane & 1);
-        *reinterpret_cast<v4f *>(&mem[72 + s]) = a;
-        *reinterpret_cast<v4f *>(&mem[72 + 384 + s]) = b;
-        if (lane < 48) mem[p] = dl;
-      }
-      v2f p2 = V2(a.x, a.y) * V2(a.x, a.y);
-      p2 = pk_fma(V2(a.z, a.w), V2(a.z, a.w), p2);
-      p2 = pk_fma(V2(b.x, b.y), V2(b.x, b.y), p2);
-      p2 = pk_fma(V2(b.z, b.w), V2(b.z, b.w), p2);
-      const float p = p2.x + p2.y;
-      P = wave_sum(p);
-    }
-    wave_fence();
-    float Q;
-    {
+      const int p = w1_phys(lane);
+      const int at = __mul24(6, lane) - 2 * (lane & 1);
+      float dl[NS];
+#pragma unroll
+      for (int s = 0; s < NS; s++) {
+        dl[s] = 0.0f;
+        if (lane < 48) dl[s] = S[s].mem[kW1Tail + p];
+      }
+      __builtin_amdgcn_wave_barrier();
+#pragma unroll
+      for (int s = 0; s < NS; s++) {
+        float *mem = S[s].mem;
+        const v4f a = pre_a[s], b = pre_b[s];
+        *reinterpret_cast<v4f *>(&mem[72 + at]) = a;
+        *reinterpret_cast<v4f *>(&mem[72 + 384 + at]) = b;
+        if (lane < 48) mem[p] = dl[s];
+        v2f p2 = V2(a.x, a.y) * V2(a.x, a.y);
+        p2 = pk_fma(V2(a.z, a.w), V2(a.z, a.w), p2);
+        p2 = pk_fma(V2(b.x, b.y), V2(b.x, b.y), p2);
+        p2 = pk_fma(V2(b.z, b.w), V2(b.z, b.w), p2);
+        P[s] = wave_sum(p2.x + p2.y);
+      }
+    }
+    wave_fence();
+    float Q[NS];
+    float4 tw_in = make_float4(1.0f, 1.0f, 1.0f, 1.0f), tw_next = tw_in;
+    if constexpr (!SHORT && NS > 1) {
+      tw_in = *reinterpret_cast<const float4 *>(tail_w[min(max(lane - 45, 0), 10)]);
+      tw_next = *reinterpret_cast<const float4 *>(tail_w[10 + max(lane - 46, 0)]);
+    }
+#pragma unroll
+    for (int s = 0; s < NS; s++) {
+      float *mem = S[s].mem;
       float lo[4], hi[4];
       if (own_block()) {
         v2f W[28];
@@ -287,33 +334,36 @@
         qmf_core_f32<4, 28, 1>(W, T, lo, hi);
       } else { for (int d = 0; d < 4; d++) { lo[d] = mem[lane + d]; hi[d] = 1.0f; } }
       {
-        const v4f *p4 = reinterpret_cast<const v4f *>(pcm + ((f + 1 < f_end) ? f + 1 : f) * 512);
-        pre_a = p4[lane]; pre_b = p4[64 + lane];
-      }
-      if (lane < 48) mem[kW2 + lane] = mem[kW2 + 256 + lane];
+        const v4f *p4 = reinterpret_cast<const v4f *>(pcmf[s] + (int64_t)(k < last[s] ? k + 1 : last[s]) * 512);
+        pre_a[s] = p4[lane]; pre_b[s] = p4[64 + lane];
+      }
+      float d2 = 0.0f;
+      if (lane < 48) d2 = mem[kW2 + 256 + lane];
+      __builtin_amdgcn_wave_barrier();
+      if (lane < 48) mem[kW2 + lane] = d2;
       *reinterpret_cast<float4 *>(&mem[kW2 + 48 + 4 * lane]) = make_float4(lo[0], lo[1], lo[2], lo[3]);
       v2f q2 = V2(lo[0], lo[1]) * V2(lo[0], lo[1]);
       q2 = pk_fma(V2(lo[2], lo[3]), V2(lo[2], lo[3]), q2);
       const float q = q2.x + q2.y;
-      Q = wave_sum(q);
+      Q[s] = wave_sum(q);
       if constexpr (!SHORT) {
-      if (emit && lane < 36) *reinterpret_cast<float2 *>(&mem[kIn2 + 111 + 2 * lane]) = *reinterpret_cast<const float2 *>(&S.pre2[2 * lane]);
+      if (emit && lane < 36) *reinterpret_cast<float2 *>(&mem[kIn2 + 111 + 2 * lane]) = *reinterpret_cast<const float2 *>(&S[s].pre2[2 * lane]);
       {
         const int wi = min(max(lane - 45, 0), 10);
-        const float4 wh = *reinterpret_cast<const float4 *>(tail_w[wi]);
+        const float4 wh = NS > 1 ? tw_in : *reinterpret_cast<const float4 *>(tail_w[wi]);
         const v2f h01 = V2(hi[0], hi[1]) * V2(wh.x, wh.y), h23 = V2(hi[2], hi[3]) * V2(wh.z, wh.w);
         if (emit && lane <= 54) *reinterpret_cast<float4 *>(&mem[kIn2 + 183 + 4 * lane]) = make_float4(h01.x, h01.y, h23.x, h23.y);
       }
       if (lane >= 46) {
-        const float4 wl = *reinterpret_cast<const float4 *>(tail_w[10 + lane - 46]);
+        const float4 wl = NS > 1 ? tw_next : *reinterpret_cast<const float4 *>(tail_w[10 + lane - 46]);
         const v2f l01 = V2(hi[0], hi[1]) * V2(wl.x, wl.y), l23 = V2(hi[2], hi[3]) * V2(wl.z, wl.w);
-        *reinterpret_cast<float4 *>(&S.pre2[4 * (lane - 46)]) = make_float4(l01.x, l01.y, l23.x, l23.y);
+        *reinterpret_cast<float4 *>(&S[s].pre2[4 * (lane - 46)]) = make_float4(l01.x, l01.y, l23.x, l23.y);
       }
       } else {
         if (emit) {
-          if (lane < 32) mem[kE2 + lane] = S.pre2[1 + lane];
+          if (lane < 32) mem[kE2 + lane] = S[s].pre2[1 + lane];
           if (lane < 39) {
-            const float x = S.pre2[33 + lane];
+            const float x = S[s].pre2[33 + lane];
             mem[kE2 + 32 + lane] = win[lane & 31] * x;
             mem[kH2 + lane] = x * win[31 - (lane & 31)];
           }
@@ -325,13 +375,22 @@
           if (pos < 256) {
             const float e = win[pos & 31] * x;
             if (emit) { mem[kE2 + 32 + pos] = e; mem[kH2 + pos] = x * win[31 - (pos & 31)]; }
-            if (pos >= 224) S.pre2[1 + pos - 224] = e;
-          } else S.pre2[33 + pos - 256] = x;
+            if (pos >= 224) S[s].pre2[1 + pos - 224] = e;
+          } else S[s].pre2[33 + pos - 256] = x;
         }
       }
     }
     wave_fence();
-    {
+    v2f ow_in = V2(1.0f, 1.0f);
+    float ow_next0 = 1.0f, ow_next1 = 1.0f;
+    if constexpr (!SHORT && NS > 1) {
+      ow_in = *reinterpret_cast<const v2f *>(out_w[lane]);
+      const int kw = 2 * max(lane - 48, 0);
+      ow_next0 = win[kw]; ow_next1 = win[kw + 1];
+    }
+#pragma unroll
+    for (int s = 0; s < NS; s++) {
+      float *mem = S[s].mem;
       float lo[2], hi[2];
       if (own_block()) {
         v2f W[26];
@@ -347,7 +406,7 @@
       if constexpr (!SHORT) {
       const int u = lane + 40, at = kR2 + 2 * (u + (u & ~15));
       {
-        const v2f wh = *reinterpret_cast<const v2f *>(out_w[lane]);
+        const v2f wh = NS > 1 ? ow_in : *reinterpret_cast<const v2f *>(out_w[lane]);
         const v2f o0 = V2(lo[0], lo[1]) * wh, o1 = V2(hi[1], hi[0]) * wh.yx;
         if (emit) {
           *reinterpret_cast<v2f *>(&mem[at]) = o0;
@@ -355,15 +414,15 @@
         }
       }
       if (lane >= 48) {
-        const int k = 2 * (lane - 48);
-        const float wl0 = win[k], wl1 = win[k + 1];
+        const int kw = 2 * (lane - 48);
+        const float wl0 = NS > 1 ? ow_next0 : win[kw], wl1 = NS > 1 ? ow_next1 : win[kw + 1];
         if (emit) {
           const int uo = lane - 24, ato = kR2 + 2 * (uo + (uo & ~15));
-          *reinterpret_cast<float2 *>(&mem[ato]) = make_float2(ov0a, ov0b);
-          *reinterpret_cast<float2 *>(&mem[ato + 32]) = make_float2(ov1b, ov1a);
+          *reinterpret_cast<float2 *>(&mem[ato]) = make_float2(ov0a[s], ov0b[s]);
+          *reinterpret_cast<float2 *>(&mem[ato + 32]) = make_float2(ov1b[s], ov1a[s]);
         }
-        ov0a = wl0 * lo[0]; ov0b = wl1 * lo[1];
-        ov1a = wl0 * hi[0]; ov1b = wl1 * hi[1];
+        ov0a[s] = wl0 * lo[0]; ov0b[s] = wl1 * lo[1];
+        ov1a[s] = wl0 * hi[0]; ov1b[s] = wl1 * hi[1];
       }
       } else {
         const int k = (2 * lane) & 31;
@@ -371,27 +430,37 @@
         const float e00 = wl0 * lo[0], e01 = wl1 * lo[1], e10 = wl0 * hi[0], e11 = wl1 * hi[1];
         if (emit) {
           if (lane >= 48) {
-            *reinterpret_cast<float2 *>(&mem[kE0 + 2 * (lane - 48)]) = make_float2(ov0a, ov0b);
-            *reinterpret_cast<float2 *>(&mem[kE1 + 2 * (lane - 48)]) = make_float2(ov1a, ov1b);
+            *reinterpret_cast<float2 *>(&mem[kE0 + 2 * (lane - 48)]) = make_float2(ov0a[s], ov0b[s]);
+            *reinterpret_cast<float2 *>(&mem[kE1 + 2 * (lane - 48)]) = make_float2(ov1a[s], ov1b[s]);
           }
           *reinterpret_cast<float2 *>(&mem[kE0 + 32 + 2 * lane]) = make_float2(e00, e01);
           *reinterpret_cast<float2 *>(&mem[kE1 + 32 + 2 * lane]) = make_float2(e10, e11);
           *reinterpret_cast<float2 *>(&mem[kH0 + 2 * lane]) = make_float2(lo[0] * wh0, lo[1] * wh1);
           *reinterpret_cast<float2 *>(&mem[kH1 + 2 * lane]) = make_float2(hi[0] * wh0, hi[1] * wh1);
         }
-        if (lane >= 48) { ov0a = e00; ov0b = e01; ov1a = e10; ov1b = e11; }
-      }
-    }
-    const float W = __builtin_amdgcn_sqrtf(P + p_prev), Lw = __builtin_amdgcn_sqrtf(Q + q_prev);
-    p_prev = P; q_prev = Q;
+        if (lane >= 48) { ov0a[s] = e00; ov0b[s] = e01; ov1a[s] = e10; ov1b[s] = e11; }
+      }
+    }
+    float W[NS], Lw[NS];
+#pragma unroll
+    for (int s = 0; s < NS; s++) {
+      W[s] = __builtin_amdgcn_sqrtf(P[s] + p_prev[s]); Lw[s] = __builtin_amdgcn_sqrtf(Q[s] + q_prev[s]);
+      p_prev[s] = P[s]; q_prev[s] = Q[s];
+    }
     wave_fence();
     if (!emit) {
-      asm volatile("" : "+v"(pre_a), "+v"(pre_b));
+      deliver_pcm();
+      if constexpr (NS > 1) {
+#pragma unroll
+        for (int s = 0; s < NS; s++)
+          if (kmin[s] == 0) reset_state(s);
+        wave_fence();
+      }
       continue;
     }
 
-    v2f x[4];
-    float zrow;
+    v2f xs[NS][4];
+    float zrow[NS];
     uint32_t gw_sf = 0;
     if constexpr (!SHORT) {
     const SpecBase &B = B0;
@@ -399,6 +468,9 @@
       const int qb = 4 * B.q2;
       const v2f t0 = table_f2(RT, B.pt0), t1 = table_f2(RT, B.pt0 + 2 * qb);
       const v2f t2 = table_f2(RT, B.pt0 + qb), t3 = table_f2(RT, B.pt0 + __mul24(3, qb));
+#pragma unroll
+      for (int s = 0; s < NS; s++) {
+      const float *mem = S[s].mem;
       const float a0 = mem[B.ia3 + 192], c0 = mem[B.ic0];
       const float a1 = mem[B.ia3 + 64], c1 = mem[B.ic0 + 128];
       const float a2 = mem[B.ia3 + 128], c2 = mem[B.ic0 + 64];
@@ -409,28 +481,34 @@
       const v2f rm0 = pk_fma(V2(b0, d0), PMN, V2(a0, c0)), rm3 = pk_fma(V2(b3, d3), PNM, V2(a3, c3));
       const v2f rm1 = V2(a1, c1), rm2 = V2(a2, c2);
       auto twiddle = [](v2f rm, v2f t) { const v2f u = pk_mul_yx_yny(rm, t); return pk_fma(rm, t.xx, u); };
+      v2f (&x)[4] = xs[s];
       x[0] = twiddle(rm0, t0); x[1] = twiddle(rm1, t1); x[2] = twiddle(rm2, t2); x[3] = twiddle(rm3, t3);
       v2f en2 = x[0] * x[0];
 #pragma unroll
       for (int j = 1; j < 4; j++) en2 = pk_fma(x[j], x[j], en2);
-      zrow = row_allreduce(en2.x + en2.y);
+      zrow[s] = row_allreduce(en2.x + en2.y);
       const v2f u0 = x[0] + x[1], u1 = x[0] - x[1], u2 = x[2] + x[3], u3 = x[2] - x[3];
       x[0] = u0 + u2;
       x[2] = u0 - u2;
       x[1] = pk_fma(u3.yx, PMN, u1);
       x[3] = pk_fma(u3.yx, PNM, u1);
-    }
-    v2f *z = reinterpret_cast<v2f *>(mem);
-    {
-      float4 *dst = reinterpret_cast<float4 *>(z + B.za);
+      }
+    }
+    auto z = [&](int s) { return reinterpret_cast<v2f *>(S[s].mem); };
+#pragma unroll
+    for (int s = 0; s < NS; s++) {
+      v2f (&x)[4] = xs[s];
+      float4 *dst = reinterpret_cast<float4 *>(z(s) + B.za);
       dst[0] = make_float4(x[0].x, x[0].y, x[1].x, x[1].y);
       dst[1] = make_float4(x[2].x, x[2].y, x[3].x, x[3].y);
     }
     const int twb = (int)offsetof(C1DevTables, r4b) + 24 * (B.g & 3);
     const v2f wBa = table_f2(RT, twb), wBb = table_f2(RT, twb + 8), wBc = table_f2(RT, twb + 16);
     wave_fence();
-    {
-      v2f *p = z + B.zb;
+#pragma unroll
+    for (int s = 0; s < NS; s++) {
+      v2f (&x)[4] = xs[s];
+      v2f *p = z(s) + B.zb;
       x[0] = lds_f2(p); x[1] = lds_f2(p + 4); x[2] = lds_f2(p + 8); x[3] = lds_f2(p + 12);
       radix4_round(x, wBa, wBb, wBc);
       p[0] = x[0]; p[4] = x[1]; p[8] = x[2]; p[12] = x[3];
@@ -439,8 +517,10 @@
     const v2f wCa = table_f2(RT, twc), wCb = table_f2(RT, twc + 8), wCc = table_f2(RT, twc + 16);
     const v2f wDa = table_f2(RT, twd), wDb = table_f2(RT, twd + 256);
     wave_fence();
-    {
-      v2f *p = z + B.zc;
+#pragma unroll
+    for (int s = 0; s < NS; s++) {
+      v2f (&x)[4] = xs[s];
+      v2f *p = z(s) + B.zc;
       x[0] = lds_f2(p); x[1] = lds_f2(p + 20); x[2] = lds_f2(p + 40); x[3] = lds_f2(p + 60);
       radix4_round(x, wCa, wCb, wCc);
       if (B.band2) { p[0] = x[0]; p[20] = x[1]; p[40] = x[2]; p[60] = x[3]; }
@@ -450,16 +530,19 @@
     const v2f p0 = table_f2(RT, po0), p1 = table_f2(RT, po1);
     const v2f p2 = table_f2(RT, po0 + 256), p3 = table_f2(RT, po1 + 256);
     wave_fence();
+    const int cf = (int)(gw.x & 0xffffu), cs = (int)(gw.x >> 16);
+    const int su = (int)(gw.z << 16) >> 16, st = (int)gw.z >> 16, sut = su + st;
+#pragma unroll
+    for (int s = 0; s < NS; s++) {
+    v2f (&x)[4] = xs[s];
     if (B.band2) {
-      const v2f *p = z + B.zd;
+      const v2f *p = z(s) + B.zd;
       x[0] = lds_f2(p); x[1] = lds_f2(p + 80); x[2] = lds_f2(p + 40); x[3] = lds_f2(p + 120);
       const v2f y1 = cmul32n(x[1], wDa), y3 = cmul32n(x[3], wDb);
       const v2f e0 = x[0], e2 = x[2];
       x[0] = e0 + y1; x[1] = e0 - y1; x[2] = e2 + y3; x[3] = e2 - y3;
     }
-    char *coefw = reinterpret_cast<char *>(mem + kR2);
-    const int cf = (int)(gw.x & 0xffffu), cs = (int)(gw.x >> 16);
-    const int su = (int)(gw.z << 16) >> 16, st = (int)gw.z >> 16, sut = su + st;
+    char *coefw = reinterpret_cast<char *>(S[s].mem + kR2);
 #pragma unroll
     for (int j = 0; j < 4; j++) {
       const v2f t = j == 0 ? p0 : (j == 1 ? p1 : (j == 2 ? p2 : p3));
@@ -469,12 +552,14 @@
       *reinterpret_cast<float *>(coefw + (cf + step)) = -o.x;
       *reinterpret_cast<float *>(coefw + (cs - step)) = o.y;
     }
+    }
     gw_sf = gw.w;
     wave_fence();
 
     }
-    float *coef = mem + kR2;
     if constexpr (SHORT) {
+    float *mem = S[0].mem;
+    v2f (&x)[4] = xs[0];
     int eb = s_eb0, hb = s_hb0, r2 = s_r2;
     asm volatile("" : "+v"(eb), "+v"(hb), "+v"(r2));
     {
@@ -495,7 +580,7 @@
       en += dpp_read<0xB1>(en);
       en += dpp_read<0x4E>(en);
       en = fmaxf(en, dpp_read<0x141>(en));
-      zrow = fmaxf(en, dpp_read<0x140>(en));
+      zrow[0] = fmaxf(en, dpp_read<0x140>(en));
       const v2f u0 = x[0] + x[1], u1 = x[0] - x[1], u2 = x[2] + x[3], u3 = x[2] - x[3];
       x[0] = u0 + u2;
       x[2] = u0 - u2;
@@ -536,39 +621,50 @@
     wave_fence();
 
     }
-    const int64_t unit = f * L.channels + ch;
-    asm volatile("" : "+v"(pre_a), "+v"(pre_b));
-    {
-      v4f *dst = reinterpret_cast<v4f *>(L.coefs + (unit << 9));
-      const v4f *src = reinterpret_cast<const v4f *>(coef);
-      const int lq = lane_for_this_frame(lane0);
-      __builtin_nontemporal_store(src[lq], &dst[lq]);
-      __builtin_nontemporal_store(src[64 + lq], &dst[64 + lq]);
-    }
-    const float Z0 = __builtin_amdgcn_sqrtf(lane_value(zrow, 0)), Z1 = __builtin_amdgcn_sqrtf(lane_value(zrow, 16));
-    const float Z2 = __builtin_amdgcn_sqrtf(SHORT ? fmaxf(lane_value(zrow, 32), lane_value(zrow, 48)) : lane_value(zrow, 32) + lane_value(zrow, 48));
+    deliver_pcm();
+    const int lq = lane_for_this_frame(lane0);
     const float eabs = T->spec_eabs;
     const float cz0 = SHORT ? T->spec_cz_short[0] : T->spec_cz[0], cz1 = SHORT ? T->spec_cz_short[1] : T->spec_cz[1], cz2 = SHORT ? T->spec_cz_short[2] : T->spec_cz[2];
     const float cw0 = SHORT ? T->spec_cw_short[0] : T->spec_cw[0], cw1 = SHORT ? T->spec_cw_short[1] : T->spec_cw[1], cw2 = SHORT ? T->spec_cw_short[2] : T->spec_cw[2];
     const float cl0 = SHORT ? T->spec_cl_short[0] : T->spec_cl[0], cl1 = SHORT ? T->spec_cl_short[1] : T->spec_cl[1], cl2 = SHORT ? T->spec_cl_short[2] : T->spec_cl[2];
-    const float e0 = __builtin_fmaf(cz0, Z0, __builtin_fmaf(cw0, W, __builtin_fmaf(cl0, Lw, eabs)));
-    const float e1 = __builtin_fmaf(cz1, Z1, __builtin_fmaf(cw1, W, __builtin_fmaf(cl1, Lw, eabs)));
-    const float e2 = __builtin_fmaf(cz2, Z2, __builtin_fmaf(cw2, W, __builtin_fmaf(cl2, Lw, eabs)));
+    SfLong SFL = SFL0;
+    int sf_src;
+    if constexpr (SHORT) {
+      asm volatile("" : "+v"(SFL.src), "+v"(SFL.cnt));
+      sf_src = SFL.src;
+    } else {
+      const uint32_t sw = gw_sf;
+      SFL.b = (int)((sw >> 9) & 63u);
+      SFL.wide = ((sw >> 15) & 1u) != 0u;
+      SFL.store = ((sw >> 16) & 1u) != 0u;
+      sf_src = (int)(sw & 0x1ffu);
+    }
+#pragma unroll
+    for (int s = 0; s < NS; s++) {
+    const bool live = NS == 1 || k < stop[s];
+    float *coef = S[s].mem + kR2;
+    const int64_t unit = unit0[s] + (int64_t)k * L.channels;
+    if (live) {
+      v4f *dst = reinterpret_cast<v4f *>(L.coefs + (unit << 9));
+      const v4f *src = reinterpret_cast<const v4f *>(coef);
+      __builtin_nontemporal_store(src[lq], &dst[lq]);
+      __builtin_nontemporal_store(src[64 + lq], &dst[64 + lq]);
+    }
+    const float zr = zrow[s];
+    const float Z0 = __builtin_amdgcn_sqrtf(lane_value(zr, 0)), Z1 = __builtin_amdgcn_sqrtf(lane_value(zr, 16));
+    const float Z2 = __builtin_amdgcn_sqrtf(SHORT ? fmaxf(lane_value(zr, 32), lane_value(zr, 48)) : lane_value(zr, 32) + lane_value(zr, 48));
+    const float e0 = __builtin_fmaf(cz0, Z0, __builtin_fmaf(cw0, W[s], __builtin_fmaf(cl0, Lw[s], eabs)));
+    const float e1 = __builtin_fmaf(cz1, Z1, __builtin_fmaf(cw1, W[s], __builtin_fmaf(cl1, Lw[s], eabs)));
+    const float e2 = __builtin_fmaf(cz2, Z2, __builtin_fmaf(cw2, W[s], __builtin_fmaf(cl2, Lw[s], eabs)));
     bool unstable;
     {
-      SfLong SFL = SFL0;
       float mx = 0.0f;
       if constexpr (SHORT) {
-        asm volatile("" : "+v"(SFL.src), "+v"(SFL.cnt));
-        const float *src = coef + SFL.src;
+        const float *src = coef + sf_src;
 #pragma unroll
         for (int j = 0; j < 12; j++) mx = fmaxf(mx, fabsf(src[j < SFL.cnt ? j : SFL.cnt - 1]));
       } else {
-        const uint32_t sw = gw_sf;
-        SFL.b = (int)((sw >> 9) & 63u);
-        SFL.wide = ((sw >> 15) & 1u) != 0u;
-        SFL.store = ((sw >> 16) & 1u) != 0u;
-        const float4 *grp = reinterpret_cast<const float4 *>(coef + (sw & 0x1ffu));
+        const float4 *grp = reinterpret_cast<const float4 *>(coef + sf_src);
         mx = sf_scan_long_groups(grp[0], grp[1], grp[2]);
       }
       const float other = __int_as_float(__builtin_amdgcn_update_dpp(0, __float_as_int(mx), 0xB1, 0xf, 0xf, false));
@@ -576,21 +672,29 @@
       const float e = SFL.b >= 36 ? e2 : (SFL.b >= 20 ? e1 : e0);
       const float lo = fmaxf((mx - e) * 0.99999976f, 0.0f), hi = (mx + e) * 1.00000024f;
       const int s_lo = scale_factor_index_fast(lo, T->sf_m1, T->sf_m2), s_hi = scale_factor_index_fast(hi, T->sf_m1, T->sf_m2);
-      if (SFL.store) S.sfi[SFL.b] = (uint8_t)s_lo;
+      if (SFL.store) S[s].sfi[SFL.b] = (uint8_t)s_lo;
       unstable = lane < 60 && !(s_lo == s_hi && e < __builtin_huge_valf());
     }
     const bool any_unstable = __builtin_amdgcn_ballot_w64(unstable) != 0;
     wave_fence();
-    if (L.defer_list != nullptr && (((int)(f - f0)) & (kSpecCheckFrames - 1)) == 0) {
-      if (spec_should_defer(S.sfi, lane, e0, e1, e2, L.opts, L.spec_defer)) { deferred_from = (uint32_t)unit; break; }
-    }
-    if (any_unstable) open_bits |= 1ull << (int)((f - f0) & 63);
-    if (lane < 16) reinterpret_cast<uint32_t *>(L.side + unit * kSideBytes)[lane] = reinterpret_cast<const uint32_t *>(S.sfi)[lane];
+    bool stays = live;
+    if (live && L.defer_list != nullptr && (k & (kSpecCheckFrames - 1)) == 0) {
+      if (spec_should_defer(S[s].sfi, lane, e0, e1, e2, L.opts, L.spec_defer)) { deferred_from[s] = (uint32_t)unit; stop[s] = k; stays = false; }
+    }
+    if (stays) {
+    if (any_unstable) open_bits[s] |= 1ull << (k & 63);
+    if (lane < 16) reinterpret_cast<uint32_t *>(L.side + unit * kSideBytes)[lane] = reinterpret_cast<const uint32_t *>(S[s].sfi)[lane];
     if (lane == 0) *reinterpret_cast<float4 *>(L.eps + unit * kEpsFloats) = make_float4(e0, e1, e2, __int_as_float(any_unstable ? 1 : 0));
-    wave_fence();
-  }
-  if (L.defer_list != nullptr && lane0 == 0) L.defer_list[slot] = deferred_from;
-  if (L.open_masks != nullptr && lane0 == 0) L.open_masks[slot] = open_bits;
+    }
+    wave_fence();
+    }
+  }
+#pragma unroll
+  for (int s = 0; s < NS; s++) {
+    if (s > 0 && slot0 + (uint32_t)s >= n_slots) break;
+    if (L.defer_list != nullptr && lane0 == 0) L.defer_list[slot0 + s] = deferred_from[s];
+    if (L.open_masks != nullptr && lane0 == 0) L.open_masks[slot0 + s] = open_bits[s];
+  }
 }
 
 __global__ __launch_bounds__(256) void k_defer_compact(const uint32_t *__restrict__ slots, uint32_t n_slots, uint32_t *__restrict__ list, uint32_t *__restrict__ counts,
@@ -673,15 +777,16 @@
                      L.channels, run, (uint32_t)L.frames);
 }
 
-void c1k_launch_analysis_spec(const C1EncodeLaunch &L0, bool all_short, hipStream_t stream) {
-  static const int slots = c1k_wave_slots(k_analysis_spec<false>);
+void c1k_launch_analysis_spec(const C1EncodeLaunch &L0, bool all_short, int streams, hipStream_t stream) {
+  static const int slots = c1k_wave_slots(k_analysis_spec<false, 1>);
   C1EncodeLaunch L = L0;
   L.run_frames = c1k_pick_run(L.frames, L.channels, slots);
   const int64_t runs = (L.frames + L.run_frames - 1) / L.run_frames, n_slots = runs * L.channels;
-  const dim3 grid((unsigned)((n_slots + kSpecWaves - 1) / kSpecWaves)), block(C1_WAVE * kSpecWaves);
+  const dim3 grid((unsigned)((n_slots + kSpecWaves - 1) / kSpecWaves));
   static const bool no_spread = getenv("C1_NO_SPREAD") != nullptr;
   L.spread_bits = 0;
   if (!no_spread) while ((1ll << L.spread_bits) < (int64_t)grid.x) L.spread_bits++;
-  if (all_short) hipLaunchKernelGGL((k_analysis_spec<true>), grid, block, 0, stream, L);
-  else hipLaunchKernelGGL((k_analysis_spec<false>), grid, block, 0, stream, L);
-}
+  if (all_short) hipLaunchKernelGGL((k_analysis_spec<true, 1>), grid, dim3(C1_WAVE * kSpecWaves), 0, stream, L);
+  else if (streams == 1) hipLaunchKernelGGL((k_analysis_spec<false, 1>), grid, dim3(C1_WAVE * kSpecWaves), 0, stream, L);
+  else hipLaunchKernelGGL((k_analysis_spec<false, 2>), grid, dim3(C1_WAVE * kSpecWaves / 2), 0, stream, L);
+}
```

Result: slower. 185.8 million (-6.1%).
